# linkedin/spark-tfrecord

Hardware: AMD Instinct MI355X
Metric: rows/sec read+write (1M-row Example round-trip) (higher is better)
Workload: dtype wire(int64/float32/bytes); 1 GPU; model=Example{id:int64, ints:Int64List[8], floats:FloatList[16], tokens:BytesList[2]}, global_batch=1000000, parallelism=dp1, rows_per_rank=1000000, engine=gpu, storage=/dev/shm, crc_verify=True

## Files before the change

### csrc/codec_core.h

```cpp
#pragma once

#include <cstdint>
#include <cstring>

#include "crc32c.h"

namespace tfrec {

using i64 = int64_t;
using u64 = uint64_t;
using u32 = uint32_t;
using u8 = uint8_t;

enum Kind : int32_t { KIND_BYTES = 1, KIND_FLOAT = 2, KIND_INT64 = 3 };

enum RecordFormat : int32_t { FMT_EXAMPLE = 0, FMT_SEQUENCE = 1, FMT_BYTE_ARRAY = 2 };

enum CodecErr : int32_t {
  ERR_OK = 0,
  ERR_TRUNCATED = -1,
  ERR_BAD_VARINT = -2,
  ERR_KIND_MISMATCH = -3,
  ERR_BAD_WIRETYPE = -4,
  ERR_OVERFLOW = -5,
  ERR_NAME_TOO_LONG = -6,
};


TFR_HOSTDEV inline int popcount64(u64 x) { return __builtin_popcountll(x); }

TFR_HOSTDEV inline int ctz64(u64 x) { return __builtin_ctzll(x); }

constexpr u64 kMsbMask = 0x8080808080808080ull;

TFR_HOSTDEV inline const u8* read_varint(const u8* p, const u8* end, u64* out) {
  if (end - p >= 8) {
    u64 w;
    __builtin_memcpy(&w, p, 8);
    u64 stops = ~w & kMsbMask;
    if (stops) {
      int nb = (ctz64(stops) >> 3) + 1;
      u64 v = 0;
      for (int i = 0; i < nb; ++i)
        v |= ((w >> (8 * i)) & 0x7F) << (7 * i);
      *out = v;
      return p + nb;
    }
    u64 v = 0;
    for (int i = 0; i < 8; ++i) v |= ((w >> (8 * i)) & 0x7F) << (7 * i);
    const u8* q = p + 8;
    for (int shift = 56; q < end && shift < 64; shift += 7) {
      u8 b = *q++;
      v |= static_cast<u64>(b & 0x7F) << shift;
      if (!(b & 0x80)) {
        *out = v;
        return q;
      }
    }
    return nullptr;
  }
  u64 v = 0;
  int shift = 0;
  while (p < end) {
    u8 b = *p++;
    v |= static_cast<u64>(b & 0x7F) << shift;
    if (!(b & 0x80)) {
      *out = v;
      return p;
    }
    shift += 7;
    if (shift >= 64) return nullptr;
  }
  return nullptr;
}

TFR_HOSTDEV inline int varint_size(u64 v) {
  int n = 1;
  while (v >= 0x80) {
    v >>= 7;
    ++n;
  }
  return n;
}

TFR_HOSTDEV inline u8* write_varint(u8* p, u64 v) {
  while (v >= 0x80) {
    *p++ = static_cast<u8>(v) | 0x80;
    v >>= 7;
  }
  *p++ = static_cast<u8>(v);
  return p;
}


struct FieldDescRaw {
  int32_t kind;
  int32_t is_seq;
  int32_t name_off;
  int32_t name_len;
};

struct SchemaView {
  int32_t nfields;
  const FieldDescRaw* fields;
  const u8* names;

  TFR_HOSTDEV const u8* name(int f) const { return names + fields[f].name_off; }
  TFR_HOSTDEV int name_len(int f) const { return fields[f].name_len; }
};

TFR_HOSTDEV inline SchemaView schema_view(const u8* blob) {
  SchemaView v;
  int32_t n;
  __builtin_memcpy(&n, blob, 4);
  v.nfields = n;
  v.fields = reinterpret_cast<const FieldDescRaw*>(blob + 4);
  v.names = blob + 4 + n * static_cast<int>(sizeof(FieldDescRaw));
  return v;
}

TFR_HOSTDEV inline bool name_eq(const u8* a, const u8* b, int n) {
  while (n >= 8) {
    u64 x, y;
    __builtin_memcpy(&x, a, 8);
    __builtin_memcpy(&y, b, 8);
    if (x != y) return false;
    a += 8;
    b += 8;
    n -= 8;
  }
  for (int i = 0; i < n; ++i)
    if (a[i] != b[i]) return false;
  return true;
}

TFR_HOSTDEV inline int schema_find(const SchemaView& s, const u8* name, int len,
                                   int want_seq) {
  for (int f = 0; f < s.nfields; ++f) {
    if (s.fields[f].is_seq == want_seq && s.fields[f].name_len == len &&
        name_eq(s.name(f), name, len))
      return f;
  }
  return -1;
}


struct FieldStat {
  i64 pos;
  i64 len;
  i64 nvals;
  i64 nbytes;
  i64 nlists;
  int32_t kind_found;
  int32_t err;
};

TFR_HOSTDEV inline void field_stat_clear(FieldStat* st) {
  st->pos = -1;
  st->len = 0;
  st->nvals = 0;
  st->nbytes = 0;
  st->nlists = 0;
  st->kind_found = 0;
  st->err = 0;
}

TFR_HOSTDEV inline const u8* skip_field(const u8* p, const u8* end, u32 wiretype) {
  u64 tmp;
  switch (wiretype) {
    case 0:
      return read_varint(p, end, &tmp);
    case 1:
      return (end - p >= 8) ? p + 8 : nullptr;
    case 2:
      p = read_varint(p, end, &tmp);
      if (!p || static_cast<u64>(end - p) < tmp) return nullptr;
      return p + tmp;
    case 5:
      return (end - p >= 4) ? p + 4 : nullptr;
    default:
      return nullptr;
  }
}

TFR_HOSTDEV inline int32_t count_list_body(const u8* p, const u8* end, int32_t kind,
                                           i64* nvals, i64* nbytes) {
  while (p < end) {
    u64 tag;
    p = read_varint(p, end, &tag);
    if (!p) return ERR_BAD_VARINT;
    u32 fieldno = static_cast<u32>(tag >> 3);
    u32 wt = static_cast<u32>(tag & 7);
    if (fieldno != 1) {
      p = skip_field(p, end, wt);
      if (!p) return ERR_TRUNCATED;
      continue;
    }
    if (kind == KIND_BYTES) {
      if (wt != 2) return ERR_BAD_WIRETYPE;
      u64 len;
      p = read_varint(p, end, &len);
      if (!p || static_cast<u64>(end - p) < len) return ERR_TRUNCATED;
      *nvals += 1;
      *nbytes += static_cast<i64>(len);
      p += len;
    } else if (kind == KIND_FLOAT) {
      if (wt == 2) {
        u64 len;
        p = read_varint(p, end, &len);
        if (!p || static_cast<u64>(end - p) < len) return ERR_TRUNCATED;
        *nvals += static_cast<i64>(len / 4);
        p += len;
      } else if (wt == 5) {
        if (end - p < 4) return ERR_TRUNCATED;
        *nvals += 1;
        p += 4;
      } else {
        return ERR_BAD_WIRETYPE;
      }
    } else {
      if (wt == 2) {
        u64 len;
        p = read_varint(p, end, &len);
        if (!p || static_cast<u64>(end - p) < len) return ERR_TRUNCATED;
        const u8* q = p;
        const u8* qe = p + len;
        if (len && (qe[-1] & 0x80)) return ERR_BAD_VARINT;
        i64 cnt = 0;
        while (qe - q >= 8) {
          u64 w;
          __builtin_memcpy(&w, q, 8);
          cnt += popcount64(~w & kMsbMask);
          q += 8;
        }
        for (; q < qe; ++q) cnt += !(*q & 0x80);
        *nvals += cnt;
        p = qe;
      } else if (wt == 0) {
        u64 v;
        p = read_varint(p, end, &v);
        if (!p) return ERR_BAD_VARINT;
        *nvals += 1;
      } else {
        return ERR_BAD_WIRETYPE;
      }
    }
  }
  return ERR_OK;
}

TFR_HOSTDEV inline int32_t scan_feature_body(const u8* p, const u8* end,
                                             int32_t expect_kind, int32_t* kind_found,
                                             i64* nvals, i64* nbytes) {
  while (p < end) {
    u64 tag;
    p = read_varint(p, end, &tag);
    if (!p) return ERR_BAD_VARINT;
    u32 fieldno = static_cast<u32>(tag >> 3);
    u32 wt = static_cast<u32>(tag & 7);
    if (fieldno >= 1 && fieldno <= 3 && wt == 2) {
      u64 len;
      p = read_varint(p, end, &len);
      if (!p || static_cast<u64>(end - p) < len) return ERR_TRUNCATED;
      *kind_found = static_cast<int32_t>(fieldno);
      if (expect_kind >= 0 && static_cast<int32_t>(fieldno) != expect_kind)
        return ERR_KIND_MISMATCH;
      int32_t rc = count_list_body(p, p + len, static_cast<int32_t>(fieldno), nvals,
                                   nbytes);
      if (rc != ERR_OK) return rc;
      p += len;
    } else {
      p = skip_field(p, end, wt);
      if (!p) return ERR_TRUNCATED;
    }
  }
  return ERR_OK;
}

TFR_HOSTDEV inline int32_t scan_features_body(const u8* p, const u8* end, i64 base,
                                              const SchemaView& schema, int want_seq,
                                              FieldStat* stats) {
  const u8* body_start = p;
  while (p < end) {
    u64 tag;
    p = read_varint(p, end, &tag);
    if (!p) return ERR_BAD_VARINT;
    u32 fieldno = static_cast<u32>(tag >> 3);
    u32 wt = static_cast<u32>(tag & 7);
    if (fieldno != 1 || wt != 2) {
      p = skip_field(p, end, wt);
      if (!p) return ERR_TRUNCATED;
      continue;
    }
    u64 entry_len;
    p = read_varint(p, end, &entry_len);
    if (!p || static_cast<u64>(end - p) < entry_len) return ERR_TRUNCATED;
    const u8* ep = p;
    const u8* ee = p + entry_len;
    p = ee;
    const u8* key = nullptr;
    u64 key_len = 0;
    const u8* val = nullptr;
    u64 val_len = 0;
    while (ep < ee) {
      u64 etag;
      ep = read_varint(ep, ee, &etag);
      if (!ep) return ERR_BAD_VARINT;
      u32 efn = static_cast<u32>(etag >> 3);
      u32 ewt = static_cast<u32>(etag & 7);
      if (efn == 1 && ewt == 2) {
        ep = read_varint(ep, ee, &key_len);
        if (!ep || static_cast<u64>(ee - ep) < key_len) return ERR_TRUNCATED;
        key = ep;
        ep += key_len;
      } else if (efn == 2 && ewt == 2) {
        ep = read_varint(ep, ee, &val_len);
        if (!ep || static_cast<u64>(ee - ep) < val_len) return ERR_TRUNCATED;
        val = ep;
        ep += val_len;
      } else {
        ep = skip_field(ep, ee, ewt);
        if (!ep) return ERR_TRUNCATED;
      }
    }
    if (!key) continue;
    int f = schema_find(schema, key, static_cast<int>(key_len), want_seq);
    if (f < 0) continue;
    FieldStat* st = &stats[f];
    st->nvals = 0;
    st->nbytes = 0;
    st->nlists = 0;
    st->kind_found = 0;
    st->err = 0;
    st->pos = base + (val ? (val - body_start) : 0);
    st->len = static_cast<i64>(val_len);
    if (!want_seq) {
      int32_t rc = scan_feature_body(val, val + val_len, schema.fields[f].kind,
                                     &st->kind_found, &st->nvals, &st->nbytes);
      if (rc != ERR_OK) st->err = rc;
    } else {
      const u8* lp = val;
      const u8* le = val + val_len;
      while (lp < le) {
        u64 ltag;
        lp = read_varint(lp, le, &ltag);
        if (!lp) {
          st->err = ERR_BAD_VARINT;
          break;
        }
        u32 lfn = static_cast<u32>(ltag >> 3);
        u32 lwt = static_cast<u32>(ltag & 7);
        if (lfn == 1 && lwt == 2) {
          u64 flen;
          lp = read_varint(lp, le, &flen);
          if (!lp || static_cast<u64>(le - lp) < flen) {
            st->err = ERR_TRUNCATED;
            break;
          }
          st->nlists += 1;
          int32_t kf = 0;
          int32_t rc = scan_feature_body(lp, lp + flen, schema.fields[f].kind, &kf,
                                         &st->nvals, &st->nbytes);
          if (rc != ERR_OK) {
            st->err = rc;
            break;
          }
          if (kf) st->kind_found = kf;
          lp += flen;
        } else {
          lp = skip_field(lp, le, lwt);
          if (!lp) {
            st->err = ERR_TRUNCATED;
            break;
          }
        }
      }
    }
  }
  return ERR_OK;
}

TFR_HOSTDEV inline int32_t scan_record(const u8* data, i64 abs_off, i64 rec_len,
                                       int32_t fmt, const SchemaView& schema,
                                       FieldStat* stats) {
  const u8* p = data + abs_off;
  const u8* end = p + rec_len;
  while (p < end) {
    u64 tag;
    p = read_varint(p, end, &tag);
    if (!p) return ERR_BAD_VARINT;
    u32 fieldno = static_cast<u32>(tag >> 3);
    u32 wt = static_cast<u32>(tag & 7);
    bool is_features =
        (fmt == FMT_EXAMPLE && fieldno == 1) || (fmt == FMT_SEQUENCE && fieldno == 1);
    bool is_feature_lists = (fmt == FMT_SEQUENCE && fieldno == 2);
    if ((is_features || is_feature_lists) && wt == 2) {
      u64 len;
      p = read_varint(p, end, &len);
      if (!p || static_cast<u64>(end - p) < len) return ERR_TRUNCATED;
      i64 base = (p - data);
      if (is_features) {
        int32_t rc = scan_features_body(p, p + len, base, schema, 0, stats);
        if (rc != ERR_OK) return rc;
      } else {
        int32_t rc = scan_features_body(p, p + len, base, schema, 1, stats);
        if (rc != ERR_OK) return rc;
      }
      p += len;
    } else {
      p = skip_field(p, end, wt);
      if (!p) return ERR_TRUNCATED;
    }
  }
  return ERR_OK;
}


constexpr int32_t ERR_RETRY_UNFUSED = -100;

TFR_HOSTDEV inline u32 crc32c_step8(u32 crc, u64 w, const uint32_t (*tab)[256]) {
  w ^= crc;
  return tab[7][w & 0xFF] ^ tab[6][(w >> 8) & 0xFF] ^ tab[5][(w >> 16) & 0xFF] ^
         tab[4][(w >> 24) & 0xFF] ^ tab[3][(w >> 32) & 0xFF] ^
         tab[2][(w >> 40) & 0xFF] ^ tab[1][(w >> 48) & 0xFF] ^
         tab[0][(w >> 56) & 0xFF];
}

struct ScanCur {
  const u8* base;
  i64 len;
  i64 pos;
  i64 wpos;
  u64 w0, w1;
  u32 crc;
  const uint32_t (*tab)[256];
};

TFR_HOSTDEV inline u64 cur_load(const ScanCur& c, i64 at) {
  if (at + 8 <= c.len) {
    u64 w;
    __builtin_memcpy(&w, c.base + at, 8);
    return w;
  }
  u64 w = 0;
  for (i64 b = at; b < c.len; ++b) w |= (u64)c.base[b] << (8 * (b - at));
  return w;
}

TFR_HOSTDEV inline void cur_init(ScanCur& c, const u8* base, i64 len,
                                 const uint32_t (*tab)[256]) {
  c.base = base;
  c.len = len;
  c.pos = 0;
  c.wpos = 0;
  c.tab = tab;
  c.crc = 0xFFFFFFFFu;
  c.w0 = cur_load(c, 0);
  c.w1 = cur_load(c, 8);
}

TFR_HOSTDEV inline u64 cur_peek(const ScanCur& c) {
  int sh = (int)(c.pos - c.wpos) * 8;
  if (sh == 0) return c.w0;
  if (sh == 64) return c.w1;
  return (c.w0 >> sh) | (c.w1 << (64 - sh));
}

TFR_HOSTDEV inline void cur_advance(ScanCur& c, i64 k) {
  c.pos += k;
  while (c.pos > c.wpos + 8) {
    if (c.wpos + 8 <= c.len) c.crc = crc32c_step8(c.crc, c.w0, c.tab);
    c.w0 = c.w1;
    c.wpos += 8;
    c.w1 = cur_load(c, c.wpos + 8);
  }
}

TFR_HOSTDEV inline u32 cur_finish_crc(ScanCur& c) {
  while (c.wpos + 8 <= c.len) {
    c.crc = crc32c_step8(c.crc, c.w0, c.tab);
    c.w0 = c.w1;
    c.wpos += 8;
    c.w1 = cur_load(c, c.wpos + 8);
  }
  u32 crc = c.crc;
  for (i64 b = c.wpos; b < c.len; ++b)
    crc = c.tab[0][(crc ^ c.base[b]) & 0xFF] ^ (crc >> 8);
  return ~crc;
}

TFR_HOSTDEV inline bool cur_varint(ScanCur& c, i64 end, u64* out) {
  i64 avail = end - c.pos;
  if (avail <= 0) return false;
  u64 w = cur_peek(c);
  u64 stops = ~w & kMsbMask;
  if (stops) {
    int nb = (ctz64(stops) >> 3) + 1;
    if (nb > avail) return false;
    u64 v = 0;
    for (int i = 0; i < nb; ++i) v |= ((w >> (8 * i)) & 0x7F) << (7 * i);
    *out = v;
    cur_advance(c, nb);
    return true;
  }
  if (avail < 9) return false;
  u64 v = 0;
  for (int i = 0; i < 8; ++i) v |= ((w >> (8 * i)) & 0x7F) << (7 * i);
  cur_advance(c, 8);
  for (int shift = 56; shift < 64 && c.pos < end; shift += 7) {
    u8 b = (u8)cur_peek(c);
    v |= (u64)(b & 0x7F) << shift;
    cur_advance(c, 1);
    if (!(b & 0x80)) {
      *out = v;
      return true;
    }
  }
  return false;
}

TFR_HOSTDEV inline int32_t cur_skip_field(ScanCur& c, i64 end, u32 wt) {
  u64 tmp;
  switch (wt) {
    case 0:
      return cur_varint(c, end, &tmp) ? ERR_OK : ERR_BAD_VARINT;
    case 1:
      if (end - c.pos < 8) return ERR_TRUNCATED;
      cur_advance(c, 8);
      return ERR_OK;
    case 2:
      if (!cur_varint(c, end, &tmp)) return ERR_BAD_VARINT;
      if ((u64)(end - c.pos) < tmp) return ERR_TRUNCATED;
      cur_advance(c, (i64)tmp);
      return ERR_OK;
    case 5:
      if (end - c.pos < 4) return ERR_TRUNCATED;
      cur_advance(c, 4);
      return ERR_OK;
    default:
      return ERR_BAD_WIRETYPE;
  }
}

TFR_HOSTDEV inline i64 cur_count_terms(ScanCur& c, i64 n) {
  i64 cnt = 0;
  while (n >= 8) {
    cnt += popcount64(~cur_peek(c) & kMsbMask);
    cur_advance(c, 8);
    n -= 8;
  }
  if (n > 0) {
    u64 mask = kMsbMask >> (8 * (8 - n));
    cnt += popcount64(~cur_peek(c) & mask);
    cur_advance(c, n);
  }
  return cnt;
}

TFR_HOSTDEV inline int32_t cur_count_list_body(ScanCur& c, i64 end, int32_t kind,
                                               i64* nvals, i64* nbytes) {
  while (c.pos < end) {
    u64 tag;
    if (!cur_varint(c, end, &tag)) return ERR_BAD_VARINT;
    u32 fieldno = (u32)(tag >> 3), wt = (u32)(tag & 7);
    if (fieldno != 1) {
      int32_t rc = cur_skip_field(c, end, wt);
      if (rc != ERR_OK) return rc;
      continue;
    }
    if (kind == KIND_BYTES) {
      if (wt != 2) return ERR_BAD_WIRETYPE;
      u64 blen;
      if (!cur_varint(c, end, &blen)) return ERR_BAD_VARINT;
      if ((u64)(end - c.pos) < blen) return ERR_TRUNCATED;
      *nvals += 1;
      *nbytes += (i64)blen;
      cur_advance(c, (i64)blen);
    } else if (kind == KIND_FLOAT) {
      if (wt == 2) {
        u64 blen;
        if (!cur_varint(c, end, &blen)) return ERR_BAD_VARINT;
        if ((u64)(end - c.pos) < blen) return ERR_TRUNCATED;
        *nvals += (i64)(blen / 4);
        cur_advance(c, (i64)blen);
      } else if (wt == 5) {
        if (end - c.pos < 4) return ERR_TRUNCATED;
        *nvals += 1;
        cur_advance(c, 4);
      } else {
        return ERR_BAD_WIRETYPE;
      }
    } else {
      if (wt == 2) {
        u64 blen;
        if (!cur_varint(c, end, &blen)) return ERR_BAD_VARINT;
        if ((u64)(end - c.pos) < blen) return ERR_TRUNCATED;
        if (blen && (c.base[c.pos + (i64)blen - 1] & 0x80))
          return ERR_BAD_VARINT;
        *nvals += cur_count_terms(c, (i64)blen);
      } else if (wt == 0) {
        u64 v;
        if (!cur_varint(c, end, &v)) return ERR_BAD_VARINT;
        *nvals += 1;
      } else {
        return ERR_BAD_WIRETYPE;
      }
    }
  }
  return ERR_OK;
}

TFR_HOSTDEV inline int32_t cur_scan_feature_body(ScanCur& c, i64 end,
                                                 int32_t expect_kind,
                                                 int32_t* kind_found, i64* nvals,
                                                 i64* nbytes) {
  while (c.pos < end) {
    u64 tag;
    if (!cur_varint(c, end, &tag)) return ERR_BAD_VARINT;
    u32 fieldno = (u32)(tag >> 3), wt = (u32)(tag & 7);
    if (fieldno >= 1 && fieldno <= 3 && wt == 2) {
      u64 blen;
      if (!cur_varint(c, end, &blen)) return ERR_BAD_VARINT;
      if ((u64)(end - c.pos) < blen) return ERR_TRUNCATED;
      *kind_found = (int32_t)fieldno;
      if (expect_kind >= 0 && (int32_t)fieldno != expect_kind)
        return ERR_KIND_MISMATCH;
      int32_t rc = cur_count_list_body(c, c.pos + (i64)blen, (int32_t)fieldno,
                                       nvals, nbytes);
      if (rc != ERR_OK) return rc;
    } else {
      int32_t rc = cur_skip_field(c, end, wt);
      if (rc != ERR_OK) return rc;
    }
  }
  return ERR_OK;
}

TFR_HOSTDEV inline int32_t cur_scan_features_body(ScanCur& c, i64 end, i64 data_rel,
                                                  const SchemaView& schema,
                                                  int want_seq, FieldStat* stats) {
  i64 body_start = c.pos;
  while (c.pos < end) {
    u64 tag;
    if (!cur_varint(c, end, &tag)) return ERR_BAD_VARINT;
    u32 fieldno = (u32)(tag >> 3), wt = (u32)(tag & 7);
    if (fieldno != 1 || wt != 2) {
      int32_t rc = cur_skip_field(c, end, wt);
      if (rc != ERR_OK) return rc;
      continue;
    }
    u64 entry_len;
    if (!cur_varint(c, end, &entry_len)) return ERR_BAD_VARINT;
    if ((u64)(end - c.pos) < entry_len) return ERR_TRUNCATED;
    i64 ee = c.pos + (i64)entry_len;
    int f = -1;
    bool key_seen = false;
    bool val_seen = false;
    while (c.pos < ee) {
      u64 etag;
      if (!cur_varint(c, ee, &etag)) return ERR_BAD_VARINT;
      u32 efn = (u32)(etag >> 3), ewt = (u32)(etag & 7);
      if (efn == 1 && ewt == 2) {
        if (val_seen) return ERR_RETRY_UNFUSED;
        u64 klen;
        if (!cur_varint(c, ee, &klen)) return ERR_BAD_VARINT;
        if ((u64)(ee - c.pos) < klen) return ERR_TRUNCATED;
        f = schema_find(schema, c.base + c.pos, (int)klen, want_seq);
        key_seen = true;
        cur_advance(c, (i64)klen);
      } else if (efn == 2 && ewt == 2) {
        if (!key_seen) return ERR_RETRY_UNFUSED;
        val_seen = true;
        u64 vlen;
        if (!cur_varint(c, ee, &vlen)) return ERR_BAD_VARINT;
        if ((u64)(ee - c.pos) < vlen) return ERR_TRUNCATED;
        i64 ve = c.pos + (i64)vlen;
        if (f < 0) {
          cur_advance(c, (i64)vlen);
          continue;
        }
        FieldStat* st = &stats[f];
        st->nvals = 0;
        st->nbytes = 0;
        st->nlists = 0;
        st->kind_found = 0;
        st->err = 0;
        st->pos = data_rel + c.pos;
        st->len = (i64)vlen;
        if (!want_seq) {
          int32_t rc = cur_scan_feature_body(c, ve, schema.fields[f].kind,
                                             &st->kind_found, &st->nvals,
                                             &st->nbytes);
          if (rc == ERR_RETRY_UNFUSED) return rc;
          if (rc != ERR_OK) st->err = rc;
        } else {
          while (c.pos < ve && st->err == ERR_OK) {
            u64 ltag;
            if (!cur_varint(c, ve, &ltag)) {
              st->err = ERR_BAD_VARINT;
              break;
            }
            u32 lfn = (u32)(ltag >> 3), lwt = (u32)(ltag & 7);
            if (lfn == 1 && lwt == 2) {
              u64 flen;
              if (!cur_varint(c, ve, &flen) || (u64)(ve - c.pos) < flen) {
                st->err = ERR_TRUNCATED;
                break;
              }
              st->nlists += 1;
              int32_t kf = 0;
              int32_t rc = cur_scan_feature_body(c, c.pos + (i64)flen,
                                                 schema.fields[f].kind, &kf,
                                                 &st->nvals, &st->nbytes);
              if (rc == ERR_RETRY_UNFUSED) return rc;
              if (rc != ERR_OK) {
                st->err = rc;
                break;
              }
              if (kf) st->kind_found = kf;
            } else {
              int32_t rc = cur_skip_field(c, ve, lwt);
              if (rc != ERR_OK) {
                st->err = ERR_TRUNCATED;
                break;
              }
            }
          }
        }
        if (c.pos < ve) cur_advance(c, ve - c.pos);
      } else {
        int32_t rc = cur_skip_field(c, ee, ewt);
        if (rc != ERR_OK) return rc;
      }
    }
    if (f >= 0 && !val_seen) {
      FieldStat* st = &stats[f];
      st->pos = data_rel + body_start;
      st->len = 0;
      st->nvals = 0;
      st->nbytes = 0;
      st->nlists = 0;
      st->kind_found = 0;
      st->err = 0;
    }
  }
  return ERR_OK;
}

TFR_HOSTDEV inline int32_t scan_record_fused(const u8* data, i64 abs_off,
                                             i64 rec_len, int32_t fmt,
                                             const SchemaView& schema,
                                             FieldStat* stats, u32* crc_out,
                                             const uint32_t (*tab)[256]) {
  ScanCur c;
  cur_init(c, data + abs_off, rec_len, tab);
  while (c.pos < rec_len) {
    u64 tag;
    if (!cur_varint(c, rec_len, &tag)) return ERR_BAD_VARINT;
    u32 fieldno = (u32)(tag >> 3), wt = (u32)(tag & 7);
    bool is_features = fieldno == 1;
    bool is_fl = (fmt == FMT_SEQUENCE && fieldno == 2);
    if ((is_features || is_fl) && wt == 2) {
      u64 blen;
      if (!cur_varint(c, rec_len, &blen)) return ERR_BAD_VARINT;
      if ((u64)(rec_len - c.pos) < blen) return ERR_TRUNCATED;
      int32_t rc = cur_scan_features_body(c, c.pos + (i64)blen, abs_off, schema,
                                          is_fl ? 1 : 0, stats);
      if (rc != ERR_OK) return rc;
    } else {
      int32_t rc = cur_skip_field(c, rec_len, wt);
      if (rc != ERR_OK) return rc;
    }
  }
  *crc_out = cur_finish_crc(c);
  return ERR_OK;
}


struct DecodeDst {
  i64* i64_vals;
  float* f32_vals;
  u8* bytes_data;
  i64* elem_len;
  i64* sub_count;
};


template <bool OFFS = false>
TFR_HOSTDEV inline int32_t extract_list_body(const u8* p, const u8* end, int32_t kind,
                                             const DecodeDst& dst, i64* vi, i64* bi) {
  while (p < end) {
    u64 tag;
    p = read_varint(p, end, &tag);
    if (!p) return ERR_BAD_VARINT;
    u32 fieldno = static_cast<u32>(tag >> 3);
    u32 wt = static_cast<u32>(tag & 7);
    if (fieldno != 1) {
      p = skip_field(p, end, wt);
      if (!p) return ERR_TRUNCATED;
      continue;
    }
    if (kind == KIND_BYTES) {
      u64 len;
      p = read_varint(p, end, &len);
      if (!p || static_cast<u64>(end - p) < len) return ERR_TRUNCATED;
      u8* d = dst.bytes_data + *bi;
      u64 i = 0;
      for (; i + 8 <= len; i += 8) {
        u64 w;
        __builtin_memcpy(&w, p + i, 8);
        __builtin_memcpy(d + i, &w, 8);
      }
      for (; i < len; ++i) d[i] = p[i];
      dst.elem_len[*vi] = OFFS ? *bi : static_cast<i64>(len);
      *bi += static_cast<i64>(len);
      *vi += 1;
      p += len;
    } else if (kind == KIND_FLOAT) {
      if (wt == 2) {
        u64 len;
        p = read_varint(p, end, &len);
        if (!p || static_cast<u64>(end - p) < len) return ERR_TRUNCATED;
        u64 n = len / 4;
        __builtin_memcpy(dst.f32_vals + *vi, p, n * 4);
        *vi += static_cast<i64>(n);
        p += len;
      } else {
        if (end - p < 4) return ERR_TRUNCATED;
        float v;
        __builtin_memcpy(&v, p, 4);
        dst.f32_vals[(*vi)++] = v;
        p += 4;
      }
    } else {
      if (wt == 2) {
        u64 len;
        p = read_varint(p, end, &len);
        if (!p || static_cast<u64>(end - p) < len) return ERR_TRUNCATED;
        const u8* q = p;
        const u8* qe = p + len;
        while (q < qe) {
          u64 v;
          q = read_varint(q, qe, &v);
          if (!q) return ERR_BAD_VARINT;
          dst.i64_vals[(*vi)++] = static_cast<i64>(v);
        }
        p = qe;
      } else {
        u64 v;
        p = read_varint(p, end, &v);
        if (!p) return ERR_BAD_VARINT;
        dst.i64_vals[(*vi)++] = static_cast<i64>(v);
      }
    }
  }
  return ERR_OK;
}

template <bool OFFS = false>
TFR_HOSTDEV inline int32_t extract_feature_body(const u8* p, const u8* end,
                                                int32_t kind, const DecodeDst& dst,
                                                i64* vi, i64* bi) {
  while (p < end) {
    u64 tag;
    p = read_varint(p, end, &tag);
    if (!p) return ERR_BAD_VARINT;
    u32 fieldno = static_cast<u32>(tag >> 3);
    u32 wt = static_cast<u32>(tag & 7);
    if (fieldno >= 1 && fieldno <= 3 && wt == 2) {
      u64 len;
      p = read_varint(p, end, &len);
      if (!p || static_cast<u64>(end - p) < len) return ERR_TRUNCATED;
      int32_t rc = extract_list_body<OFFS>(p, p + len, kind, dst, vi, bi);
      if (rc != ERR_OK) return rc;
      p += len;
    } else {
      p = skip_field(p, end, wt);
      if (!p) return ERR_TRUNCATED;
    }
  }
  return ERR_OK;
}

template <bool OFFS = false>
TFR_HOSTDEV inline int32_t extract_field(const u8* data, i64 pos, i64 len,
                                         int32_t kind, int32_t is_seq,
                                         const DecodeDst& dst, i64 val_base,
                                         i64 byte_base, i64 list_base) {
  if (pos < 0) return ERR_OK;
  const u8* p = data + pos;
  const u8* end = p + len;
  i64 vi = val_base;
  i64 bi = byte_base;
  if (!is_seq)
    return extract_feature_body<OFFS>(p, end, kind, dst, &vi, &bi);
  i64 li = list_base;
  while (p < end) {
    u64 tag;
    p = read_varint(p, end, &tag);
    if (!p) return ERR_BAD_VARINT;
    u32 fieldno = static_cast<u32>(tag >> 3);
    u32 wt = static_cast<u32>(tag & 7);
    if (fieldno == 1 && wt == 2) {
      u64 flen;
      p = read_varint(p, end, &flen);
      if (!p || static_cast<u64>(end - p) < flen) return ERR_TRUNCATED;
      i64 v_before = vi;
      int32_t rc = extract_feature_body<OFFS>(p, p + flen, kind, dst, &vi, &bi);
      if (rc != ERR_OK) return rc;
      dst.sub_count[li++] = OFFS ? v_before : vi - v_before;
      p += flen;
    } else {
      p = skip_field(p, end, wt);
      if (!p) return ERR_TRUNCATED;
    }
  }
  return ERR_OK;
}


struct FieldColumn {
  int32_t kind;
  int32_t is_seq;
  const u8* presence;
  const i64* row_off;
  const i64* list_off;
  const i64* sub_off;
  const i64* elem_off;
  const u8* bytes_data;
  const i64* i64_vals;
  const float* f32_vals;
};

TFR_HOSTDEV inline i64 list_body_size(const FieldColumn& c, i64 v0, i64 v1) {
  if (c.kind == KIND_FLOAT) {
    i64 n = v1 - v0;
    return n ? (1 + varint_size(static_cast<u64>(4 * n)) + 4 * n) : 0;
  }
  if (c.kind == KIND_INT64) {
    i64 packed = 0;
    for (i64 v = v0; v < v1; ++v)
      packed += varint_size(static_cast<u64>(c.i64_vals[v]));
    return packed ? (1 + varint_size(static_cast<u64>(packed)) + packed) : 0;
  }
  i64 sz = 0;
  for (i64 v = v0; v < v1; ++v) {
    i64 blen = c.elem_off[v + 1] - c.elem_off[v];
    sz += 1 + varint_size(static_cast<u64>(blen)) + blen;
  }
  return sz;
}

TFR_HOSTDEV inline i64 feature_body_size(const FieldColumn& c, i64 v0, i64 v1) {
  i64 body = list_body_size(c, v0, v1);
  return 1 + varint_size(static_cast<u64>(body)) + body;
}

TFR_HOSTDEV inline u8* emit_list_body(u8* o, const FieldColumn& c, i64 v0, i64 v1) {
  if (c.kind == KIND_FLOAT) {
    i64 n = v1 - v0;
    if (n) {
      *o++ = 0x0A;
      o = write_varint(o, static_cast<u64>(4 * n));
      __builtin_memcpy(o, c.f32_vals + v0, static_cast<size_t>(4 * n));
      o += 4 * n;
    }
  } else if (c.kind == KIND_INT64) {
    i64 packed = 0;
    for (i64 v = v0; v < v1; ++v)
      packed += varint_size(static_cast<u64>(c.i64_vals[v]));
    if (packed) {
      *o++ = 0x0A;
      o = write_varint(o, static_cast<u64>(packed));
      for (i64 v = v0; v < v1; ++v)
        o = write_varint(o, static_cast<u64>(c.i64_vals[v]));
    }
  } else {
    for (i64 v = v0; v < v1; ++v) {
      i64 b0 = c.elem_off[v];
      i64 blen = c.elem_off[v + 1] - b0;
      *o++ = 0x0A;
      o = write_varint(o, static_cast<u64>(blen));
      for (i64 i = 0; i < blen; ++i) o[i] = c.bytes_data[b0 + i];
      o += blen;
    }
  }
  return o;
}

TFR_HOSTDEV inline u8* emit_feature_body(u8* o, const FieldColumn& c, i64 v0, i64 v1) {
  i64 body = list_body_size(c, v0, v1);
  *o++ = static_cast<u8>((c.kind << 3) | 2);
  o = write_varint(o, static_cast<u64>(body));
  return emit_list_body(o, c, v0, v1);
}

TFR_HOSTDEV inline i64 features_entry_size(const FieldColumn& c, const SchemaView& s,
                                           int f, i64 v0, i64 v1) {
  i64 fb = feature_body_size(c, v0, v1);
  i64 klen = s.name_len(f);
  return (1 + varint_size(static_cast<u64>(klen)) + klen) +
         (1 + varint_size(static_cast<u64>(fb)) + fb);
}

TFR_HOSTDEV inline u8* emit_features_entry(u8* o, const FieldColumn& c,
                                           const SchemaView& s, int f, i64 v0, i64 v1) {
  i64 fb = feature_body_size(c, v0, v1);
  i64 klen = s.name_len(f);
  *o++ = 0x0A;
  o = write_varint(o, static_cast<u64>(klen));
  const u8* nm = s.name(f);
  for (i64 i = 0; i < klen; ++i) o[i] = nm[i];
  o += klen;
  *o++ = 0x12;
  o = write_varint(o, static_cast<u64>(fb));
  return emit_feature_body(o, c, v0, v1);
}

TFR_HOSTDEV inline i64 feature_list_body_size(const FieldColumn& c, i64 r) {
  i64 sz = 0;
  for (i64 j = c.list_off[r]; j < c.list_off[r + 1]; ++j) {
    i64 fb = feature_body_size(c, c.sub_off[j], c.sub_off[j + 1]);
    sz += 1 + varint_size(static_cast<u64>(fb)) + fb;
  }
  return sz;
}

TFR_HOSTDEV inline u8* emit_feature_list_body(u8* o, const FieldColumn& c, i64 r) {
  for (i64 j = c.list_off[r]; j < c.list_off[r + 1]; ++j) {
    i64 fb = feature_body_size(c, c.sub_off[j], c.sub_off[j + 1]);
    *o++ = 0x0A;
    o = write_varint(o, static_cast<u64>(fb));
    o = emit_feature_body(o, c, c.sub_off[j], c.sub_off[j + 1]);
  }
  return o;
}

TFR_HOSTDEV inline i64 feature_lists_entry_size(const FieldColumn& c,
                                                const SchemaView& s, int f, i64 r) {
  i64 flb = feature_list_body_size(c, r);
  i64 klen = s.name_len(f);
  return (1 + varint_size(static_cast<u64>(klen)) + klen) +
         (1 + varint_size(static_cast<u64>(flb)) + flb);
}

TFR_HOSTDEV inline u8* emit_feature_lists_entry(u8* o, const FieldColumn& c,
                                                const SchemaView& s, int f, i64 r) {
  i64 flb = feature_list_body_size(c, r);
  i64 klen = s.name_len(f);
  *o++ = 0x0A;
  o = write_varint(o, static_cast<u64>(klen));
  const u8* nm = s.name(f);
  for (i64 i = 0; i < klen; ++i) o[i] = nm[i];
  o += klen;
  *o++ = 0x12;
  o = write_varint(o, static_cast<u64>(flb));
  return emit_feature_list_body(o, c, r);
}

TFR_HOSTDEV inline i64 record_payload_size(const FieldColumn* cols,
                                           const SchemaView& s, int32_t fmt, i64 r) {
  i64 ctx_body = 0;
  i64 fl_body = 0;
  for (int f = 0; f < s.nfields; ++f) {
    const FieldColumn& c = cols[f];
    if (!c.presence[r]) continue;
    if (!c.is_seq) {
      i64 e = features_entry_size(c, s, f, c.row_off[r], c.row_off[r + 1]);
      ctx_body += 1 + varint_size(static_cast<u64>(e)) + e;
    } else {
      i64 e = feature_lists_entry_size(c, s, f, r);
      fl_body += 1 + varint_size(static_cast<u64>(e)) + e;
    }
  }
  i64 total = 0;
  if (fmt == FMT_EXAMPLE) {
    total += 1 + varint_size(static_cast<u64>(ctx_body)) + ctx_body;
  } else {
    if (ctx_body) total += 1 + varint_size(static_cast<u64>(ctx_body)) + ctx_body;
    total += 1 + varint_size(static_cast<u64>(fl_body)) + fl_body;
  }
  return total;
}

TFR_HOSTDEV inline u8* emit_record_payload(u8* o, const FieldColumn* cols,
                                           const SchemaView& s, int32_t fmt, i64 r) {
  i64 ctx_body = 0, fl_body = 0;
  for (int f = 0; f < s.nfields; ++f) {
    const FieldColumn& c = cols[f];
    if (!c.presence[r]) continue;
    if (!c.is_seq) {
      i64 e = features_entry_size(c, s, f, c.row_off[r], c.row_off[r + 1]);
      ctx_body += 1 + varint_size(static_cast<u64>(e)) + e;
    } else {
      i64 e = feature_lists_entry_size(c, s, f, r);
      fl_body += 1 + varint_size(static_cast<u64>(e)) + e;
    }
  }
  auto emit_ctx = [&](u8* oo) {
    for (int f = 0; f < s.nfields; ++f) {
      const FieldColumn& c = cols[f];
      if (!c.presence[r] || c.is_seq) continue;
      i64 e = features_entry_size(c, s, f, c.row_off[r], c.row_off[r + 1]);
      *oo++ = 0x0A;
      oo = write_varint(oo, static_cast<u64>(e));
      oo = emit_features_entry(oo, c, s, f, c.row_off[r], c.row_off[r + 1]);
    }
    return oo;
  };
  auto emit_fl = [&](u8* oo) {
    for (int f = 0; f < s.nfields; ++f) {
      const FieldColumn& c = cols[f];
      if (!c.presence[r] || !c.is_seq) continue;
      i64 e = feature_lists_entry_size(c, s, f, r);
      *oo++ = 0x0A;
      oo = write_varint(oo, static_cast<u64>(e));
      oo = emit_feature_lists_entry(oo, c, s, f, r);
    }
    return oo;
  };
  if (fmt == FMT_EXAMPLE) {
    *o++ = 0x0A;
    o = write_varint(o, static_cast<u64>(ctx_body));
    o = emit_ctx(o);
  } else {
    if (ctx_body) {
      *o++ = 0x0A;
      o = write_varint(o, static_cast<u64>(ctx_body));
      o = emit_ctx(o);
    }
    *o++ = 0x12;
    o = write_varint(o, static_cast<u64>(fl_body));
    o = emit_fl(o);
  }
  return o;
}



struct WriteCur {
  u8* base;
  i64 pos;
  i64 wpos;
  u64 win;
  u32 crc;
  const uint32_t (*tab)[256];
};

TFR_HOSTDEV inline void wcur_init(WriteCur& w, u8* base,
                                  const uint32_t (*tab)[256]) {
  w.base = base;
  w.pos = 0;
  w.wpos = 0;
  w.win = 0;
  w.crc = 0xFFFFFFFFu;
  w.tab = tab;
}

TFR_HOSTDEV inline void wcur_flush8(WriteCur& w) {
  __builtin_memcpy(w.base + w.wpos, &w.win, 8);
  w.crc = crc32c_step8(w.crc, w.win, w.tab);
  w.wpos += 8;
  w.win = 0;
}

TFR_HOSTDEV inline void wcur_put(WriteCur& w, u8 b) {
  w.win |= (u64)b << (8 * (w.pos - w.wpos));
  if (++w.pos - w.wpos == 8) wcur_flush8(w);
}

TFR_HOSTDEV inline void wcur_varint(WriteCur& w, u64 v) {
  while (v >= 0x80) {
    wcur_put(w, (u8)(v | 0x80));
    v >>= 7;
  }
  wcur_put(w, (u8)v);
}

TFR_HOSTDEV inline void wcur_bytes(WriteCur& w, const u8* src, i64 n) {
  while (n > 0 && (w.pos - w.wpos) != 0) {
    wcur_put(w, *src++);
    --n;
  }
  while (n >= 8) {
    __builtin_memcpy(&w.win, src, 8);
    w.pos += 8;
    wcur_flush8(w);
    src += 8;
    n -= 8;
  }
  while (n-- > 0) wcur_put(w, *src++);
}

TFR_HOSTDEV inline u32 wcur_finish(WriteCur& w) {
  int rem = (int)(w.pos - w.wpos);
  if (!rem) return ~w.crc;
  __builtin_memcpy(w.base + w.wpos, &w.win, (size_t)rem);
  u32 crc = w.crc;
  for (int i = 0; i < rem; ++i)
    crc = w.tab[0][(crc ^ (u8)(w.win >> (8 * i))) & 0xFF] ^ (crc >> 8);
  return ~crc;
}

TFR_HOSTDEV inline void wcur_list_body(WriteCur& w, const FieldColumn& c,
                                       i64 v0, i64 v1) {
  if (c.kind == KIND_FLOAT) {
    i64 n = v1 - v0;
    if (n) {
      wcur_put(w, 0x0A);
      wcur_varint(w, (u64)(4 * n));
      wcur_bytes(w, (const u8*)(c.f32_vals + v0), 4 * n);
    }
  } else if (c.kind == KIND_INT64) {
    i64 packed = 0;
    for (i64 v = v0; v < v1; ++v)
      packed += varint_size((u64)c.i64_vals[v]);
    if (packed) {
      wcur_put(w, 0x0A);
      wcur_varint(w, (u64)packed);
      for (i64 v = v0; v < v1; ++v) wcur_varint(w, (u64)c.i64_vals[v]);
    }
  } else {
    for (i64 v = v0; v < v1; ++v) {
      i64 b0 = c.elem_off[v];
      i64 blen = c.elem_off[v + 1] - b0;
      wcur_put(w, 0x0A);
      wcur_varint(w, (u64)blen);
      wcur_bytes(w, c.bytes_data + b0, blen);
    }
  }
}

TFR_HOSTDEV inline void wcur_feature_body(WriteCur& w, const FieldColumn& c,
                                          i64 v0, i64 v1) {
  i64 body = list_body_size(c, v0, v1);
  wcur_put(w, (u8)((c.kind << 3) | 2));
  wcur_varint(w, (u64)body);
  wcur_list_body(w, c, v0, v1);
}

TFR_HOSTDEV inline void wcur_features_entry(WriteCur& w, const FieldColumn& c,
                                            const SchemaView& s, int f, i64 v0,
                                            i64 v1) {
  i64 fb = feature_body_size(c, v0, v1);
  i64 klen = s.name_len(f);
  wcur_put(w, 0x0A);
  wcur_varint(w, (u64)klen);
  wcur_bytes(w, s.name(f), klen);
  wcur_put(w, 0x12);
  wcur_varint(w, (u64)fb);
  wcur_feature_body(w, c, v0, v1);
}

TFR_HOSTDEV inline void wcur_feature_list_body(WriteCur& w,
                                               const FieldColumn& c, i64 r) {
  for (i64 j = c.list_off[r]; j < c.list_off[r + 1]; ++j) {
    i64 fb = feature_body_size(c, c.sub_off[j], c.sub_off[j + 1]);
    wcur_put(w, 0x0A);
    wcur_varint(w, (u64)fb);
    wcur_feature_body(w, c, c.sub_off[j], c.sub_off[j + 1]);
  }
}

TFR_HOSTDEV inline void wcur_feature_lists_entry(WriteCur& w,
                                                 const FieldColumn& c,
                                                 const SchemaView& s, int f,
                                                 i64 r) {
  i64 flb = feature_list_body_size(c, r);
  i64 klen = s.name_len(f);
  wcur_put(w, 0x0A);
  wcur_varint(w, (u64)klen);
  wcur_bytes(w, s.name(f), klen);
  wcur_put(w, 0x12);
  wcur_varint(w, (u64)flb);
  wcur_feature_list_body(w, c, r);
}

TFR_HOSTDEV inline i64 emit_record_payload_fused(u8* o, const FieldColumn* cols,
                                                 const SchemaView& s, int32_t fmt,
                                                 i64 r, u32* crc_out,
                                                 const uint32_t (*tab)[256]) {
  i64 ctx_body = 0, fl_body = 0;
  for (int f = 0; f < s.nfields; ++f) {
    const FieldColumn& c = cols[f];
    if (!c.presence[r]) continue;
    if (!c.is_seq) {
      i64 e = features_entry_size(c, s, f, c.row_off[r], c.row_off[r + 1]);
      ctx_body += 1 + varint_size((u64)e) + e;
    } else {
      i64 e = feature_lists_entry_size(c, s, f, r);
      fl_body += 1 + varint_size((u64)e) + e;
    }
  }
  WriteCur w;
  wcur_init(w, o, tab);
  auto emit_ctx = [&]() {
    for (int f = 0; f < s.nfields; ++f) {
      const FieldColumn& c = cols[f];
      if (!c.presence[r] || c.is_seq) continue;
      i64 e = features_entry_size(c, s, f, c.row_off[r], c.row_off[r + 1]);
      wcur_put(w, 0x0A);
      wcur_varint(w, (u64)e);
      wcur_features_entry(w, c, s, f, c.row_off[r], c.row_off[r + 1]);
    }
  };
  auto emit_fl = [&]() {
    for (int f = 0; f < s.nfields; ++f) {
      const FieldColumn& c = cols[f];
      if (!c.presence[r] || !c.is_seq) continue;
      i64 e = feature_lists_entry_size(c, s, f, r);
      wcur_put(w, 0x0A);
      wcur_varint(w, (u64)e);
      wcur_feature_lists_entry(w, c, s, f, r);
    }
  };
  if (fmt == FMT_EXAMPLE) {
    wcur_put(w, 0x0A);
    wcur_varint(w, (u64)ctx_body);
    emit_ctx();
  } else {
    if (ctx_body) {
      wcur_put(w, 0x0A);
      wcur_varint(w, (u64)ctx_body);
      emit_ctx();
    }
    wcur_put(w, 0x12);
    wcur_varint(w, (u64)fl_body);
    emit_fl();
  }
  *crc_out = wcur_finish(w);
  return w.pos;
}

constexpr i64 kFrameOverhead = 16;

TFR_HOSTDEV inline void write_frame_header_footer(u8* file, i64 frame_off,
                                                  i64 payload_len,
                                                  const u32 (*tab)[256]) {
  u8* h = file + frame_off;
  u64 len_le = static_cast<u64>(payload_len);
  __builtin_memcpy(h, &len_le, 8);
  u32 lc = mask_crc(crc32c_sw(h, 8, 0, tab));
  __builtin_memcpy(h + 8, &lc, 4);
  u32 dc = mask_crc(crc32c_sw(h + 12, static_cast<size_t>(payload_len), 0, tab));
  __builtin_memcpy(h + 12 + payload_len, &dc, 4);
}

TFR_HOSTDEV inline void write_frame_header_footer_crc(u8* file, i64 frame_off,
                                                      i64 payload_len,
                                                      u32 payload_crc,
                                                      const u32 (*tab)[256]) {
  u8* h = file + frame_off;
  u64 len_le = static_cast<u64>(payload_len);
  __builtin_memcpy(h, &len_le, 8);
  u32 lc = mask_crc(crc32c_sw(h, 8, 0, tab));
  __builtin_memcpy(h + 8, &lc, 4);
  u32 dc = mask_crc(payload_crc);
  __builtin_memcpy(h + 12 + payload_len, &dc, 4);
}

}
```

### csrc/hip/kernels.hip

```cpp

#include <hip/hip_runtime.h>
#include <pybind11/pybind11.h>
#include <pybind11/stl.h>
#include <rocprim/rocprim.hpp>

#include <fcntl.h>
#include <sys/mman.h>
#include <sys/stat.h>
#include <unistd.h>

#include <cstdint>
#include <map>
#include <mutex>
#include <stdexcept>
#include <string>
#include <vector>

#include "../codec_core.h"

namespace py = pybind11;
using namespace tfrec;

#define HIP_CHECK(expr)                                                          \
  do {                                                                           \
    hipError_t _e = (expr);                                                      \
    if (_e != hipSuccess)                                                        \
      throw std::runtime_error(std::string("HIP error: ") +                      \
                               hipGetErrorString(_e) + " at " __FILE__ ":" +     \
                               std::to_string(__LINE__));                        \
  } while (0)

namespace {

constexpr int kBlock = 256;

__device__ inline void stage_crc_tables(uint32_t (*lds)[256]) {
  const uint32_t* src = &kCrcTables.t[0][0];
  uint32_t* dst = &lds[0][0];
  for (int i = threadIdx.x; i < 8 * 256; i += blockDim.x) dst[i] = src[i];
  __syncthreads();
}

__device__ inline void set_err(int32_t* err, int32_t code, i64 r) {
  err[0] = code;
  i64 v = r + 1;
  atomicMax(&err[1], v > 0x7FFFFFFF ? (int32_t)0x7FFFFFFF : (int32_t)v);
}


__global__ void crc_verify_kernel(const u8* __restrict__ data,
                                  const i64* __restrict__ off,
                                  const i64* __restrict__ len, i64 R,
                                  unsigned long long* err_out) {
  __shared__ uint32_t tab[8][256];
  stage_crc_tables(tab);
  for (i64 r = blockIdx.x * (i64)blockDim.x + threadIdx.x; r < R;
       r += (i64)gridDim.x * blockDim.x) {
    const u8* h = data + off[r] - 12;
    u32 len_crc, data_crc;
    __builtin_memcpy(&len_crc, h + 8, 4);
    __builtin_memcpy(&data_crc, h + 12 + len[r], 4);
    bool ok = mask_crc(crc32c_sw(h, 8, 0, tab)) == len_crc &&
              mask_crc(crc32c_sw(h + 12, (size_t)len[r], 0, tab)) == data_crc;
    if (!ok) atomicMin(err_out, (unsigned long long)(r + 1));
  }
}


static_assert(sizeof(FieldStat) == 48, "FieldStat layout shared with Python");

__global__ void scan_records_kernel(const u8* __restrict__ data,
                                    const i64* __restrict__ off,
                                    const i64* __restrict__ len, i64 R, int32_t fmt,
                                    const u8* __restrict__ schema_blob, int F,
                                    FieldStat* __restrict__ stats,
                                    int32_t* __restrict__ err,
                                    unsigned long long* crc_err,
                                    i64 rec_base, const i64* gate) {
  __shared__ uint32_t tab[8][256];
  if (gate && *gate) return;
  if (crc_err) stage_crc_tables(tab);
  SchemaView schema = schema_view(schema_blob);
  for (i64 r = blockIdx.x * (i64)blockDim.x + threadIdx.x; r < R;
       r += (i64)gridDim.x * blockDim.x) {
    FieldStat* st = stats + r * F;
    for (int f = 0; f < F; ++f) field_stat_clear(&st[f]);
    int32_t rc;
    if (crc_err) {
      u32 payload_crc = 0;
      rc = scan_record_fused(data, off[r], len[r], fmt, schema, st,
                             &payload_crc, tab);
      if (rc == ERR_RETRY_UNFUSED) {
        for (int f = 0; f < F; ++f) field_stat_clear(&st[f]);
        rc = scan_record(data, off[r], len[r], fmt, schema, st);
        payload_crc = crc32c_sw(data + off[r], (size_t)len[r], 0, tab);
      }
      if (rc != ERR_OK)
        payload_crc = crc32c_sw(data + off[r], (size_t)len[r], 0, tab);
      const u8* h = data + off[r] - 12;
      u32 len_crc, data_crc;
      __builtin_memcpy(&len_crc, h + 8, 4);
      __builtin_memcpy(&data_crc, h + 12 + len[r], 4);
      bool ok = mask_crc(crc32c_sw(h, 8, 0, tab)) == len_crc &&
                mask_crc(payload_crc) == data_crc;
      if (!ok) atomicMin(crc_err, (unsigned long long)(rec_base + r + 1));
    } else {
      rc = scan_record(data, off[r], len[r], fmt, schema, st);
    }
    if (rc != ERR_OK) set_err(err, rc, rec_base + r);
    for (int f = 0; f < F; ++f)
      if (st[f].err != ERR_OK) set_err(err, st[f].err, rec_base + r);
  }
}


struct DevFieldDst {
  int32_t kind;
  int32_t is_seq;
  i64* i64_vals;
  float* f32_vals;
  u8* bytes_data;
  i64* elem_off;
  i64* sub_off;
  u8* presence;
  const i64* val_base;
  const i64* byte_base;
  const i64* list_base;
  i64 cap_vals;
  i64 cap_bytes;
  i64 cap_elem_off;
  i64 cap_sub_off;
};

__device__ inline void store_end_sentinels(const DevFieldDst* __restrict__ metas,
                                           int F, i64 r_end) {
  if (blockIdx.x != 0) return;
  for (int f = threadIdx.x; f < F; f += blockDim.x) {
    const DevFieldDst& m = metas[f];
    if (m.kind == KIND_BYTES && m.elem_off && m.val_base && m.byte_base)
      m.elem_off[m.val_base[r_end]] = m.byte_base[r_end];
    if (m.is_seq && m.sub_off && m.list_base && m.val_base)
      m.sub_off[m.list_base[r_end]] = m.val_base[r_end];
  }
}

__global__ void extract_gate_kernel(const DevFieldDst* __restrict__ metas, int F,
                                    i64 r_end, const i64* broken,
                                    const unsigned long long* crc,
                                    const int32_t* scan_err, i64* refused) {
  int bad = 0;
  if (threadIdx.x == 0) {
    if (broken && *broken) bad = 1;
    if (crc && *crc != ~0ULL) bad = 1;
    if (scan_err && scan_err[0] != 0) bad = 1;
  }
  for (int f = threadIdx.x; f < F; f += blockDim.x) {
    const DevFieldDst& m = metas[f];
    i64 nv = m.val_base ? m.val_base[r_end] : 0;
    i64 nb = m.byte_base ? m.byte_base[r_end] : 0;
    i64 nl = m.list_base ? m.list_base[r_end] : 0;
    if (m.kind == KIND_BYTES) {
      if (nb > m.cap_bytes || nv + 1 > m.cap_elem_off) bad = 1;
    } else if (nv > m.cap_vals) {
      bad = 1;
    }
    if (m.is_seq && nl + 1 > m.cap_sub_off) bad = 1;
  }
  int any = __syncthreads_or(bad);
  if (threadIdx.x == 0) *refused = any ? 1 : 0;
}

__global__ void extract_fields_kernel(const u8* __restrict__ data, i64 R, int F,
                                      const FieldStat* __restrict__ stats,
                                      const DevFieldDst* __restrict__ metas,
                                      int32_t* __restrict__ err, i64 r0,
                                      const i64* refused) {
  if (refused && *refused) return;
  store_end_sentinels(metas, F, r0 + R);
  i64 total = R * F;
  for (i64 idx = blockIdx.x * (i64)blockDim.x + threadIdx.x; idx < total;
       idx += (i64)gridDim.x * blockDim.x) {
    i64 q = idx / F;
    int f = (int)(idx - q * F);
    i64 r = r0 + q;
    const DevFieldDst& m = metas[f];
    const FieldStat& st = stats[r * F + f];
    DecodeDst dst{m.i64_vals, m.f32_vals, m.bytes_data, m.elem_off, m.sub_off};
    if (m.presence) m.presence[r] = st.pos >= 0 ? 1 : 0;
    int32_t rc = extract_field<true>(data, st.pos, st.len, m.kind, m.is_seq,
                                     dst, m.val_base ? m.val_base[r] : 0,
                                     m.byte_base ? m.byte_base[r] : 0,
                                     m.list_base ? m.list_base[r] : 0);
    if (rc != ERR_OK) set_err(err, rc, r);
  }
}



__global__ void size_records_kernel(const FieldColumn* __restrict__ cols,
                                    const u8* __restrict__ schema_blob, int32_t fmt,
                                    i64 R, i64* __restrict__ psize) {
  SchemaView schema = schema_view(schema_blob);
  for (i64 r = blockIdx.x * (i64)blockDim.x + threadIdx.x; r < R;
       r += (i64)gridDim.x * blockDim.x) {
    psize[r] = record_payload_size(cols, schema, fmt, r) + kFrameOverhead;
  }
}

__global__ void emit_records_kernel(const FieldColumn* __restrict__ cols,
                                    const u8* __restrict__ schema_blob, int32_t fmt,
                                    i64 r0, i64 R, const i64* __restrict__ frame_off,
                                    u8* __restrict__ file,
                                    int32_t* __restrict__ err) {
  __shared__ uint32_t tab[8][256];
  stage_crc_tables(tab);
  SchemaView schema = schema_view(schema_blob);
  for (i64 r = r0 + blockIdx.x * (i64)blockDim.x + threadIdx.x; r < R;
       r += (i64)gridDim.x * blockDim.x) {
    i64 payload = (frame_off[r + 1] - frame_off[r]) - kFrameOverhead;
    u8* o = file + frame_off[r] + 12;
    u32 crc = 0;
    i64 emitted = emit_record_payload_fused(o, cols, schema, fmt, r, &crc,
                                            tab);
    if (emitted != payload) set_err(err, ERR_OVERFLOW, r);
    write_frame_header_footer_crc(file, frame_off[r], payload, crc, tab);
  }
}


constexpr i64 kWaveRecordBytes = 8 << 10;

__device__ inline u32 crc32c_wave(const u8* p, i64 n,
                                  const uint32_t (*tab)[256]) {
  int lane = threadIdx.x & 63;
  i64 chunk = (n + 63) / 64;
  if (chunk < 64) chunk = 64;
  i64 s = (i64)lane * chunk;
  i64 e = s + chunk < n ? s + chunk : n;
  u32 my = (s < e) ? crc32c_sw(p + s, (size_t)(e - s), 0, tab) : 0;
  u32 acc = __shfl(my, 0);
  if (chunk < n) {
    u32 op = crc32c_shift_elem((u64)chunk);
    for (int i = 1; i < 64; ++i) {
      i64 si = (i64)i * chunk;
      if (si >= n) break;
      u32 ci = __shfl(my, i);
      i64 li = (si + chunk < n ? chunk : n - si);
      acc = (li == chunk) ? (crc_gfmul(acc, op) ^ ci)
                          : crc32c_combine_fast(acc, ci, (u64)li);
    }
  }
  return acc;
}

__device__ inline void copy_wave(u8* d, const u8* s, i64 n) {
  int lane = threadIdx.x & 63;
  i64 i = (i64)lane * 8;
  for (; i + 8 <= n; i += 64 * 8) {
    u64 w;
    __builtin_memcpy(&w, s + i, 8);
    __builtin_memcpy(d + i, &w, 8);
  }
  i64 tail = n & ~((i64)7);
  for (i64 b = tail + lane; b < n; b += 64) d[b] = s[b];
}

__global__ void crc_verify_wave_kernel(const u8* __restrict__ data,
                                       const i64* __restrict__ off,
                                       const i64* __restrict__ len, i64 R,
                                       unsigned long long* err_out) {
  __shared__ uint32_t tab[8][256];
  stage_crc_tables(tab);
  i64 wave = (blockIdx.x * (i64)blockDim.x + threadIdx.x) / 64;
  i64 nwaves = ((i64)gridDim.x * blockDim.x) / 64;
  for (i64 r = wave; r < R; r += nwaves) {
    const u8* h = data + off[r] - 12;
    u32 payload = crc32c_wave(h + 12, len[r], tab);
    if ((threadIdx.x & 63) == 0) {
      u32 len_crc, data_crc;
      __builtin_memcpy(&len_crc, h + 8, 4);
      __builtin_memcpy(&data_crc, h + 12 + len[r], 4);
      bool ok = mask_crc(crc32c_sw(h, 8, 0, tab)) == len_crc &&
                mask_crc(payload) == data_crc;
      if (!ok) atomicMin(err_out, (unsigned long long)(r + 1));
    }
  }
}

__global__ void frame_bytes_wave_kernel(const u8* __restrict__ src,
                                        const i64* __restrict__ elem_off,
                                        const i64* __restrict__ frame_off, i64 R,
                                        u8* __restrict__ file) {
  __shared__ uint32_t tab[8][256];
  stage_crc_tables(tab);
  i64 wave = (blockIdx.x * (i64)blockDim.x + threadIdx.x) / 64;
  i64 nwaves = ((i64)gridDim.x * blockDim.x) / 64;
  for (i64 r = wave; r < R; r += nwaves) {
    i64 n = elem_off[r + 1] - elem_off[r];
    const u8* s = src + elem_off[r];
    u8* d = file + frame_off[r] + 12;
    copy_wave(d, s, n);
    u32 crc = crc32c_wave(s, n, tab);
    if ((threadIdx.x & 63) == 0)
      write_frame_header_footer_crc(file, frame_off[r], n, crc, tab);
  }
}

__global__ void gather_payloads_wave_kernel(const u8* __restrict__ data,
                                            const i64* __restrict__ off,
                                            const i64* __restrict__ len,
                                            const i64* __restrict__ dst_off,
                                            i64 R, u8* __restrict__ out) {
  i64 wave = (blockIdx.x * (i64)blockDim.x + threadIdx.x) / 64;
  i64 nwaves = ((i64)gridDim.x * blockDim.x) / 64;
  for (i64 r = wave; r < R; r += nwaves)
    copy_wave(out + dst_off[r], data + off[r], len[r]);
}


__device__ inline i64 wave_incl_scan(i64 v) {
  int lane = threadIdx.x & 63;
  for (int d = 1; d < 64; d <<= 1) {
    i64 y = __shfl_up(v, d);
    if (lane >= d) v += y;
  }
  return v;
}

__device__ inline i64 wave_extract_i64_packed(const u8* __restrict__ p, i64 n,
                                              i64* __restrict__ out, i64 base,
                                              bool* bad) {
  int lane = threadIdx.x & 63;
  i64 chunk = (n + 63) / 64;
  i64 lo = (i64)lane * chunk;
  i64 hi = lo + chunk < n ? lo + chunk : n;
  i64 cnt = 0;
  for (i64 i = lo; i < hi; ++i) cnt += !(p[i] & 0x80);
  i64 incl = wave_incl_scan(cnt);
  i64 excl = incl - cnt;
  i64 total = __shfl(incl, 63);
  i64 q = lo;
  i64 pre = 0;
  if (lo > 0 && lo < hi) {
    if (p[lo - 1] & 0x80) {
      while (q < hi && (p[q] & 0x80)) ++q;
      if (q < hi) {
        ++q;
        pre = 1;
      }
    }
  }
  i64 idx = base + excl + pre;
  i64 idx_end = base + total;
  bool overlong = false;
  while (q < hi) {
    u64 v = 0;
    int shift = 0;
    i64 j = q;
    bool terminated = false;
    while (j < n && shift < 70) {
      u8 b = p[j++];
      v |= (u64)(b & 0x7F) << shift;
      shift += 7;
      if (!(b & 0x80)) {
        terminated = true;
        break;
      }
    }
    if (!terminated) {
      overlong = true;
      break;
    }
    if (idx < idx_end) out[idx] = (i64)v;
    ++idx;
    q = j;
  }
  *bad = __any(overlong) != 0;
  return total;
}

__device__ inline int32_t extract_list_body_wave(const u8* __restrict__ p,
                                                 const u8* end, int32_t kind,
                                                 const DecodeDst& dst, i64* vi,
                                                 i64* bi) {
  int lane = threadIdx.x & 63;
  while (p < end) {
    u64 tag;
    p = read_varint(p, end, &tag);
    if (!p) return ERR_BAD_VARINT;
    u32 fieldno = (u32)(tag >> 3), wt = (u32)(tag & 7);
    if (fieldno != 1) {
      p = skip_field(p, end, wt);
      if (!p) return ERR_TRUNCATED;
      continue;
    }
    if (kind == KIND_BYTES) {
      u64 len;
      p = read_varint(p, end, &len);
      if (!p || (u64)(end - p) < len) return ERR_TRUNCATED;
      copy_wave(dst.bytes_data + *bi, p, (i64)len);
      if (lane == 0) dst.elem_len[*vi] = *bi;
      *bi += (i64)len;
      *vi += 1;
      p += len;
    } else if (kind == KIND_FLOAT) {
      if (wt == 2) {
        u64 len;
        p = read_varint(p, end, &len);
        if (!p || (u64)(end - p) < len) return ERR_TRUNCATED;
        u64 nv = len / 4;
        copy_wave((u8*)(dst.f32_vals + *vi), p, (i64)(nv * 4));
        *vi += (i64)nv;
        p += len;
      } else {
        if (end - p < 4) return ERR_TRUNCATED;
        if (lane == 0) {
          float v;
          __builtin_memcpy(&v, p, 4);
          dst.f32_vals[*vi] = v;
        }
        (*vi)++;
        p += 4;
      }
    } else {
      if (wt == 2) {
        u64 len;
        p = read_varint(p, end, &len);
        if (!p || (u64)(end - p) < len) return ERR_TRUNCATED;
        bool bad;
        *vi += wave_extract_i64_packed(p, (i64)len, dst.i64_vals, *vi, &bad);
        if (bad) return ERR_BAD_VARINT;
        p += len;
      } else {
        u64 v;
        p = read_varint(p, end, &v);
        if (!p) return ERR_BAD_VARINT;
        if (lane == 0) dst.i64_vals[*vi] = (i64)v;
        (*vi)++;
      }
    }
  }
  return ERR_OK;
}

__device__ inline int32_t extract_feature_body_wave(const u8* __restrict__ p,
                                                    const u8* end, int32_t kind,
                                                    const DecodeDst& dst,
                                                    i64* vi, i64* bi) {
  while (p < end) {
    u64 tag;
    p = read_varint(p, end, &tag);
    if (!p) return ERR_BAD_VARINT;
    u32 fieldno = (u32)(tag >> 3), wt = (u32)(tag & 7);
    if (fieldno >= 1 && fieldno <= 3 && wt == 2) {
      u64 len;
      p = read_varint(p, end, &len);
      if (!p || (u64)(end - p) < len) return ERR_TRUNCATED;
      int32_t rc = extract_list_body_wave(p, p + len, kind, dst, vi, bi);
      if (rc != ERR_OK) return rc;
      p += len;
    } else {
      p = skip_field(p, end, wt);
      if (!p) return ERR_TRUNCATED;
    }
  }
  return ERR_OK;
}

__device__ inline int32_t extract_field_wave(const u8* __restrict__ data,
                                             i64 pos, i64 len, int32_t kind,
                                             int32_t is_seq, const DecodeDst& dst,
                                             i64 val_base, i64 byte_base,
                                             i64 list_base) {
  if (pos < 0) return ERR_OK;
  int lane = threadIdx.x & 63;
  const u8* p = data + pos;
  const u8* end = p + len;
  i64 vi = val_base;
  i64 bi = byte_base;
  if (!is_seq) return extract_feature_body_wave(p, end, kind, dst, &vi, &bi);
  i64 li = list_base;
  while (p < end) {
    u64 tag;
    p = read_varint(p, end, &tag);
    if (!p) return ERR_BAD_VARINT;
    u32 fieldno = (u32)(tag >> 3), wt = (u32)(tag & 7);
    if (fieldno == 1 && wt == 2) {
      u64 flen;
      p = read_varint(p, end, &flen);
      if (!p || (u64)(end - p) < flen) return ERR_TRUNCATED;
      i64 v_before = vi;
      int32_t rc = extract_feature_body_wave(p, p + flen, kind, dst, &vi, &bi);
      if (rc != ERR_OK) return rc;
      if (lane == 0) dst.sub_count[li] = v_before;
      ++li;
      p += flen;
    } else {
      p = skip_field(p, end, wt);
      if (!p) return ERR_TRUNCATED;
    }
  }
  return ERR_OK;
}

__global__ void scan_records_wave_kernel(const u8* __restrict__ data,
                                         const i64* __restrict__ off,
                                         const i64* __restrict__ len, i64 R,
                                         int32_t fmt,
                                         const u8* __restrict__ schema_blob,
                                         int F, FieldStat* __restrict__ stats,
                                         int32_t* __restrict__ err,
                                         unsigned long long* crc_err,
                                         i64 rec_base, const i64* gate) {
  __shared__ uint32_t tab[8][256];
  if (gate && *gate) return;
  stage_crc_tables(tab);
  SchemaView schema = schema_view(schema_blob);
  i64 wave = (blockIdx.x * (i64)blockDim.x + threadIdx.x) / 64;
  i64 nwaves = ((i64)gridDim.x * blockDim.x) / 64;
  int lane = threadIdx.x & 63;
  for (i64 r = wave; r < R; r += nwaves) {
    if (lane == 0) {
      FieldStat* st = stats + r * F;
      for (int f = 0; f < F; ++f) field_stat_clear(&st[f]);
      int32_t rc = scan_record(data, off[r], len[r], fmt, schema, st);
      if (rc != ERR_OK) set_err(err, rc, rec_base + r);
      for (int f = 0; f < F; ++f)
        if (st[f].err != ERR_OK) set_err(err, st[f].err, rec_base + r);
    }
    if (crc_err) {
      const u8* h = data + off[r] - 12;
      u32 payload = crc32c_wave(h + 12, len[r], tab);
      if (lane == 0) {
        u32 len_crc, data_crc;
        __builtin_memcpy(&len_crc, h + 8, 4);
        __builtin_memcpy(&data_crc, h + 12 + len[r], 4);
        bool ok = mask_crc(crc32c_sw(h, 8, 0, tab)) == len_crc &&
                  mask_crc(payload) == data_crc;
        if (!ok) atomicMin(crc_err, (unsigned long long)(rec_base + r + 1));
      }
    }
  }
}

__global__ void extract_fields_wave_kernel(const u8* __restrict__ data, i64 R,
                                           int F,
                                           const FieldStat* __restrict__ stats,
                                           const DevFieldDst* __restrict__ metas,
                                           int32_t* __restrict__ err, i64 r0,
                                           const i64* refused) {
  if (refused && *refused) return;
  store_end_sentinels(metas, F, r0 + R);
  i64 total = R * F;
  i64 wave = (blockIdx.x * (i64)blockDim.x + threadIdx.x) / 64;
  i64 nwaves = ((i64)gridDim.x * blockDim.x) / 64;
  for (i64 idx = wave; idx < total; idx += nwaves) {
    i64 q = idx / F;
    int f = (int)(idx - q * F);
    i64 r = r0 + q;
    const DevFieldDst& m = metas[f];
    const FieldStat& st = stats[r * F + f];
    DecodeDst dst{m.i64_vals, m.f32_vals, m.bytes_data, m.elem_off, m.sub_off};
    bool lane0 = (threadIdx.x & 63) == 0;
    if (lane0 && m.presence) m.presence[r] = st.pos >= 0 ? 1 : 0;
    int32_t rc = extract_field_wave(data, st.pos, st.len, m.kind, m.is_seq, dst,
                                    m.val_base ? m.val_base[r] : 0,
                                    m.byte_base ? m.byte_base[r] : 0,
                                    m.list_base ? m.list_base[r] : 0);
    if (rc != ERR_OK && lane0) set_err(err, rc, r);
  }
}


__device__ inline i64 wave_emit_i64_packed(u8* __restrict__ o,
                                           const i64* __restrict__ vals,
                                           i64 v0, i64 v1) {
  int lane = threadIdx.x & 63;
  i64 n = v1 - v0;
  i64 chunk = (n + 63) / 64;
  i64 lo = v0 + (i64)lane * chunk;
  i64 hi = lo + chunk < v1 ? lo + chunk : v1;
  i64 sz = 0;
  for (i64 v = lo; v < hi; ++v) sz += varint_size((u64)vals[v]);
  i64 incl = wave_incl_scan(sz);
  u8* q = o + (incl - sz);
  for (i64 v = lo; v < hi; ++v) q = write_varint(q, (u64)vals[v]);
  return __shfl(incl, 63);
}

struct WaveCur {
  u8* base;
  i64 pos;
};

__device__ inline void wvc_put(WaveCur& w, u8 b) {
  if ((threadIdx.x & 63) == 0) w.base[w.pos] = b;
  w.pos += 1;
}

__device__ inline void wvc_varint(WaveCur& w, u64 v) {
  if ((threadIdx.x & 63) == 0) write_varint(w.base + w.pos, v);
  w.pos += varint_size(v);
}

__device__ inline void wvc_bytes(WaveCur& w, const u8* s, i64 n) {
  copy_wave(w.base + w.pos, s, n);
  w.pos += n;
}

__device__ inline void wvc_list_body(WaveCur& w, const FieldColumn& c, i64 v0,
                                     i64 v1) {
  if (c.kind == KIND_FLOAT) {
    i64 n = v1 - v0;
    if (n) {
      wvc_put(w, 0x0A);
      wvc_varint(w, (u64)(4 * n));
      wvc_bytes(w, (const u8*)(c.f32_vals + v0), 4 * n);
    }
  } else if (c.kind == KIND_INT64) {
    i64 packed = 0;
    for (i64 v = v0; v < v1; ++v) packed += varint_size((u64)c.i64_vals[v]);
    if (packed) {
      wvc_put(w, 0x0A);
      wvc_varint(w, (u64)packed);
      w.pos += wave_emit_i64_packed(w.base + w.pos, c.i64_vals, v0, v1);
    }
  } else {
    for (i64 v = v0; v < v1; ++v) {
      i64 b0 = c.elem_off[v];
      i64 blen = c.elem_off[v + 1] - b0;
      wvc_put(w, 0x0A);
      wvc_varint(w, (u64)blen);
      wvc_bytes(w, c.bytes_data + b0, blen);
    }
  }
}

__device__ inline void wvc_feature_body(WaveCur& w, const FieldColumn& c,
                                        i64 v0, i64 v1) {
  i64 body = list_body_size(c, v0, v1);
  wvc_put(w, (u8)((c.kind << 3) | 2));
  wvc_varint(w, (u64)body);
  wvc_list_body(w, c, v0, v1);
}

__device__ inline void wvc_features_entry(WaveCur& w, const FieldColumn& c,
                                          const SchemaView& s, int f, i64 v0,
                                          i64 v1) {
  i64 fb = feature_body_size(c, v0, v1);
  i64 klen = s.name_len(f);
  wvc_put(w, 0x0A);
  wvc_varint(w, (u64)klen);
  wvc_bytes(w, s.name(f), klen);
  wvc_put(w, 0x12);
  wvc_varint(w, (u64)fb);
  wvc_feature_body(w, c, v0, v1);
}

__device__ inline void wvc_feature_lists_entry(WaveCur& w, const FieldColumn& c,
                                               const SchemaView& s, int f,
                                               i64 r) {
  i64 flb = feature_list_body_size(c, r);
  i64 klen = s.name_len(f);
  wvc_put(w, 0x0A);
  wvc_varint(w, (u64)klen);
  wvc_bytes(w, s.name(f), klen);
  wvc_put(w, 0x12);
  wvc_varint(w, (u64)flb);
  for (i64 j = c.list_off[r]; j < c.list_off[r + 1]; ++j) {
    i64 fb = feature_body_size(c, c.sub_off[j], c.sub_off[j + 1]);
    wvc_put(w, 0x0A);
    wvc_varint(w, (u64)fb);
    wvc_feature_body(w, c, c.sub_off[j], c.sub_off[j + 1]);
  }
}

__device__ inline i64 emit_record_payload_wave(u8* o, const FieldColumn* cols,
                                               const SchemaView& s, int32_t fmt,
                                               i64 r) {
  i64 ctx_body = 0, fl_body = 0;
  for (int f = 0; f < s.nfields; ++f) {
    const FieldColumn& c = cols[f];
    if (!c.presence[r]) continue;
    if (!c.is_seq) {
      i64 e = features_entry_size(c, s, f, c.row_off[r], c.row_off[r + 1]);
      ctx_body += 1 + varint_size((u64)e) + e;
    } else {
      i64 e = feature_lists_entry_size(c, s, f, r);
      fl_body += 1 + varint_size((u64)e) + e;
    }
  }
  WaveCur w{o, 0};
  auto emit_ctx = [&]() {
    for (int f = 0; f < s.nfields; ++f) {
      const FieldColumn& c = cols[f];
      if (!c.presence[r] || c.is_seq) continue;
      i64 e = features_entry_size(c, s, f, c.row_off[r], c.row_off[r + 1]);
      wvc_put(w, 0x0A);
      wvc_varint(w, (u64)e);
      wvc_features_entry(w, c, s, f, c.row_off[r], c.row_off[r + 1]);
    }
  };
  auto emit_fl = [&]() {
    for (int f = 0; f < s.nfields; ++f) {
      const FieldColumn& c = cols[f];
      if (!c.presence[r] || !c.is_seq) continue;
      i64 e = feature_lists_entry_size(c, s, f, r);
      wvc_put(w, 0x0A);
      wvc_varint(w, (u64)e);
      wvc_feature_lists_entry(w, c, s, f, r);
    }
  };
  if (fmt == FMT_EXAMPLE) {
    wvc_put(w, 0x0A);
    wvc_varint(w, (u64)ctx_body);
    emit_ctx();
  } else {
    if (ctx_body) {
      wvc_put(w, 0x0A);
      wvc_varint(w, (u64)ctx_body);
      emit_ctx();
    }
    wvc_put(w, 0x12);
    wvc_varint(w, (u64)fl_body);
    emit_fl();
  }
  return w.pos;
}

__global__ void emit_records_wave_kernel(const FieldColumn* __restrict__ cols,
                                         const u8* __restrict__ schema_blob,
                                         int32_t fmt, i64 r0, i64 R,
                                         const i64* __restrict__ frame_off,
                                         u8* __restrict__ file,
                                         int32_t* __restrict__ err) {
  __shared__ uint32_t tab[8][256];
  stage_crc_tables(tab);
  SchemaView schema = schema_view(schema_blob);
  i64 wave = (blockIdx.x * (i64)blockDim.x + threadIdx.x) / 64;
  i64 nwaves = ((i64)gridDim.x * blockDim.x) / 64;
  int lane = threadIdx.x & 63;
  for (i64 r = r0 + wave; r < R; r += nwaves) {
    i64 payload = (frame_off[r + 1] - frame_off[r]) - kFrameOverhead;
    u8* o = file + frame_off[r] + 12;
    i64 emitted = emit_record_payload_wave(o, cols, schema, fmt, r);
    if (emitted != payload && lane == 0) set_err(err, ERR_OVERFLOW, r);
    __threadfence_block();
    u32 crc = crc32c_wave(o, payload, tab);
    if (lane == 0)
      write_frame_header_footer_crc(file, frame_off[r], payload, crc, tab);
  }
}

__global__ void frame_bytes_kernel(const u8* __restrict__ src,
                                   const i64* __restrict__ elem_off,
                                   const i64* __restrict__ frame_off, i64 R,
                                   u8* __restrict__ file) {
  __shared__ uint32_t tab[8][256];
  stage_crc_tables(tab);
  for (i64 r = blockIdx.x * (i64)blockDim.x + threadIdx.x; r < R;
       r += (i64)gridDim.x * blockDim.x) {
    i64 n = elem_off[r + 1] - elem_off[r];
    WriteCur w;
    wcur_init(w, file + frame_off[r] + 12, tab);
    wcur_bytes(w, src + elem_off[r], n);
    u32 crc = wcur_finish(w);
    write_frame_header_footer_crc(file, frame_off[r], n, crc, tab);
  }
}

__device__ inline u32 crc8b_reg(u64 w, const uint32_t (*tab)[256]) {
  w ^= 0xFFFFFFFFull;
  u32 c = tab[7][w & 0xFF] ^ tab[6][(w >> 8) & 0xFF] ^ tab[5][(w >> 16) & 0xFF] ^
          tab[4][(w >> 24) & 0xFF] ^ tab[3][(w >> 32) & 0xFF] ^
          tab[2][(w >> 40) & 0xFF] ^ tab[1][(w >> 48) & 0xFF] ^
          tab[0][(w >> 56) & 0xFF];
  return ~c;
}

constexpr int kPosPerLane = 16;

template <typename F>
__device__ inline void eval_frame_chunk(const u8* __restrict__ data,
                                        const u64* __restrict__ wdata, i64 N,
                                        i64 c, i64 pos_start, i64 pos_end,
                                        const uint32_t (*tab)[256], F&& f) {
  i64 p0 = c * kPosPerLane;
  i64 w0 = p0 >> 3;
  u64 w[4];
  if (p0 + 32 <= N) {
#pragma unroll
    for (int j = 0; j < 4; ++j) w[j] = wdata[w0 + j];
  } else {
#pragma unroll
    for (int j = 0; j < 4; ++j) {
      u64 v = 0;
      i64 boff = (w0 + j) * 8;
      for (int b = 0; b < 8 && boff + b < N; ++b)
        v |= (u64)data[boff + b] << (8 * b);
      w[j] = v;
    }
  }
#pragma unroll
  for (int k = 0; k < kPosPerLane; ++k) {
    i64 i = p0 + k;
    if (i + 16 > N || i >= pos_end) break;
    if (i < pos_start) continue;
    constexpr int _ppl = kPosPerLane;
    static_assert(_ppl == 16, "index math below assumes 16 positions");
    const int wi = k >> 3;
    const int sh = (k & 7) * 8;
    u64 len = (sh == 0) ? w[wi] : (w[wi] >> sh) | (w[wi + 1] << (64 - sh));
    if (len > (u64)(N - i) - 16) continue;
    const int wi2 = (k + 8) >> 3;
    const int sh2 = sh;
    u64 hi = (sh2 == 0) ? w[wi2]
                        : (w[wi2] >> sh2) | (w[wi2 + 1] << (64 - sh2));
    u32 want = (u32)hi;
    if (mask_crc(crc8b_reg(len, tab)) != want) continue;
    f(i, (i64)len);
  }
}

template <bool EMIT>
__global__ void frame_scan_pass_kernel(const u8* __restrict__ data, i64 N,
                                       i64 pos_start, i64 pos_end,
                                       i64 block_base,
                                       i64* __restrict__ block_data,
                                       i64* __restrict__ cand_pos,
                                       i64* __restrict__ cand_len) {
  __shared__ uint32_t tab[8][256];
  __shared__ unsigned int cnt[256];
  stage_crc_tables(tab);
  const u64* wdata = reinterpret_cast<const u64*>(data);
  i64 c_lo = pos_start / kPosPerLane;
  i64 c_hi = (pos_end + kPosPerLane - 1) / kPosPerLane;
  i64 c = c_lo + (i64)blockIdx.x * blockDim.x + threadIdx.x;
  unsigned int my = 0;
  if (c < c_hi)
    eval_frame_chunk(data, wdata, N, c, pos_start, pos_end, tab,
                     [&](i64, i64) { ++my; });
  cnt[threadIdx.x] = my;
  __syncthreads();
  if (!EMIT) {
    for (int off = blockDim.x / 2; off; off >>= 1) {
      if ((int)threadIdx.x < off) cnt[threadIdx.x] += cnt[threadIdx.x + off];
      __syncthreads();
    }
    if (threadIdx.x == 0) block_data[block_base + blockIdx.x] = (i64)cnt[0];
    return;
  }
  for (int off = 1; off < (int)blockDim.x; off <<= 1) {
    unsigned int v = (int)threadIdx.x >= off ? cnt[threadIdx.x - off] : 0;
    __syncthreads();
    cnt[threadIdx.x] += v;
    __syncthreads();
  }
  i64 slot = block_data[block_base + blockIdx.x] + (i64)(cnt[threadIdx.x] - my);
  if (c < c_hi)
    eval_frame_chunk(data, wdata, N, c, pos_start, pos_end, tab,
                     [&](i64 i, i64 len) {
                       cand_pos[slot] = i;
                       cand_len[slot] = len;
                       ++slot;
                     });
}

__global__ void frame_chain_kernel(const i64* __restrict__ pos,
                                   const i64* __restrict__ len, i64 C,
                                   const i64* __restrict__ carry_in,
                                   i64* __restrict__ carry_out,
                                   i64* __restrict__ off,
                                   i64* __restrict__ broken) {
  for (i64 k = blockIdx.x * (i64)blockDim.x + threadIdx.x; k < C;
       k += (i64)gridDim.x * blockDim.x) {
    i64 p = pos[k];
    i64 want = k == 0 ? *carry_in : pos[k - 1] + 16 + len[k - 1];
    if (p != want) *broken = 1;
    off[k] = p + 12;
    if (k == C - 1) *carry_out = p + 16 + len[k];
  }
}

__global__ void stream_snapshot_kernel(const i64* count, const i64* status,
                                       int nst, const i64* carry, const i64* v,
                                       const i64* b, const i64* l, i64 stride,
                                       int F, i64 r, i64* out) {
  int n = 2 + nst + (v ? 3 * F : 0);
  for (int i = threadIdx.x; i < n; i += blockDim.x) {
    i64 x;
    if (i == 0) {
      x = count ? *count : 0;
    } else if (i <= nst) {
      x = status[i - 1];
    } else if (i == nst + 1) {
      x = carry ? *carry : 0;
    } else {
      int k = i - (nst + 2);
      int plane = k / F;
      int f = k - plane * F;
      const i64* src = plane == 0 ? v : plane == 1 ? b : l;
      x = src[(i64)f * stride + r];
    }
    out[i] = x;
  }
}


struct InferSlot {
  unsigned long long hash;
  long long nameref;
  long long code;
};
static_assert(sizeof(InferSlot) == 24, "layout shared with Python [S,3] i64");

__device__ inline u64 fnv1a64(const u8* s, u64 n) {
  u64 h = 1469598103934665603ull;
  for (u64 i = 0; i < n; ++i) h = (h ^ s[i]) * 1099511628211ull;
  return h ? h : 1ull;
}

constexpr int kLdsInfer = 64;

struct LdsInferSlot {
  unsigned long long hash;
  long long nameref;
  unsigned int code;
};

__device__ inline bool lds_infer_merge(LdsInferSlot* ltab, u64 hash,
                                       long long nameref, int code) {
  int idx = (int)(hash % (u64)kLdsInfer);
  for (int probe = 0; probe < kLdsInfer; ++probe) {
    LdsInferSlot& s = ltab[idx];
    unsigned long long seen =
        atomicCAS(&s.hash, 0ull, (unsigned long long)hash);
    if (seen == 0ull) s.nameref = nameref;
    if (seen == 0ull || seen == hash) {
      atomicMax(&s.code, (unsigned int)code);
      return true;
    }
    idx = (idx + 1) % kLdsInfer;
  }
  return false;
}

__device__ inline bool infer_slot_merge(InferSlot* table, int lo, int half,
                                        u64 hash, long long nameref, int code) {
  int idx = lo + (int)(hash % (u64)half);
  for (int probe = 0; probe < half; ++probe) {
    InferSlot& s = table[idx];
    unsigned long long seen =
        atomicCAS(&s.hash, 0ull, (unsigned long long)hash);
    if (seen == 0ull) s.nameref = nameref;
    if (seen == 0ull || seen == hash) {
      atomicMax((unsigned long long*)&s.code, (unsigned long long)code);
      return true;
    }
    idx = (idx + 1 - lo) % half + lo;
  }
  return false;
}

__device__ inline int32_t infer_features_body_dev(const u8* data, const u8* p,
                                                  const u8* end, bool seq,
                                                  LdsInferSlot* ltab,
                                                  InferSlot* table, int nslots) {
  int half = nslots / 2;
  int lo = seq ? half : 0;
  while (p < end) {
    u64 tag;
    p = read_varint(p, end, &tag);
    if (!p) return ERR_BAD_VARINT;
    u32 fieldno = (u32)(tag >> 3), wt = (u32)(tag & 7);
    if (fieldno != 1 || wt != 2) {
      p = skip_field(p, end, wt);
      if (!p) return ERR_TRUNCATED;
      continue;
    }
    u64 entry_len;
    p = read_varint(p, end, &entry_len);
    if (!p || (u64)(end - p) < entry_len) return ERR_TRUNCATED;
    const u8* ep = p;
    const u8* ee = p + entry_len;
    p = ee;
    const u8* key = nullptr;
    u64 key_len = 0;
    const u8* val = nullptr;
    u64 val_len = 0;
    while (ep < ee) {
      u64 etag;
      ep = read_varint(ep, ee, &etag);
      if (!ep) return ERR_BAD_VARINT;
      u32 efn = (u32)(etag >> 3), ewt = (u32)(etag & 7);
      if (efn == 1 && ewt == 2) {
        ep = read_varint(ep, ee, &key_len);
        if (!ep || (u64)(ee - ep) < key_len) return ERR_TRUNCATED;
        key = ep;
        ep += key_len;
      } else if (efn == 2 && ewt == 2) {
        ep = read_varint(ep, ee, &val_len);
        if (!ep || (u64)(ee - ep) < val_len) return ERR_TRUNCATED;
        val = ep;
        ep += val_len;
      } else {
        ep = skip_field(ep, ee, ewt);
        if (!ep) return ERR_TRUNCATED;
      }
    }
    if (!key) continue;
    int code = 0;
    if (val) {
      if (!seq) {
        int32_t kf = 0;
        i64 nvals = 0, nbytes = 0;
        int32_t rc = scan_feature_body(val, val + val_len, -1, &kf, &nvals, &nbytes);
        if (rc != ERR_OK) return rc;
        if (kf != 0 && nvals > 0) code = (4 - kf) + (nvals > 1 ? 3 : 0);
      } else {
        const u8* lp = val;
        const u8* le = val + val_len;
        int kind_seen = 0;
        while (lp < le) {
          u64 ltag;
          lp = read_varint(lp, le, &ltag);
          if (!lp) return ERR_BAD_VARINT;
          u32 lfn = (u32)(ltag >> 3), lwt = (u32)(ltag & 7);
          if (lfn == 1 && lwt == 2) {
            u64 flen;
            lp = read_varint(lp, le, &flen);
            if (!lp || (u64)(le - lp) < flen) return ERR_TRUNCATED;
            int32_t kf = 0;
            i64 nvals = 0, nbytes = 0;
            int32_t rc = scan_feature_body(lp, lp + flen, -1, &kf, &nvals, &nbytes);
            if (rc != ERR_OK) return rc;
            if (kf) {
              int r = 4 - kf;
              kind_seen = kind_seen > r ? kind_seen : r;
            }
            lp += flen;
          } else {
            lp = skip_field(lp, le, lwt);
            if (!lp) return ERR_TRUNCATED;
          }
        }
        if (kind_seen) code = 6 + kind_seen;
      }
    }
    if (key_len > 0xFFFF) return ERR_NAME_TOO_LONG;
    long long nameref = ((long long)(key - data) << 16) | (long long)key_len;
    u64 hash = fnv1a64(key, key_len);
    if (!lds_infer_merge(ltab, hash, nameref, code) &&
        !infer_slot_merge(table, lo, half, hash, nameref, code))
      return ERR_OVERFLOW;
  }
  return ERR_OK;
}

__global__ void infer_codes_kernel(const u8* __restrict__ data,
                                   const i64* __restrict__ off,
                                   const i64* __restrict__ len, i64 R, int32_t fmt,
                                   InferSlot* __restrict__ table, int nslots,
                                   int32_t* __restrict__ err) {
  __shared__ LdsInferSlot lctx[kLdsInfer];
  __shared__ LdsInferSlot lseq[kLdsInfer];
  for (int i = threadIdx.x; i < kLdsInfer; i += blockDim.x) {
    lctx[i].hash = 0;
    lctx[i].code = 0;
    lseq[i].hash = 0;
    lseq[i].code = 0;
  }
  __syncthreads();
  for (i64 r = blockIdx.x * (i64)blockDim.x + threadIdx.x; r < R;
       r += (i64)gridDim.x * blockDim.x) {
    const u8* p = data + off[r];
    const u8* end = p + len[r];
    while (p < end) {
      u64 tag;
      const u8* np = read_varint(p, end, &tag);
      if (!np) {
        set_err(err, ERR_BAD_VARINT, r);
        break;
      }
      p = np;
      u32 fieldno = (u32)(tag >> 3), wt = (u32)(tag & 7);
      bool is_features = fieldno == 1;
      bool is_fl = (fmt == FMT_SEQUENCE && fieldno == 2);
      if ((is_features || is_fl) && wt == 2) {
        u64 blen;
        p = read_varint(p, end, &blen);
        if (!p || (u64)(end - p) < blen) {
          set_err(err, ERR_TRUNCATED, r);
          break;
        }
        int32_t rc = infer_features_body_dev(data, p, p + blen, is_fl,
                                             is_fl ? lseq : lctx, table, nslots);
        if (rc != ERR_OK) {
          set_err(err, rc, r);
          break;
        }
        p += blen;
      } else {
        p = skip_field(p, end, wt);
        if (!p) {
          set_err(err, ERR_TRUNCATED, r);
          break;
        }
      }
    }
  }
  __syncthreads();
  int half = nslots / 2;
  for (int i = threadIdx.x; i < kLdsInfer; i += blockDim.x) {
    if (lctx[i].hash &&
        !infer_slot_merge(table, 0, half, lctx[i].hash, lctx[i].nameref,
                          (int)lctx[i].code))
      err[0] = ERR_OVERFLOW;
    if (lseq[i].hash &&
        !infer_slot_merge(table, half, half, lseq[i].hash, lseq[i].nameref,
                          (int)lseq[i].code))
      err[0] = ERR_OVERFLOW;
  }
}

__global__ void gather_payloads_kernel(const u8* __restrict__ data,
                                       const i64* __restrict__ off,
                                       const i64* __restrict__ len,
                                       const i64* __restrict__ dst_off, i64 R,
                                       u8* __restrict__ out) {
  for (i64 r = blockIdx.x * (i64)blockDim.x + threadIdx.x; r < R;
       r += (i64)gridDim.x * blockDim.x) {
    const u8* s = data + off[r];
    u8* d = out + dst_off[r];
    i64 n = len[r];
    i64 i = 0;
    for (; i + 8 <= n; i += 8) {
      u64 w;
      __builtin_memcpy(&w, s + i, 8);
      __builtin_memcpy(d + i, &w, 8);
    }
    for (; i < n; ++i) d[i] = s[i];
  }
}


inline int grid_for(i64 n, i64 max_blocks = 0) {
  i64 blocks = (n + kBlock - 1) / kBlock;
  i64 cap = max_blocks > 0 && max_blocks < 8192 ? max_blocks : 8192;
  if (blocks > cap) blocks = cap;
  if (blocks < 1) blocks = 1;
  return (int)blocks;
}

void gpu_crc_verify(uintptr_t data, uintptr_t off, uintptr_t len, i64 R,
                    uintptr_t err_out, uintptr_t stream, i64 avg_bytes) {
  if (avg_bytes > kWaveRecordBytes) {
    hipLaunchKernelGGL(crc_verify_wave_kernel, dim3(grid_for(R * 64)),
                       dim3(kBlock), 0, (hipStream_t)stream, (const u8*)data,
                       (const i64*)off, (const i64*)len, R,
                       (unsigned long long*)err_out);
  } else {
    hipLaunchKernelGGL(crc_verify_kernel, dim3(grid_for(R)), dim3(kBlock), 0,
                       (hipStream_t)stream, (const u8*)data, (const i64*)off,
                       (const i64*)len, R, (unsigned long long*)err_out);
  }
  HIP_CHECK(hipGetLastError());
}

void gpu_scan_records(uintptr_t data, uintptr_t off, uintptr_t len, i64 R,
                      int32_t fmt, uintptr_t schema_blob, int F, uintptr_t stats,
                      uintptr_t err, uintptr_t crc_err, uintptr_t stream,
                      i64 avg_bytes, i64 rec_base, i64 max_blocks,
                      uintptr_t gate) {
  if (R <= 0) return;
  if (avg_bytes > kWaveRecordBytes) {
    hipLaunchKernelGGL(scan_records_wave_kernel,
                       dim3(grid_for(R * 64, max_blocks)), dim3(kBlock), 0,
                       (hipStream_t)stream, (const u8*)data, (const i64*)off,
                       (const i64*)len, R, fmt, (const u8*)schema_blob, F,
                       (FieldStat*)stats, (int32_t*)err,
                       (unsigned long long*)crc_err, rec_base,
                       (const i64*)gate);
  } else {
    hipLaunchKernelGGL(scan_records_kernel, dim3(grid_for(R, max_blocks)),
                       dim3(kBlock), 0, (hipStream_t)stream, (const u8*)data,
                       (const i64*)off, (const i64*)len, R, fmt,
                       (const u8*)schema_blob, F, (FieldStat*)stats,
                       (int32_t*)err, (unsigned long long*)crc_err, rec_base,
                       (const i64*)gate);
  }
  HIP_CHECK(hipGetLastError());
}

void gpu_extract_fields(uintptr_t data, i64 R, int F, uintptr_t stats,
                        py::list metas, uintptr_t meta_dev, uintptr_t err,
                        uintptr_t stream, i64 avg_bytes, i64 r0,
                        i64 max_blocks, bool upload, uintptr_t gate_broken,
                        uintptr_t gate_crc, uintptr_t gate_err,
                        uintptr_t gate_out) {
  if (R <= 0 || F <= 0) return;
  if (upload) {
    std::vector<DevFieldDst> host_metas(F);
    for (int f = 0; f < F; ++f) {
      py::dict d = metas[f].cast<py::dict>();
      auto ptr = [&](const char* k) {
        return d.contains(k) ? d[k].cast<uintptr_t>() : (uintptr_t)0;
      };
      auto cap = [&](const char* k) {
        return d.contains(k) ? d[k].cast<i64>() : (i64)0;
      };
      DevFieldDst& m = host_metas[f];
      m.kind = d["kind"].cast<int32_t>();
      m.is_seq = d["is_seq"].cast<int32_t>();
      m.i64_vals = (i64*)ptr("i64_vals");
      m.f32_vals = (float*)ptr("f32_vals");
      m.bytes_data = (u8*)ptr("bytes_data");
      m.elem_off = (i64*)ptr("elem_off");
      m.sub_off = (i64*)ptr("sub_off");
      m.presence = (u8*)ptr("presence");
      m.val_base = (const i64*)ptr("val_base");
      m.byte_base = (const i64*)ptr("byte_base");
      m.list_base = (const i64*)ptr("list_base");
      m.cap_vals = cap("cap_vals");
      m.cap_bytes = cap("cap_bytes");
      m.cap_elem_off = cap("cap_elem_off");
      m.cap_sub_off = cap("cap_sub_off");
    }
    HIP_CHECK(hipMemcpyAsync((void*)meta_dev, host_metas.data(),
                             sizeof(DevFieldDst) * F, hipMemcpyHostToDevice,
                             (hipStream_t)stream));
  }
  if (gate_out) {
    hipLaunchKernelGGL(extract_gate_kernel, dim3(1), dim3(kBlock), 0,
                       (hipStream_t)stream, (const DevFieldDst*)meta_dev, F,
                       r0 + R, (const i64*)gate_broken,
                       (const unsigned long long*)gate_crc,
                       (const int32_t*)gate_err, (i64*)gate_out);
  }
  if (avg_bytes > kWaveRecordBytes) {
    hipLaunchKernelGGL(extract_fields_wave_kernel,
                       dim3(grid_for(R * F * 64, max_blocks)), dim3(kBlock), 0,
                       (hipStream_t)stream, (const u8*)data, R, F,
                       (const FieldStat*)stats, (const DevFieldDst*)meta_dev,
                       (int32_t*)err, r0, (const i64*)gate_out);
  } else {
    hipLaunchKernelGGL(extract_fields_kernel,
                       dim3(grid_for(R * F, max_blocks)), dim3(kBlock), 0,
                       (hipStream_t)stream, (const u8*)data, R, F,
                       (const FieldStat*)stats, (const DevFieldDst*)meta_dev,
                       (int32_t*)err, r0, (const i64*)gate_out);
  }
  HIP_CHECK(hipGetLastError());
}

struct SnapshotEvent {
  int device = -1;
  hipEvent_t ev = nullptr;
};
thread_local SnapshotEvent snapshot_event;

void gpu_stream_snapshot(uintptr_t count, uintptr_t status, int nst,
                         uintptr_t carry, uintptr_t v, uintptr_t b, uintptr_t l,
                         i64 stride, int F, i64 r, uintptr_t out_host,
                         uintptr_t stream) {
  int dev = 0;
  HIP_CHECK(hipGetDevice(&dev));
  SnapshotEvent& se = snapshot_event;
  if (se.device != dev) {
    if (se.ev) (void)hipEventDestroy(se.ev);
    se.ev = nullptr;
    HIP_CHECK(hipEventCreateWithFlags(&se.ev, hipEventDisableTiming));
    se.device = dev;
  }
  void* out_dev = nullptr;
  HIP_CHECK(hipHostGetDevicePointer(&out_dev, (void*)out_host, 0));
  hipLaunchKernelGGL(stream_snapshot_kernel, dim3(1), dim3(kBlock), 0,
                     (hipStream_t)stream, (const i64*)count,
                     (const i64*)status, nst, (const i64*)carry, (const i64*)v,
                     (const i64*)b, (const i64*)l, stride, v ? F : 0, r,
                     (i64*)out_dev);
  HIP_CHECK(hipGetLastError());
  HIP_CHECK(hipEventRecord(se.ev, (hipStream_t)stream));
}

void gpu_stream_snapshot_wait() {
  SnapshotEvent& se = snapshot_event;
  if (!se.ev)
    throw std::runtime_error("gpu_stream_snapshot_wait: no snapshot taken");
  py::gil_scoped_release rel;
  HIP_CHECK(hipEventSynchronize(se.ev));
}

size_t gpu_devcols_bytes(int F) { return sizeof(FieldColumn) * (size_t)F; }

void fill_devcols(py::list cols, std::vector<FieldColumn>& out) {
  int F = (int)cols.size();
  out.resize(F);
  for (int f = 0; f < F; ++f) {
    py::dict d = cols[f].cast<py::dict>();
    FieldColumn& c = out[f];
    c.kind = d["kind"].cast<int32_t>();
    c.is_seq = d["is_seq"].cast<int32_t>();
    c.presence = (const u8*)d["presence"].cast<uintptr_t>();
    c.row_off = (const i64*)d["row_off"].cast<uintptr_t>();
    c.list_off = (const i64*)d["list_off"].cast<uintptr_t>();
    c.sub_off = (const i64*)d["sub_off"].cast<uintptr_t>();
    c.elem_off = (const i64*)d["elem_off"].cast<uintptr_t>();
    c.bytes_data = (const u8*)d["values_bytes"].cast<uintptr_t>();
    c.i64_vals = (const i64*)d["values_i64"].cast<uintptr_t>();
    c.f32_vals = (const float*)d["values_f32"].cast<uintptr_t>();
  }
}

void gpu_size_records(py::list cols, uintptr_t cols_dev, uintptr_t schema_blob,
                      int32_t fmt, i64 R, uintptr_t psize, uintptr_t stream) {
  static thread_local std::vector<FieldColumn> host_cols;
  fill_devcols(cols, host_cols);
  HIP_CHECK(hipMemcpyAsync((void*)cols_dev, host_cols.data(),
                           sizeof(FieldColumn) * host_cols.size(),
                           hipMemcpyHostToDevice, (hipStream_t)stream));
  hipLaunchKernelGGL(size_records_kernel, dim3(grid_for(R)), dim3(kBlock), 0,
                     (hipStream_t)stream, (const FieldColumn*)cols_dev,
                     (const u8*)schema_blob, fmt, R, (i64*)psize);
  HIP_CHECK(hipGetLastError());
}

void gpu_emit_records(uintptr_t cols_dev, uintptr_t schema_blob, int32_t fmt,
                      i64 r0, i64 R, uintptr_t frame_off, uintptr_t file,
                      uintptr_t err, uintptr_t stream, i64 avg_bytes) {
  if (avg_bytes > kWaveRecordBytes) {
    hipLaunchKernelGGL(emit_records_wave_kernel, dim3(grid_for((R - r0) * 64)),
                       dim3(kBlock), 0, (hipStream_t)stream,
                       (const FieldColumn*)cols_dev, (const u8*)schema_blob,
                       fmt, r0, R, (const i64*)frame_off, (u8*)file,
                       (int32_t*)err);
  } else {
    hipLaunchKernelGGL(emit_records_kernel, dim3(grid_for(R - r0)),
                       dim3(kBlock), 0, (hipStream_t)stream,
                       (const FieldColumn*)cols_dev, (const u8*)schema_blob,
                       fmt, r0, R, (const i64*)frame_off, (u8*)file,
                       (int32_t*)err);
  }
  HIP_CHECK(hipGetLastError());
}

void gpu_frame_bytes(uintptr_t src, uintptr_t elem_off, uintptr_t frame_off, i64 R,
                     uintptr_t file, uintptr_t stream, i64 avg_bytes) {
  if (avg_bytes > kWaveRecordBytes) {
    hipLaunchKernelGGL(frame_bytes_wave_kernel, dim3(grid_for(R * 64)),
                       dim3(kBlock), 0, (hipStream_t)stream, (const u8*)src,
                       (const i64*)elem_off, (const i64*)frame_off, R,
                       (u8*)file);
  } else {
    hipLaunchKernelGGL(frame_bytes_kernel, dim3(grid_for(R)), dim3(kBlock), 0,
                       (hipStream_t)stream, (const u8*)src, (const i64*)elem_off,
                       (const i64*)frame_off, R, (u8*)file);
  }
  HIP_CHECK(hipGetLastError());
}

i64 gpu_frame_scan_blocks(i64 pos_start, i64 pos_end) {
  i64 c_lo = pos_start / kPosPerLane;
  i64 c_hi = (pos_end + kPosPerLane - 1) / kPosPerLane;
  i64 n = c_hi - c_lo;
  return (n + kBlock - 1) / kBlock;
}

void gpu_frame_scan_count(uintptr_t data, i64 N, i64 pos_start, i64 pos_end,
                          i64 block_base, uintptr_t block_counts,
                          uintptr_t stream) {
  i64 B = gpu_frame_scan_blocks(pos_start, pos_end);
  if (B <= 0) return;
  hipLaunchKernelGGL(frame_scan_pass_kernel<false>, dim3((uint32_t)B),
                     dim3(kBlock), 0, (hipStream_t)stream, (const u8*)data, N,
                     pos_start, pos_end, block_base, (i64*)block_counts,
                     nullptr, nullptr);
  HIP_CHECK(hipGetLastError());
}

void gpu_frame_scan_emit(uintptr_t data, i64 N, i64 pos_start, i64 pos_end,
                         i64 block_base, uintptr_t block_off,
                         uintptr_t cand_pos, uintptr_t cand_len,
                         uintptr_t stream) {
  i64 B = gpu_frame_scan_blocks(pos_start, pos_end);
  if (B <= 0) return;
  hipLaunchKernelGGL(frame_scan_pass_kernel<true>, dim3((uint32_t)B),
                     dim3(kBlock), 0, (hipStream_t)stream, (const u8*)data, N,
                     pos_start, pos_end, block_base, (i64*)block_off,
                     (i64*)cand_pos, (i64*)cand_len);
  HIP_CHECK(hipGetLastError());
}

void gpu_frame_chain(uintptr_t pos, uintptr_t len, i64 C, uintptr_t carry_in,
                     uintptr_t carry_out, uintptr_t off, uintptr_t broken,
                     uintptr_t stream) {
  if (C <= 0) return;
  hipLaunchKernelGGL(frame_chain_kernel, dim3(grid_for(C)), dim3(kBlock), 0,
                     (hipStream_t)stream, (const i64*)pos, (const i64*)len, C,
                     (const i64*)carry_in, (i64*)carry_out, (i64*)off,
                     (i64*)broken);
  HIP_CHECK(hipGetLastError());
}

void gpu_infer_codes(uintptr_t data, uintptr_t off, uintptr_t len, i64 R,
                     int32_t fmt, uintptr_t table, int nslots, uintptr_t err,
                     uintptr_t stream) {
  hipLaunchKernelGGL(infer_codes_kernel, dim3(grid_for(R)), dim3(kBlock), 0,
                     (hipStream_t)stream, (const u8*)data, (const i64*)off,
                     (const i64*)len, R, fmt, (InferSlot*)table, nslots,
                     (int32_t*)err);
  HIP_CHECK(hipGetLastError());
}

void gpu_gather_payloads(uintptr_t data, uintptr_t off, uintptr_t len,
                         uintptr_t dst_off, i64 R, uintptr_t out,
                         uintptr_t stream, i64 avg_bytes) {
  if (avg_bytes > kWaveRecordBytes) {
    hipLaunchKernelGGL(gather_payloads_wave_kernel, dim3(grid_for(R * 64)),
                       dim3(kBlock), 0, (hipStream_t)stream, (const u8*)data,
                       (const i64*)off, (const i64*)len, (const i64*)dst_off,
                       R, (u8*)out);
  } else {
    hipLaunchKernelGGL(gather_payloads_kernel, dim3(grid_for(R)), dim3(kBlock),
                       0, (hipStream_t)stream, (const u8*)data,
                       (const i64*)off, (const i64*)len, (const i64*)dst_off,
                       R, (u8*)out);
  }
  HIP_CHECK(hipGetLastError());
}


struct StridedLoadI64 {
  const i64* p;
  i64 stride;
  __host__ __device__ i64 operator()(i64 i) const { return p[i * stride]; }
};

size_t gpu_scan_temp_bytes(i64 n) {
  size_t bytes = 0;
  auto it = rocprim::make_transform_iterator(
      rocprim::make_counting_iterator<i64>(0), StridedLoadI64{nullptr, 1});
  (void)rocprim::inclusive_scan(nullptr, bytes, it, (i64*)nullptr, (size_t)n,
                                rocprim::plus<i64>());
  return bytes;
}


struct Seg3 {
  i64 v0, v1, v2;
  u32 flag;
};

struct Seg3Combine {
  __host__ __device__ Seg3 operator()(const Seg3& a, const Seg3& b) const {
    if (b.flag) return b;
    return Seg3{a.v0 + b.v0, a.v1 + b.v1, a.v2 + b.v2, a.flag};
  }
};

struct Seg3Load {
  const i64* stats;
  i64 n;
  int F;
  i64 r0;
  i64 stride;
  const i64* b0;
  const i64* b1;
  const i64* b2;
  __host__ __device__ Seg3 operator()(i64 idx) const {
    i64 f = idx / n;
    i64 q = idx - f * n;
    const i64* st = stats + ((r0 + q) * F + f) * 6;
    if (q != 0) return Seg3{st[2], st[3], st[4], 0u};
    i64 at = f * stride + r0;
    return Seg3{st[2] + b0[at], st[3] + b1[at], st[4] + b2[at], 1u};
  }
};

struct Seg3OutRef {
  i64* o0;
  i64* o1;
  i64* o2;
  __host__ __device__ Seg3OutRef& operator=(const Seg3& v) {
    *o0 = v.v0;
    *o1 = v.v1;
    *o2 = v.v2;
    return *this;
  }
};

struct Seg3OutIt {
  using value_type = Seg3;
  using reference = Seg3OutRef;
  using pointer = Seg3OutRef*;
  using difference_type = i64;
  using iterator_category = std::random_access_iterator_tag;
  i64* b0;
  i64* b1;
  i64* b2;
  i64 n;
  i64 r0;
  i64 stride;
  i64 pos;
  __host__ __device__ Seg3OutRef operator*() const { return (*this)[0]; }
  __host__ __device__ Seg3OutRef operator[](i64 k) const {
    i64 idx = pos + k;
    i64 f = idx / n;
    i64 q = idx - f * n;
    i64 at = f * stride + r0 + q + 1;
    return Seg3OutRef{b0 + at, b1 + at, b2 + at};
  }
  __host__ __device__ Seg3OutIt operator+(i64 k) const {
    return Seg3OutIt{b0, b1, b2, n, r0, stride, pos + k};
  }
  __host__ __device__ Seg3OutIt& operator+=(i64 k) {
    pos += k;
    return *this;
  }
  __host__ __device__ Seg3OutIt& operator++() {
    ++pos;
    return *this;
  }
};

size_t gpu_stat_scan_temp_bytes(i64 R, int F) {
  size_t bytes = 0;
  auto in = rocprim::make_transform_iterator(
      rocprim::make_counting_iterator<i64>(0),
      Seg3Load{nullptr, R, F, 0, R + 1, nullptr, nullptr, nullptr});
  Seg3OutIt out{nullptr, nullptr, nullptr, R, 0, R + 1, 0};
  (void)rocprim::inclusive_scan(nullptr, bytes, in, out, (size_t)(R * F),
                                Seg3Combine());
  return bytes;
}

void gpu_stat_scans(uintptr_t temp, size_t temp_bytes, uintptr_t stats, i64 R,
                    int F, uintptr_t val_base, uintptr_t byte_base,
                    uintptr_t list_base, uintptr_t stream, i64 r0, i64 r1,
                    i64 stride) {
  auto s = (hipStream_t)stream;
  if (r1 < 0) r1 = R;
  if (stride <= 0) stride = R + 1;
  if (r0 < 0 || r1 > R || r1 >= stride)
    throw std::runtime_error("gpu_stat_scans: range outside the planes");
  i64 n = r1 - r0;
  if (n <= 0 || F <= 0) return;
  auto in = rocprim::make_transform_iterator(
      rocprim::make_counting_iterator<i64>(0),
      Seg3Load{(const i64*)stats, n, F, r0, stride, (const i64*)val_base,
               (const i64*)byte_base, (const i64*)list_base});
  Seg3OutIt out{(i64*)val_base, (i64*)byte_base, (i64*)list_base, n, r0,
                stride, 0};
  size_t tb = temp_bytes;
  HIP_CHECK(rocprim::inclusive_scan((void*)temp, tb, in, out,
                                    (size_t)(n * F), Seg3Combine(), s));
}

void gpu_excl_sum_strided(uintptr_t temp, size_t temp_bytes, uintptr_t in,
                          i64 stride, uintptr_t out, i64 n, uintptr_t stream) {
  auto s = (hipStream_t)stream;
  HIP_CHECK(hipMemsetAsync((void*)out, 0, sizeof(i64), s));
  if (n <= 0) return;
  auto it = rocprim::make_transform_iterator(
      rocprim::make_counting_iterator<i64>(0), StridedLoadI64{(const i64*)in, stride});
  size_t tb = temp_bytes;
  hipError_t e = rocprim::inclusive_scan((void*)temp, tb, it, (i64*)out + 1,
                                         (size_t)n, rocprim::plus<i64>(), s);
  HIP_CHECK(e);
}


struct MappedFile {
  void* ptr = nullptr;
  size_t n = 0;
  dev_t dev = 0;
  ino_t ino = 0;
  bool pinned = false;
  bool writable = false;
};

std::map<std::string, MappedFile> g_mmap_cache;
std::mutex g_mmap_mu;
size_t g_mmap_bytes = 0;
constexpr size_t kMmapCacheCap = 4ull << 30;

void drop_mapping_locked(const std::string& key) {
  auto it = g_mmap_cache.find(key);
  if (it == g_mmap_cache.end()) return;
  if (it->second.pinned) {
    (void)hipDeviceSynchronize();
    (void)hipHostUnregister(it->second.ptr);
  }
  munmap(it->second.ptr, it->second.n);
  g_mmap_bytes -= it->second.n;
  g_mmap_cache.erase(it);
}

void sweep_stale_locked() {
  for (auto it = g_mmap_cache.begin(); it != g_mmap_cache.end();) {
    struct stat st {};
    bool live = stat(it->first.c_str(), &st) == 0 &&
                st.st_dev == it->second.dev && st.st_ino == it->second.ino &&
                (size_t)st.st_size >= it->second.n;
    if (live) {
      ++it;
    } else {
      auto key = it->first;
      ++it;
      drop_mapping_locked(key);
    }
  }
}

py::tuple file_mmap_pinned(const std::string& path, i64 n, bool writable) {
  if (n <= 0) return py::make_tuple((uintptr_t)0, true);
  std::lock_guard<std::mutex> lk(g_mmap_mu);
  sweep_stale_locked();
  int flags = writable ? (O_RDWR | O_CREAT) : O_RDWR;
  int fd = ::open(path.c_str(), flags, 0644);
  bool rdonly = false;
  if (fd < 0 && !writable) {
    fd = ::open(path.c_str(), O_RDONLY);
    rdonly = true;
  }
  if (fd < 0)
    throw std::runtime_error("open failed: " + path + ": " + strerror(errno));
  struct stat st {};
  if (fstat(fd, &st) != 0) {
    ::close(fd);
    throw std::runtime_error("stat failed: " + path);
  }
  auto it = g_mmap_cache.find(path);
  if (it != g_mmap_cache.end()) {
    MappedFile& m = it->second;
    if (m.dev == st.st_dev && m.ino == st.st_ino && m.n == (size_t)n &&
        st.st_size >= (off_t)n && (m.writable || !writable)) {
      ::close(fd);
      return py::make_tuple((uintptr_t)m.ptr, m.pinned);
    }
    drop_mapping_locked(path);
  }
  if (writable && st.st_size != (off_t)n && ftruncate(fd, (off_t)n) != 0) {
    int e = errno;
    ::close(fd);
    throw std::runtime_error("ftruncate failed: " + path + ": " + strerror(e));
  }
  if (!writable && st.st_size < (off_t)n) {
    ::close(fd);
    throw std::runtime_error("short file: " + path);
  }
  while (g_mmap_bytes + (size_t)n > kMmapCacheCap && !g_mmap_cache.empty())
    drop_mapping_locked(g_mmap_cache.begin()->first);
  int prot = PROT_READ | ((writable || !rdonly) ? PROT_WRITE : 0);
  void* p = mmap(nullptr, (size_t)n, prot, MAP_SHARED, fd, 0);
  ::close(fd);
  if (p == MAP_FAILED)
    throw std::runtime_error("mmap failed: " + path + ": " + strerror(errno));
  bool pinned = hipHostRegister(p, (size_t)n, hipHostRegisterDefault) == hipSuccess;
  if (!pinned) (void)hipGetLastError();
  MappedFile m{p, (size_t)n, st.st_dev, st.st_ino, pinned,
               writable || !rdonly};
  g_mmap_cache[path] = m;
  g_mmap_bytes += (size_t)n;
  return py::make_tuple((uintptr_t)p, pinned);
}

void file_mmap_drop(const std::string& path) {
  std::lock_guard<std::mutex> lk(g_mmap_mu);
  drop_mapping_locked(path);
}

void file_mmap_sync(const std::string& path) {
  std::lock_guard<std::mutex> lk(g_mmap_mu);
  auto it = g_mmap_cache.find(path);
  if (it != g_mmap_cache.end() && it->second.ptr) {
    if (msync(it->second.ptr, it->second.n, MS_SYNC) != 0)
      throw std::runtime_error("msync failed: " + path + ": " +
                               strerror(errno));
  }
  int fd = ::open(path.c_str(), O_RDONLY);
  if (fd >= 0) {
    (void)fsync(fd);
    ::close(fd);
  }
}


void gpu_memcpy_d2h(uintptr_t dst, uintptr_t src, i64 n, uintptr_t stream) {
  HIP_CHECK(hipMemcpyAsync((void*)dst, (const void*)src, (size_t)n,
                           hipMemcpyDeviceToHost, (hipStream_t)stream));
}

void gpu_memcpy_h2d(uintptr_t dst, uintptr_t src, i64 n, uintptr_t stream) {
  HIP_CHECK(hipMemcpyAsync((void*)dst, (const void*)src, (size_t)n,
                           hipMemcpyHostToDevice, (hipStream_t)stream));
}

}

void register_gpu(py::module_& m) {
  m.def("gpu_device_count", []() {
    int n = 0;
    hipError_t e = hipGetDeviceCount(&n);
    return (e == hipSuccess) ? n : -static_cast<int>(e);
  });
  m.def("gpu_crc_verify", &gpu_crc_verify, py::arg("data"), py::arg("off"),
        py::arg("len"), py::arg("R"), py::arg("err_out"), py::arg("stream"),
        py::arg("avg_bytes") = 0);
  m.def("gpu_scan_records", &gpu_scan_records, py::arg("data"), py::arg("off"),
        py::arg("len"), py::arg("R"), py::arg("fmt"), py::arg("schema_blob"),
        py::arg("F"), py::arg("stats"), py::arg("err"), py::arg("crc_err"),
        py::arg("stream"), py::arg("avg_bytes") = 0, py::arg("rec_base") = 0,
        py::arg("max_blocks") = 0, py::arg("gate") = 0);
  m.def("gpu_extract_fields", &gpu_extract_fields, py::arg("data"),
        py::arg("R"), py::arg("F"), py::arg("stats"), py::arg("metas"),
        py::arg("meta_dev"), py::arg("err"), py::arg("stream"),
        py::arg("avg_bytes") = 0, py::arg("r0") = 0,
        py::arg("max_blocks") = 0, py::arg("upload") = true,
        py::arg("gate_broken") = 0, py::arg("gate_crc") = 0,
        py::arg("gate_err") = 0, py::arg("gate_out") = 0);
  m.def("gpu_stream_snapshot", &gpu_stream_snapshot, py::arg("count"),
        py::arg("status"), py::arg("nst"), py::arg("carry"), py::arg("v"),
        py::arg("b"), py::arg("l"), py::arg("stride"), py::arg("F"),
        py::arg("r"), py::arg("out_host"), py::arg("stream"));
  m.def("gpu_stream_snapshot_wait", &gpu_stream_snapshot_wait);
  m.def("gpu_size_records", &gpu_size_records);
  m.def("gpu_emit_records", &gpu_emit_records, py::arg("cols_dev"),
        py::arg("schema_blob"), py::arg("fmt"), py::arg("r0"), py::arg("R"),
        py::arg("frame_off"), py::arg("file"), py::arg("err"),
        py::arg("stream"), py::arg("avg_bytes") = 0);
  m.def("gpu_frame_bytes", &gpu_frame_bytes, py::arg("src"),
        py::arg("elem_off"), py::arg("frame_off"), py::arg("R"),
        py::arg("file"), py::arg("stream"), py::arg("avg_bytes") = 0);
  m.def("gpu_frame_scan_blocks", &gpu_frame_scan_blocks);
  m.def("gpu_frame_scan_count", &gpu_frame_scan_count);
  m.def("gpu_frame_scan_emit", &gpu_frame_scan_emit);
  m.def("gpu_frame_chain", &gpu_frame_chain);
  m.def("gpu_gather_payloads", &gpu_gather_payloads, py::arg("data"),
        py::arg("off"), py::arg("len"), py::arg("dst_off"), py::arg("R"),
        py::arg("out"), py::arg("stream"), py::arg("avg_bytes") = 0);
  m.def("gpu_infer_codes", &gpu_infer_codes);
  m.def("gpu_scan_temp_bytes", &gpu_scan_temp_bytes);
  m.def("gpu_stat_scan_temp_bytes", &gpu_stat_scan_temp_bytes);
  m.def("gpu_stat_scans", &gpu_stat_scans, py::arg("temp"),
        py::arg("temp_bytes"), py::arg("stats"), py::arg("R"), py::arg("F"),
        py::arg("val_base"), py::arg("byte_base"), py::arg("list_base"),
        py::arg("stream"), py::arg("r0") = 0, py::arg("r1") = -1,
        py::arg("stride") = 0);
  m.def("gpu_excl_sum_strided", &gpu_excl_sum_strided);
  m.def("file_mmap_pinned", &file_mmap_pinned, py::arg("path"), py::arg("n"),
        py::arg("writable"));
  m.def("file_mmap_drop", &file_mmap_drop);
  m.def("file_mmap_sync", &file_mmap_sync);
  m.def("gpu_memcpy_d2h", &gpu_memcpy_d2h);
  m.def("gpu_memcpy_h2d", &gpu_memcpy_h2d);
  m.def("gpu_devcols_bytes", &gpu_devcols_bytes);
  m.def("gpu_devmeta_bytes", []() { return sizeof(DevFieldDst); });
  m.def("gpu_fieldstat_words", []() { return sizeof(FieldStat) / 8; });
}
```

### spark_tfrecord_amd/engine/gpu.py

```python

from __future__ import annotations

import os
import threading
import warnings
from typing import List, NamedTuple, Optional

import numpy as np
import torch

from .. import _native
from . import stream_plan
from ..columnar import RecordBatch, WireColumn, schema_blob, wire_fields
from ..schema import KIND_BYTES, KIND_FLOAT, KIND_INT64, StructType, is_sequence_field, wire_kind_of

FMT = {"Example": _native.FMT_EXAMPLE, "SequenceExample": _native.FMT_SEQUENCE}


def _stream() -> int:
    return torch.cuda.current_stream().cuda_stream


def _dev(x, dtype, device="cuda") -> torch.Tensor:
    if isinstance(x, torch.Tensor):
        return x.to(device=device, dtype=dtype).contiguous()
    arr = np.ascontiguousarray(x)
    with warnings.catch_warnings():
        warnings.simplefilter("ignore", UserWarning)
        return torch.as_tensor(arr, dtype=dtype).to(device)


def check_native():
    if not getattr(_native, "HAS_GPU_KERNELS", False):
        raise RuntimeError("_native was built without HIP kernels; rebuild "
                           "with build_native.py before using the GPU engine")



_pinned_tls = threading.local()


def pinned_buffer(tag: str, nbytes: int) -> torch.Tensor:
    pool = getattr(_pinned_tls, "pool", None)
    if pool is None:
        pool = _pinned_tls.pool = {}
    buf = pool.get(tag)
    if buf is None or buf.numel() < nbytes:
        cap = max(nbytes, int((buf.numel() if buf is not None else 1 << 20) * 1.5))
        buf = torch.empty(cap, dtype=torch.uint8, pin_memory=True)
        pool[tag] = buf
    return buf


_CHUNK = 64 << 20
_READ_SLICE = int(os.environ.get("TFREC_READ_SLICE", 32 << 20))
_SPLIT_SLICES = os.environ.get("TFREC_READ_SPLIT", "1") != "0"
_WRITE_SLICES = int(os.environ.get("TFREC_WRITE_SLICES", 8))
_STREAM_DECODE = os.environ.get("TFREC_STREAM_DECODE", "1") != "0"
_STREAM_HEADROOM = float(os.environ.get("TFREC_STREAM_HEADROOM", 1.125))
_STREAM_EXTRACT = os.environ.get("TFREC_STREAM_EXTRACT", "1") != "0"
_SYNC_WRITES = os.environ.get("TFREC_SYNC", "1") != "0"


def read_file_to_device(path: str, device="cuda") -> torch.Tensor:
    n = os.path.getsize(path)
    dev_t = torch.empty(max(n, 1), dtype=torch.uint8, device=device)[:n]
    if n:
        ptr, pinned = _native.file_mmap_pinned(path, n, False)
        if pinned:
            _multi_dma(dev_t.data_ptr(), ptr, n, _native.gpu_memcpy_h2d,
                       after_main=True)
            return dev_t
    return _read_file_staged(path, dev_t)


_copy_streams: Optional[list] = None


def _dma_streams() -> list:
    global _copy_streams
    if _copy_streams is None:
        _copy_streams = [torch.cuda.Stream() for _ in range(2)]
    return _copy_streams


def _multi_dma(dst: int, src: int, n: int, fn, after_main: bool):
    streams = _dma_streams()
    main = torch.cuda.current_stream()
    k = min(len(streams), max(1, n // (16 << 20)))
    span = (n + k - 1) // k
    for i in range(k):
        o = i * span
        m = min(span, n - o)
        s = streams[i]
        s.wait_stream(main)
        fn(dst + o, src + o, m, s.cuda_stream)
    if after_main:
        for i in range(k):
            main.wait_stream(streams[i])
    else:
        for i in range(k):
            streams[i].synchronize()


def _read_file_staged(path: str, dev: torch.Tensor) -> torch.Tensor:
    n = dev.numel()
    buf = pinned_buffer("fread", min(n, 2 * _CHUNK) or 1)
    ev = [torch.cuda.Event(), torch.cuda.Event()]
    fd = os.open(path, os.O_RDONLY)
    try:
        pos = 0
        which = 0
        while pos < n:
            m = min(_CHUNK, n - pos)
            ev[which].synchronize()
            _native.pread_parallel(fd, buf.data_ptr() + which * _CHUNK, m, pos)
            dev[pos:pos + m].copy_(buf[which * _CHUNK:which * _CHUNK + m],
                                   non_blocking=True)
            ev[which].record()
            pos += m
            which ^= 1 if n > _CHUNK else 0
    finally:
        os.close(fd)
    return dev


def _upload_files(dst: torch.Tensor, entries):
    main = torch.cuda.current_stream()
    streams = _dma_streams()
    used = []
    for k, (path, nbytes, off) in enumerate(entries):
        if not nbytes:
            continue
        ptr, pinned = _native.file_mmap_pinned(path, nbytes, False)
        if pinned:
            st = streams[k % len(streams)]
            st.wait_stream(main)
            _native.gpu_memcpy_h2d(dst.data_ptr() + off, ptr, nbytes,
                                   st.cuda_stream)
            used.append(st)
        else:
            _read_file_staged(path, dst[off:off + nbytes])
    for st in set(used):
        main.wait_stream(st)


def _upload_group(items, device):
    sizes = [os.path.getsize(it[0]) for it in items]
    offs = [0]
    for n in sizes[:-1]:
        offs.append(offs[-1] + n)
    total = sum(sizes)
    comp = torch.empty(max(total, 1), dtype=torch.uint8, device=device)[:total]
    _upload_files(comp, [(it[0], n, o) for it, n, o in zip(items, sizes, offs)])
    return comp, offs, sizes


def device_to_file(img: torch.Tensor, path: str):
    n = img.numel()
    if n == 0:
        open(path, "wb").close()
        return
    ptr, pinned = _native.file_mmap_pinned(path, n, True)
    if pinned:
        _multi_dma(ptr, img.data_ptr(), n, _native.gpu_memcpy_d2h,
                   after_main=False)
        if _SYNC_WRITES:
            _native.file_mmap_sync(path)
        return
    _write_file_staged(img, path)


def _write_file_staged(img: torch.Tensor, path: str):
    n = img.numel()
    buf = pinned_buffer("fwrite", min(n, 2 * _CHUNK) or 1)
    ev = [torch.cuda.Event(), torch.cuda.Event()]
    fd = os.open(path, os.O_RDWR | os.O_CREAT, 0o644)
    try:
        pos = 0
        which = 0
        m0 = min(_CHUNK, n)
        if n:
            buf[0:m0].copy_(img[0:m0], non_blocking=True)
            ev[0].record()
        while pos < n:
            m = min(_CHUNK, n - pos)
            nxt = pos + m
            nwhich = which ^ (1 if n > _CHUNK else 0)
            if nxt < n:
                m2 = min(_CHUNK, n - nxt)
                buf[nwhich * _CHUNK:nwhich * _CHUNK + m2].copy_(
                    img[nxt:nxt + m2], non_blocking=True)
                ev[nwhich].record()
            ev[which].synchronize()
            _native.pwrite_parallel(fd, buf.data_ptr() + which * _CHUNK, m, pos)
            pos = nxt
            which = nwhich
        os.ftruncate(fd, n)
        if _SYNC_WRITES:
            os.fsync(fd)
    finally:
        os.close(fd)



_scan_ws = {}


def _scan_workspace(n: int, device) -> torch.Tensor:
    key = (device.index if hasattr(device, "index") else 0)
    need = _native.gpu_scan_temp_bytes(max(n, 1))
    ws = _scan_ws.get(key)
    if ws is None or ws.numel() < need:
        ws = torch.empty(int(need * 2), dtype=torch.uint8, device=device)
        _scan_ws[key] = ws
    return ws


def _excl_sum_into(out_ptr: int, in_ptr: int, stride: int, n: int, device):
    ws = _scan_workspace(n, device)
    _native.gpu_excl_sum_strided(ws.data_ptr(), ws.numel(), in_ptr, stride,
                                 out_ptr, n, _stream())


def _stat_scan_workspace(R: int, F: int, device) -> torch.Tensor:
    key = ("stat", device.index if hasattr(device, "index") else 0)
    need = _native.gpu_stat_scan_temp_bytes(R, F)
    ws = _scan_ws.get(key)
    if ws is None or ws.numel() < need:
        ws = torch.empty(int(need * 2) or 1, dtype=torch.uint8, device=device)
        _scan_ws[key] = ws
    return ws


def excl_sum(t: torch.Tensor) -> torch.Tensor:
    n = t.numel()
    out = torch.empty(n + 1, dtype=torch.int64, device=t.device)
    _excl_sum_into(out.data_ptr(), t.data_ptr(), 1, n, t.device)
    return out


def device_to_bytes(img: torch.Tensor) -> bytes:
    n = img.numel()
    buf = pinned_buffer("d2h", n)
    buf[:n].copy_(img, non_blocking=True)
    torch.cuda.synchronize()
    return buf.numpy()[:n].tobytes()


def device_to_pinned_view(img: torch.Tensor, tag: str = "d2h_img") -> np.ndarray:
    n = img.numel()
    buf = pinned_buffer(tag, n)
    buf[:n].copy_(img, non_blocking=True)
    torch.cuda.synchronize()
    return buf.numpy()[:n]



def scan_frames_device(data: torch.Tensor):
    check_native()
    N = data.numel()
    device = data.device
    if N == 0:
        z = torch.zeros(0, dtype=torch.int64, device=device)
        return z, z.clone()
    B = _native.gpu_frame_scan_blocks(0, N)
    block_counts = torch.empty(B, dtype=torch.int64, device=device)
    _native.gpu_frame_scan_count(data.data_ptr(), N, 0, N, 0,
                                 block_counts.data_ptr(), _stream())
    off, lens, _ = _emit_and_chain(data, [(0, N)], block_counts, N)
    return off, lens


def _emit_and_chain(data, ranges, block_counts, N):
    device = data.device
    block_off = excl_sum(block_counts)
    C = int(block_off[-1].item())
    if C == 0:
        raise RuntimeError("corrupt TFRecord: no valid frame header found")
    pos = torch.empty(C, dtype=torch.int64, device=device)
    lens = torch.empty(C, dtype=torch.int64, device=device)
    base = 0
    for s, e in ranges:
        _native.gpu_frame_scan_emit(data.data_ptr(), N, s, e, base,
                                    block_off.data_ptr(), pos.data_ptr(),
                                    lens.data_ptr(), _stream())
        base += _native.gpu_frame_scan_blocks(s, e)
    expect_next = pos + 16 + lens
    ok = bool(((pos[0] == 0) & (expect_next[-1] == N)
               & (expect_next[:-1] == pos[1:]).all()).item())
    if not ok:
        pos_h = pos.cpu().numpy()
        len_h = lens.cpu().numpy()
        keep = []
        cur = 0
        pmap = {int(p): i for i, p in enumerate(pos_h)}
        while cur < N:
            i = pmap.get(cur)
            if i is None:
                raise RuntimeError(
                    f"corrupt TFRecord: broken frame chain at offset {cur}")
            keep.append(i)
            cur = int(pos_h[i] + 16 + len_h[i])
        sel = torch.as_tensor(np.asarray(keep, np.int64), device=device)
        pos = pos[sel]
        lens = lens[sel]
    return pos + 12, lens, ok



def crc_verify_device(data: torch.Tensor, off: torch.Tensor, lens: torch.Tensor,
                      avg_bytes: int = 0):
    R = off.numel()
    if R == 0:
        return
    if not avg_bytes:
        avg_bytes = max(0, (data.numel() // R) - 16)
    err = torch.full((1,), -1, dtype=torch.int64, device=data.device)
    _native.gpu_crc_verify(data.data_ptr(), off.data_ptr(), lens.data_ptr(), R,
                           err.data_ptr(), _stream(), avg_bytes)
    bad = int(err.item())
    if bad != -1:
        raise RuntimeError(
            f"corrupt TFRecord: bad CRC in record {bad - 1 if bad > 0 else bad}")


def decode_device(data: torch.Tensor, off: torch.Tensor, lens: torch.Tensor,
                  schema: StructType, record_type: str,
                  verify_crc: bool = True) -> RecordBatch:
    check_native()
    device = data.device
    R = off.numel()
    fields = wire_fields(schema)
    F = len(fields)
    if verify_crc and record_type == "ByteArray":
        crc_verify_device(data, off, lens)

    if record_type == "ByteArray":
        dst_off = excl_sum(lens.contiguous())
        total = int(dst_off[-1].item())
        out = torch.empty(total, dtype=torch.uint8, device=device)
        if R:
            _native.gpu_gather_payloads(data.data_ptr(), off.data_ptr(),
                                        lens.data_ptr(), dst_off.data_ptr(), R,
                                        out.data_ptr(), _stream(), total // R)
        col = WireColumn(kind=KIND_BYTES, is_seq=False,
                         presence=torch.ones(R, dtype=torch.uint8, device=device),
                         row_off=torch.arange(R + 1, dtype=torch.int64, device=device),
                         values=out, elem_off=dst_off)
        return RecordBatch(schema, [col], R)

    if F == 0 or R == 0:
        cols = [WireColumn(wire_kind_of(f.dataType), is_sequence_field(f.dataType),
                           torch.zeros(R, dtype=torch.uint8, device=device),
                           torch.zeros(R + 1, dtype=torch.int64, device=device),
                           torch.zeros(0, dtype=torch.int64, device=device))
                for f in fields]
        return RecordBatch(schema, cols, R)

    blob = _schema_blob_device(schema, device)
    stats = torch.empty((R, F, 6), dtype=torch.int64, device=device)
    err = torch.zeros(2, dtype=torch.int32, device=device)
    crc_err = None
    fuse_crc = verify_crc
    if fuse_crc:
        crc_err = torch.full((1,), -1, dtype=torch.int64, device=device)
    avg_bytes = max(0, (data.numel() // R) - 16) if R else 0
    _native.gpu_scan_records(data.data_ptr(), off.data_ptr(), lens.data_ptr(),
                             R, FMT[record_type], blob.data_ptr(), F,
                             stats.data_ptr(), err.data_ptr(),
                             crc_err.data_ptr() if fuse_crc else 0,
                             _stream(), avg_bytes)

    val_base = torch.empty((F, R + 1), dtype=torch.int64, device=device)
    byte_base = torch.empty((F, R + 1), dtype=torch.int64, device=device)
    list_base = torch.empty((F, R + 1), dtype=torch.int64, device=device)
    val_base[:, 0] = 0
    byte_base[:, 0] = 0
    list_base[:, 0] = 0
    ws = _stat_scan_workspace(R, F, device)
    _native.gpu_stat_scans(ws.data_ptr(), ws.numel(), stats.data_ptr(), R, F,
                           val_base.data_ptr(), byte_base.data_ptr(),
                           list_base.data_ptr(), _stream())
    totals = torch.stack([val_base[:, -1], byte_base[:, -1], list_base[:, -1]])
    totals_h = totals.cpu()
    _raise_scan_errors(int(crc_err.item()) if fuse_crc else -1,
                       int(err[0].item()), int(err[1].item()))
    vals = _FieldValues(fields, data.numel(), device)
    vals.reserve(totals_h, data.numel())
    presence = torch.empty((F, R), dtype=torch.uint8, device=device)
    vals.extract(data, stats, (val_base, byte_base, list_base), presence, 0, R,
                 _MetaTable(F, device), err, avg_bytes)
    vals.confirm(totals_h)
    cols = vals.columns(presence, val_base, list_base, R)
    if int(err[0].item()) != 0:
        _raise_extract_error(int(err[0].item()), int(err[1].item()))
    return RecordBatch(schema, cols, R)


_schema_blobs = {}


def _schema_blob_device(schema: StructType, device) -> torch.Tensor:
    raw = bytes(schema_blob(schema))
    key = (raw, str(torch.device(device)))
    blob = _schema_blobs.get(key)
    if blob is None:
        if len(_schema_blobs) >= 64:
            _schema_blobs.clear()
        blob = torch.frombuffer(bytearray(raw), dtype=torch.uint8).to(device)
        _schema_blobs[key] = blob
    return blob


def _raise_scan_errors(crc_bad: int, rc: int, rec1: int):
    if crc_bad != -1:
        raise RuntimeError(f"corrupt TFRecord: bad CRC in record {crc_bad - 1}")
    if rc != 0:
        rec = rec1 - 1
        where = f" in record {rec}" if rec >= 0 else ""
        raise RuntimeError(f"TFRecord decode failed{where} (native error "
                           f"{rc}; kind mismatch or malformed record)")


def _raise_extract_error(rc: int, rec1: int):
    rec = rec1 - 1
    where = f" (record {rec})" if rec >= 0 else ""
    raise RuntimeError(f"TFRecord decode failed in value extraction"
                       f"{where} (native error {rc})")


class _MetaTable:

    def __init__(self, F: int, device):
        self.dev = torch.empty(F * _native.gpu_devmeta_bytes(),
                               dtype=torch.uint8, device=device)
        self.last = None

    def changed(self, metas) -> bool:
        key = [tuple(m.items()) for m in metas]
        if key == self.last:
            return False
        self.last = key
        return True


class _FieldValues:

    _BUFS = {"i64_vals": (torch.int64, 0, 0, lambda k, seq: k == KIND_INT64),
             "f32_vals": (torch.float32, 0, 0, lambda k, seq: k == KIND_FLOAT),
             "elem_off": (torch.int64, 0, 1, lambda k, seq: k == KIND_BYTES),
             "bytes_data": (torch.uint8, 1, 0, lambda k, seq: k == KIND_BYTES),
             "sub_off": (torch.int64, 2, 1, lambda k, seq: seq)}

    def __init__(self, fields, total_bytes: int, device):
        self.total_bytes = total_bytes
        self.device = device
        self.kinds = [wire_kind_of(f.dataType) for f in fields]
        self.seqs = [is_sequence_field(f.dataType) for f in fields]
        self.filled = [[0] * len(fields) for _ in range(3)]
        self.bufs = [{k: torch.empty(0, dtype=d, device=device)
                      for k, (d, _, _, _) in self._BUFS.items()} for _ in fields]

    def reserve(self, totals, bytes_seen: int):
        for i, bufs in enumerate(self.bufs):
            for name, (_, dim, extra, fills) in self._BUFS.items():
                if not fills(self.kinds[i], self.seqs[i]):
                    continue
                need = int(totals[dim][i]) + extra
                old = bufs[name]
                cap = stream_plan.grown_capacity(
                    old.numel(), need, bytes_seen, self.total_bytes,
                    _STREAM_HEADROOM, min_unit=1)
                if cap == old.numel():
                    continue
                new = torch.empty(cap, dtype=old.dtype, device=self.device)
                k = min(self.filled[dim][i] + extra, old.numel())
                if k:
                    new[:k].copy_(old[:k])
                if old.numel():
                    last_read["regrows"] = last_read.get("regrows", 0) + 1
                bufs[name] = new

    def confirm(self, totals):
        self.filled = [[int(totals[d][i]) for i in range(len(self.bufs))]
                       for d in range(3)]

    def extract(self, data, stats, planes, presence, r0: int, r1: int,
                meta: _MetaTable, err, avg_bytes: int, gate=None):
        v, b, l = planes
        metas = []
        for i, bufs in enumerate(self.bufs):
            vals = bufs["i64_vals" if self.kinds[i] == KIND_INT64 else "f32_vals"]
            metas.append({
                "kind": self.kinds[i], "is_seq": 1 if self.seqs[i] else 0,
                **{name: t.data_ptr() for name, t in bufs.items()},
                "presence": presence[i].data_ptr(),
                "val_base": v[i].data_ptr(),
                "byte_base": b[i].data_ptr(),
                "list_base": l[i].data_ptr() if self.seqs[i] else 0,
                "cap_vals": vals.numel(),
                "cap_bytes": bufs["bytes_data"].numel(),
                "cap_elem_off": bufs["elem_off"].numel(),
                "cap_sub_off": bufs["sub_off"].numel(),
            })
        g_broken, g_crc, g_err, g_out = gate or (0, 0, 0, 0)
        _native.gpu_extract_fields(data.data_ptr(), r1 - r0, len(self.bufs),
                                   stats.data_ptr(), metas,
                                   meta.dev.data_ptr(), err.data_ptr(),
                                   _stream(), avg_bytes, r0=r0,
                                   upload=meta.changed(metas),
                                   gate_broken=g_broken, gate_crc=g_crc,
                                   gate_err=g_err, gate_out=g_out)

    def columns(self, presence, val_base, list_base, R: int) -> List[WireColumn]:
        cols = []
        for i, bufs in enumerate(self.bufs):
            kind, seq = self.kinds[i], self.seqs[i]
            nv, nb, nl = (self.filled[d][i] for d in range(3))
            values = (bufs["i64_vals"][:nv] if kind == KIND_INT64 else
                      bufs["f32_vals"][:nv] if kind == KIND_FLOAT else
                      bufs["bytes_data"][:nb])
            cols.append(WireColumn(
                kind, seq, presence[i][:R], val_base[i][:R + 1], values,
                bufs["elem_off"][:nv + 1] if kind == KIND_BYTES else None,
                list_base[i][:R + 1] if seq else None,
                bufs["sub_off"][:nl + 1] if seq else None))
        return cols


def decode_buffer_device(data_np: np.ndarray, schema: StructType, record_type: str,
                         verify_crc: bool = True, device="cuda") -> RecordBatch:
    data_np = np.ascontiguousarray(data_np, np.uint8)
    n = data_np.size
    stage = pinned_buffer("h2d", n)
    stage.numpy()[:n] = data_np
    data = torch.empty(n, dtype=torch.uint8, device=device)
    data.copy_(stage[:n], non_blocking=True)
    off, lens = scan_frames_device(data)
    return decode_device(data, off, lens, schema, record_type, verify_crc)


def read_file_to_batch(path: str, schema: StructType, record_type: str,
                       verify_crc: bool = True, device="cuda") -> RecordBatch:
    return read_file_to_batch_pipelined(path, schema, record_type, verify_crc,
                                        device)



def _col_ptrs(col: WireColumn) -> dict:
    def p(t):
        return t.data_ptr() if isinstance(t, torch.Tensor) and t.numel() else 0

    return {
        "kind": col.kind, "is_seq": 1 if col.is_seq else 0,
        "presence": p(col.presence), "row_off": p(col.row_off),
        "list_off": p(col.list_off) if col.list_off is not None else 0,
        "sub_off": p(col.sub_off) if col.sub_off is not None else 0,
        "elem_off": p(col.elem_off) if col.elem_off is not None else 0,
        "values_bytes": p(col.values) if col.kind == KIND_BYTES else 0,
        "values_i64": p(col.values) if col.kind == KIND_INT64 else 0,
        "values_f32": p(col.values) if col.kind == KIND_FLOAT else 0,
    }


def _check_emit_err(err: torch.Tensor):
    if int(err[0].item()) != 0:
        rec = int(err[1].item()) - 1
        where = f" in record {rec}" if rec >= 0 else ""
        raise RuntimeError(f"TFRecord encode failed: size/emit mismatch{where}")


def _size_records(batch: RecordBatch, record_type: str, device):
    blob = _schema_blob_device(batch.schema, device)
    col_dicts = [_col_ptrs(c) for c in batch.columns]
    cols_dev = torch.empty(_native.gpu_devcols_bytes(len(col_dicts)),
                           dtype=torch.uint8, device=device)
    psize = torch.empty(batch.num_rows, dtype=torch.int64, device=device)
    _native.gpu_size_records(col_dicts, cols_dev.data_ptr(), blob.data_ptr(),
                             FMT[record_type], batch.num_rows,
                             psize.data_ptr(), _stream())
    return cols_dev, blob, psize, excl_sum(psize)


def encode_device(batch: RecordBatch, record_type: str) -> torch.Tensor:
    check_native()
    R = batch.num_rows
    device = batch.columns[0].presence.device if batch.columns else torch.device("cuda")
    if record_type == "ByteArray":
        col = batch.columns[0]
        lens = col.elem_off[1:] - col.elem_off[:-1]
        frame_off = excl_sum((lens + 16).contiguous())
        total = int(frame_off[-1].item())
        file = torch.empty(total, dtype=torch.uint8, device=device)
        if R:
            _native.gpu_frame_bytes(col.values.data_ptr(), col.elem_off.data_ptr(),
                                    frame_off.data_ptr(), R, file.data_ptr(),
                                    _stream(), (total // R) - 16)
        return file

    cols_dev, blob, _, frame_off = _size_records(batch, record_type, device)
    total = int(frame_off[-1].item())
    file = torch.empty(total, dtype=torch.uint8, device=device)
    err = torch.zeros(2, dtype=torch.int32, device=device)
    _native.gpu_emit_records(cols_dev.data_ptr(), blob.data_ptr(),
                             FMT[record_type], 0, R, frame_off.data_ptr(),
                             file.data_ptr(), err.data_ptr(), _stream(),
                             total // max(R, 1))
    _check_emit_err(err)
    return file


def write_batch_to_file(batch: RecordBatch, path: str,
                        record_type: str = "Example",
                        slices: Optional[int] = None) -> int:
    check_native()
    R = batch.num_rows
    if record_type == "ByteArray" or R == 0:
        img = encode_device(batch, record_type)
        device_to_file(img, path)
        return img.numel()
    device = batch.columns[0].presence.device
    cols_dev, blob, _, frame_off = _size_records(batch, record_type, device)
    S = max(1, min(slices if slices is not None else _WRITE_SLICES, R))
    ridx = [R * s // S for s in range(S + 1)]
    bounds = frame_off[ridx].cpu()
    total = int(bounds[-1])
    file = torch.empty(total, dtype=torch.uint8, device=device)
    err = torch.zeros(2, dtype=torch.int32, device=device)
    ptr, pinned = _native.file_mmap_pinned(path, total, True)
    if not pinned:
        _native.gpu_emit_records(cols_dev.data_ptr(), blob.data_ptr(),
                                 FMT[record_type], 0, R, frame_off.data_ptr(),
                                 file.data_ptr(), err.data_ptr(), _stream(),
                                 total // R)
        _check_emit_err(err)
        _write_file_staged(file, path)
        return total
    main = torch.cuda.current_stream()
    streams = _dma_streams()
    for s in range(S):
        _native.gpu_emit_records(cols_dev.data_ptr(), blob.data_ptr(),
                                 FMT[record_type], ridx[s], ridx[s + 1],
                                 frame_off.data_ptr(), file.data_ptr(),
                                 err.data_ptr(), _stream(), total // R)
        b0, b1 = int(bounds[s]), int(bounds[s + 1])
        if b1 > b0:
            w = streams[s % len(streams)]
            w.wait_stream(main)
            _native.gpu_memcpy_d2h(ptr + b0, file.data_ptr() + b0, b1 - b0,
                                   w.cuda_stream)
    for w in streams:
        w.synchronize()
    if _SYNC_WRITES:
        _native.file_mmap_sync(path)
    _check_emit_err(err)
    return total


last_read = {}

_ST_BROKEN, _ST_CRC, _ST_ERR, _ST_XERR, _ST_NOEXT, _ST_CARRY = 0, 1, 2, 3, 4, 5


class _StreamStatus:

    def __init__(self, max_chains: int, device):
        self.words = torch.zeros(_ST_CARRY + 1 + max_chains, dtype=torch.int64,
                                 device=device)
        self.words[_ST_CRC] = -1
        self.err = self.words[_ST_ERR:_ST_ERR + 1].view(torch.int32)
        self.xerr = self.words[_ST_XERR:_ST_XERR + 1].view(torch.int32)

    def addr(self, word: int) -> int:
        return self.words.data_ptr() + word * 8

    def carry_addr(self, k: int) -> int:
        return self.addr(_ST_CARRY + k)


class _Snapshot:

    def __init__(self, h: np.ndarray, F: int):
        self.count = int(h[0])
        st = h[1:1 + _ST_CARRY]
        self.broken = int(st[_ST_BROKEN]) != 0
        pair = st[_ST_ERR:_ST_ERR + 1].view(np.int32)
        self.scan_error = (int(st[_ST_CRC]), int(pair[0]), int(pair[1]))
        xpair = st[_ST_XERR:_ST_XERR + 1].view(np.int32)
        self.xerr = (int(xpair[0]), int(xpair[1]))
        self.refused = int(st[_ST_NOEXT]) != 0
        self.chain_end = int(h[1 + _ST_CARRY])
        self.totals = h[2 + _ST_CARRY:].reshape(3, F) if F else None


class _StreamRows:

    def __init__(self, total_bytes: int, F: int, device):
        self.total_bytes = total_bytes
        self.F = F
        self.device = device
        self.cap = 0
        self.pos = self.lens = self.off = self.stats = None
        self.planes = None
        self.presence = None

    def _alloc(self, cap: int):
        i64 = dict(dtype=torch.int64, device=self.device)
        planes = presence = None
        if self.F:
            planes = [torch.empty((self.F, cap + 1), **i64) for _ in range(3)]
            for t in planes:
                t[:, 0] = 0
            presence = torch.empty((self.F, cap), dtype=torch.uint8,
                                   device=self.device)
        return (torch.empty(cap, **i64), torch.empty(cap, **i64),
                torch.empty(cap, **i64),
                torch.empty((cap, self.F, 6), **i64) if self.F else None,
                planes, presence)

    def cand_ptrs(self, c: int):
        return (self.pos.data_ptr() + c * 8, self.lens.data_ptr() + c * 8,
                self.off.data_ptr() + c * 8)

    def row_ptrs(self, r: int):
        return (self.off.data_ptr() + r * 8, self.lens.data_ptr() + r * 8,
                self.stats.data_ptr() + r * self.F * 48)

    def scan_stats(self, r0: int, r1: int):
        ws = _stat_scan_workspace(r1 - r0, self.F, self.device)
        v, b, l = self.planes
        _native.gpu_stat_scans(ws.data_ptr(), ws.numel(),
                               self.stats.data_ptr(), r1, self.F, v.data_ptr(),
                               b.data_ptr(), l.data_ptr(), _stream(), r0=r0,
                               r1=r1, stride=self.cap + 1)

    def reserve(self, need: int, n_cand: int, n_scanned: int, bytes_seen: int):
        cap = stream_plan.grown_capacity(self.cap, need, bytes_seen,
                                         self.total_bytes, _STREAM_HEADROOM)
        if cap == self.cap:
            return
        pos, lens, off, stats, planes, presence = self._alloc(cap)
        if n_cand:
            pos[:n_cand].copy_(self.pos[:n_cand])
            lens[:n_cand].copy_(self.lens[:n_cand])
            off[:n_cand].copy_(self.off[:n_cand])
        if n_scanned and stats is not None:
            stats[:n_scanned].copy_(self.stats[:n_scanned])
            for new, old in zip(planes, self.planes):
                new[:, :n_scanned + 1].copy_(old[:, :n_scanned + 1])
            presence[:, :n_scanned].copy_(self.presence[:, :n_scanned])
        self.pos, self.lens, self.off, self.stats = pos, lens, off, stats
        self.planes, self.presence = planes, presence
        if self.cap:
            last_read["regrows"] = last_read.get("regrows", 0) + 1
        self.cap = cap


class _StreamedRead:

    def __init__(self, data: torch.Tensor, nslices: int, schema: StructType,
                 record_type: str, verify_crc: bool):
        device = data.device
        self.data = data
        self.n = data.numel()
        self.schema = schema
        self.record_type = record_type
        self.verify_crc = verify_crc
        fields = wire_fields(schema)
        F = self.F = len(fields)
        self.do_scan = record_type != "ByteArray" and F > 0
        self.status = _StreamStatus(nslices, device)
        self.rows = _StreamRows(self.n, F if self.do_scan else 0, device)
        if self.do_scan:
            self.blob = _schema_blob_device(schema, device)
            self.vals = _FieldValues(fields, self.n, device)
            self.meta = _MetaTable(F, device)
        self.C = 0
        self.nchain = 0
        self.r_done = 0
        self.x_done = 0
        self.x_pending = None
        self.sized = False
        self.bytes_done = 0
        self.clean = True
        self.avg_bytes = None

    def _snapshot(self, count_ptr: int, r: int) -> _Snapshot:
        F = self.F if self.rows.planes is not None else 0
        n = 2 + _ST_CARRY + 3 * F
        buf = pinned_buffer("snapshot", n * 8)
        v, b, l = ([t.data_ptr() for t in self.rows.planes] if F
                   else (0, 0, 0))
        _native.gpu_stream_snapshot(
            count_ptr, self.status.addr(0), _ST_CARRY,
            self.status.carry_addr(self.nchain), v, b, l, self.rows.cap + 1,
            F, r, buf.data_ptr(), _stream())
        _native.gpu_stream_snapshot_wait()
        last_read["host_waits"] = last_read.get("host_waits", 0) + 1
        return _Snapshot(buf.numpy()[:n * 8].view(np.int64).copy(), F)

    def _settle(self, snap: _Snapshot):
        crc_bad, rc, _ = snap.scan_error
        if crc_bad != -1 or rc != 0:
            self.clean = False
        if self.x_pending is None:
            return
        assert self.x_pending == self.r_done
        if not snap.refused:
            self.x_done = self.x_pending
            self.vals.confirm(snap.totals)
        elif self.clean:
            self.vals.reserve(snap.totals, self.bytes_done)
        self.x_pending = None

    def _extract(self, r1: int, gated: bool):
        st = self.status
        gate = (st.addr(_ST_BROKEN), st.addr(_ST_CRC), st.addr(_ST_ERR),
                st.addr(_ST_NOEXT)) if gated else None
        self.vals.extract(self.data, self.rows.stats, self.rows.planes,
                          self.rows.presence, self.x_done, r1, self.meta,
                          st.xerr, self.avg_bytes, gate)

    def step(self, p: stream_plan.SlicePlan, counts: Optional[torch.Tensor],
             last: bool) -> bool:
        count_ptr = 0
        if counts is not None:
            block_off = excl_sum(counts)
            count_ptr = block_off.data_ptr() + counts.numel() * 8
        snap = self._snapshot(count_ptr, self.r_done)
        if snap.broken:
            return False
        if self.do_scan:
            self._settle(snap)
        c_s = snap.count
        if c_s:
            self.rows.reserve(self.C + c_s, self.C, self.r_done, p.scan_hi)
            pos, lens, off = self.rows.cand_ptrs(self.C)
            _native.gpu_frame_scan_emit(self.data.data_ptr(), self.n,
                                        p.scan_lo, p.scan_hi, 0,
                                        block_off.data_ptr(), pos, lens,
                                        _stream())
            _native.gpu_frame_chain(pos, lens, c_s,
                                    self.status.carry_addr(self.nchain),
                                    self.status.carry_addr(self.nchain + 1),
                                    off, self.status.addr(_ST_BROKEN),
                                    _stream())
            self.nchain += 1
            self.C += c_s
        if not self.do_scan:
            return True
        avail = stream_plan.launchable_records(self.C, last)
        r0 = self.r_done
        if avail > r0:
            if self.avg_bytes is None:
                self.avg_bytes = max(0, p.scan_hi // avail - 16)
            off, lens, stats = self.rows.row_ptrs(r0)
            _native.gpu_scan_records(
                self.data.data_ptr(), off, lens, avail - r0,
                FMT[self.record_type], self.blob.data_ptr(), self.F, stats,
                self.status.err.data_ptr(),
                self.status.addr(_ST_CRC) if self.verify_crc else 0, _stream(),
                self.avg_bytes, rec_base=r0,
                gate=self.status.addr(_ST_BROKEN))
            self.rows.scan_stats(r0, avail)
            self.r_done = avail
        self.bytes_done = p.scan_hi
        if not _STREAM_EXTRACT or not self.clean or avail <= self.x_done:
            return True
        if not self.sized:
            if last:
                return True
            snap = self._snapshot(0, avail)
            if snap.broken:
                return False
            self._settle(snap)
            if not self.clean:
                return True
            self.vals.reserve(snap.totals, p.scan_hi)
            self.sized = True
        self._extract(avail, gated=True)
        self.x_pending = avail
        return True

    def finish(self) -> Optional[RecordBatch]:
        R, n = self.C, self.n
        if R == 0:
            return None
        snap = self._snapshot(0, R)
        if snap.broken or snap.chain_end != n:
            return None
        if not self.do_scan:
            return decode_device(self.data, self.rows.off[:R],
                                 self.rows.lens[:R], self.schema,
                                 self.record_type, self.verify_crc)
        crc_bad, rc, rec1 = snap.scan_error
        _raise_scan_errors(crc_bad if self.verify_crc else -1, rc, rec1)
        if not self.clean:
            raise RuntimeError("streamed decode: scan error lost")
        self._settle(snap)
        xerr = snap.xerr
        if self.x_done < R:
            self.vals.reserve(snap.totals, n)
            self._extract(R, gated=False)
            self.x_done = R
            self.vals.confirm(snap.totals)
            xerr = self._snapshot(0, R).xerr
        val_base, _, list_base = self.rows.planes
        cols = self.vals.columns(self.rows.presence, val_base, list_base, R)
        if xerr[0] != 0:
            _raise_extract_error(*xerr)
        return RecordBatch(self.schema, cols, R)


def _issue_h2d_slices(data: torch.Tensor, ptr: int, plan) -> list:
    main = torch.cuda.current_stream()
    streams = _dma_streams()
    for st in streams:
        st.wait_stream(main)
    events = []
    for s, p in enumerate(plan):
        half = (p.b1 - p.b0) // 2 if _SPLIT_SLICES and len(streams) > 1 else 0
        parts = ([(p.b0, p.b0 + half, 0), (p.b0 + half, p.b1, 1)] if half
                 else [(p.b0, p.b1, s % len(streams))])
        evs = []
        for lo, hi, k in parts:
            st = streams[k]
            _native.gpu_memcpy_h2d(data.data_ptr() + lo, ptr + lo, hi - lo,
                                   st.cuda_stream)
            ev = torch.cuda.Event()
            ev.record(st)
            evs.append(ev)
        events.append(evs)
    for st in streams:
        data.record_stream(st)
    return events


def _scan_blocks(p: stream_plan.SlicePlan) -> int:
    if p.scan_hi <= p.scan_lo:
        return 0
    return int(_native.gpu_frame_scan_blocks(p.scan_lo, p.scan_hi))


def _count_slice(data, p, evs, block_counts, base: int) -> int:
    main = torch.cuda.current_stream()
    for ev in evs:
        main.wait_event(ev)
    nb = _scan_blocks(p)
    if nb:
        _native.gpu_frame_scan_count(data.data_ptr(), data.numel(), p.scan_lo,
                                     p.scan_hi, base, block_counts.data_ptr(),
                                     _stream())
    return nb


def _read_unstreamed(data, plan, block_counts, events, first: int,
                     schema: StructType, record_type: str,
                     verify_crc: bool) -> RecordBatch:
    last_read["path"] = "fallback" if _STREAM_DECODE else "unstreamed"
    base = sum(_scan_blocks(p) for p in plan[:first])
    for p, evs in zip(plan[first:], events[first:]):
        base += _count_slice(data, p, evs, block_counts, base)
    ranges = [(p.scan_lo, p.scan_hi) for p in plan if p.scan_hi > p.scan_lo]
    off, lens, _ = _emit_and_chain(data, ranges, block_counts, data.numel())
    return decode_device(data, off, lens, schema, record_type, verify_crc)


def read_file_to_batch_pipelined(path: str, schema: StructType, record_type: str,
                                 verify_crc: bool = True,
                                 device="cuda") -> RecordBatch:
    check_native()
    n = os.path.getsize(path)
    if n == 0:
        z = torch.zeros(0, dtype=torch.int64, device=device)
        return decode_device(torch.zeros(0, dtype=torch.uint8, device=device),
                             z, z.clone(), schema, record_type, verify_crc)
    ptr, pinned = _native.file_mmap_pinned(path, n, False)
    if not pinned:
        data = _read_file_staged(path, torch.empty(n, dtype=torch.uint8,
                                                   device=device))
        off, lens = scan_frames_device(data)
        return decode_device(data, off, lens, schema, record_type, verify_crc)
    data = torch.empty(n, dtype=torch.uint8, device=device)
    plan = stream_plan.plan_slices(n, _READ_SLICE)
    S = len(plan)
    block_counts = torch.empty(max(sum(_scan_blocks(p) for p in plan), 1),
                               dtype=torch.int64, device=data.device)
    events = _issue_h2d_slices(data, ptr, plan)
    last_read.update(path="streamed", slices=S, regrows=0, host_waits=0)
    unstreamed = (data, plan, block_counts, events)
    decode = (schema, record_type, verify_crc)
    if not _STREAM_DECODE:
        return _read_unstreamed(*unstreamed, 0, *decode)

    rd = _StreamedRead(data, S, *decode)
    base = 0
    for s, p in enumerate(plan):
        nb = _count_slice(data, p, events[s], block_counts, base)
        counts = block_counts[base:base + nb] if nb else None
        base += nb
        if not rd.step(p, counts, last=s == S - 1):
            return _read_unstreamed(*unstreamed, s + 1, *decode)
    batch = rd.finish()
    if batch is None:
        return _read_unstreamed(*unstreamed, S, *decode)
    return batch


def gz_device_meta(path: str):
    from ..io import paths as P

    if not getattr(_native, "HAS_GPU_KERNELS", False):
        return None
    return P.parse_gz_segments_file(path)


def _device_inflate_group(data: torch.Tensor, gz_items, device) -> bool:
    comp, comp_offs, _ = _upload_group(gz_items, device)
    in_off = []
    in_len = []
    out_off = []
    out_len = []
    for (p, meta, out_base), coff in zip(gz_items, comp_offs):
        body_off, segs, _crc, _isize = meta
        so = coff + body_off
        uo = out_base
        for c, u in segs:
            in_off.append(so)
            in_len.append(c)
            out_off.append(uo)
            out_len.append(u)
            so += c
            uo += u
    meta_np = np.array([in_off, in_len, out_off, out_len], np.int64)
    force = os.environ.get("TFREC_INFLATE_STREAMS", "")
    spw_lit = 2
    if force in ("1", "2", "4"):
        spw_lit = int(force)
        lit = np.full(meta_np.shape[1], spw_lit > 1)
    else:
        lit = meta_np[1] >= (0.85 * np.maximum(meta_np[3], 1))
    err = torch.full((1,), -1, dtype=torch.int64, device=device)
    for mask, spw in ((lit, spw_lit), (~lit, 1)):
        k = int(mask.sum())
        if k == 0:
            continue
        idx = np.nonzero(mask)[0]
        if spw == 2 and k > 2:
            idx = idx[np.argsort(-meta_np[3, idx], kind="stable")]
        sub = torch.as_tensor(
            np.ascontiguousarray(meta_np[:, idx])).to(device)
        _native.gpu_inflate_segments(
            comp.data_ptr(), sub[0].data_ptr(), sub[1].data_ptr(),
            sub[2].data_ptr(), sub[3].data_ptr(), k,
            data.data_ptr(), err.data_ptr(), _stream(), spw)
    return int(err.item()) == -1


class DeviceDecompressRejected(Exception):

    def __init__(self, paths, message):
        super().__init__(message)
        self.paths = list(paths)


class ForeignGzipRejected(DeviceDecompressRejected):

    def __init__(self, paths):
        super().__init__(
            paths, f"device inflate rejected {len(paths)} gzip file(s)")


class SnappyRejected(DeviceDecompressRejected):

    def __init__(self, paths):
        super().__init__(
            paths, f"device snappy decode rejected {len(paths)} file(s)")


last_foreign: list = []

_FOREIGN_DEFAULT_CHUNK = 32 << 10
_FOREIGN_MAX_FILES = 4096


def _foreign_chunk_bytes(chunk_bytes: Optional[int] = None) -> int:
    if chunk_bytes is None:
        chunk_bytes = os.environ.get("TFREC_GZ_FOREIGN_CHUNK",
                                     _FOREIGN_DEFAULT_CHUNK)
    chunk_bytes = int(chunk_bytes)
    if chunk_bytes < 64:
        raise ValueError(
            f"foreign gzip chunk stride must be >= 64 bytes, got {chunk_bytes}")
    return chunk_bytes


def foreign_gz_meta(path: str):
    if not getattr(_native, "HAS_GPU_KERNELS", False):
        return None
    try:
        size = os.path.getsize(path)
        if size < 18:
            return None
        with open(path, "rb") as f:
            head = f.read(min(size, 128 << 10))
            f.seek(size - 8)
            trailer = f.read(8)
    except OSError:
        return None
    return _foreign_gz_parse(head, trailer, size)


def _foreign_gz_parse(head: bytes, trailer: bytes, size: int):
    if head[:3] != b"\x1f\x8b\x08" or head[3] & 0xE0:
        return None
    flg = head[3]
    pos = 10
    if flg & 0x04:
        if pos + 2 > len(head):
            return None
        pos += 2 + int.from_bytes(head[pos:pos + 2], "little")
    for bit in (0x08, 0x10):
        if flg & bit:
            end = head.find(b"\x00", pos)
            if end < 0:
                return None
            pos = end + 1
    if flg & 0x02:
        pos += 2
    body_len = size - 8 - pos
    crc = int.from_bytes(trailer[:4], "little")
    isize = int.from_bytes(trailer[4:], "little")
    if (pos > len(head) or body_len <= 0 or body_len >= (1 << 32)
            or isize == 0 or isize > body_len * 1032 + 64):
        return None
    return pos, body_len, crc, isize


def _device_inflate_foreign_group(data: torch.Tensor, items, device,
                                  chunk_bytes: Optional[int] = None):
    chunk = _foreign_chunk_bytes(chunk_bytes)
    CC, FC, RC = (_native.FOREIGN_CHUNK_COLS, _native.FOREIGN_FILE_COLS,
                  _native.FOREIGN_RES_COLS)
    piece = int(_native.FOREIGN_CRC_PIECE)
    ok_all = []
    del last_foreign[:]
    for lo in range(0, len(items), _FOREIGN_MAX_FILES):
        part = items[lo:lo + _FOREIGN_MAX_FILES]
        nfile = len(part)
        comp, comp_offs, comp_sizes = _upload_group(part, device)
        ft = np.zeros((nfile, FC), np.int64)
        chunk0 = sym0 = piece0 = 0
        for k, (p, meta, out_base) in enumerate(part):
            body_off, body_len, crc, isize = meta
            if (body_off + body_len + 8 != comp_sizes[k] or out_base < 0
                    or out_base + isize > data.numel()):
                raise ValueError(f"foreign gzip extents changed under the "
                                 f"read: {p}")
            nchunk = -(-body_len // chunk)
            ft[k, :9] = (comp_offs[k] + body_off, body_len, isize, crc, chunk0,
                         nchunk, out_base, sym0, piece0)
            chunk0 += nchunk
            sym0 += isize
            piece0 += -(-isize // piece)
        ct = np.zeros((chunk0, CC), np.int64)
        ct[:, 0] = np.repeat(np.arange(nfile), ft[:, 5])
        ct[:, 1] = -1
        ct[:, 4] = -2
        ct[:, 6] = -1
        res = np.zeros((nfile, RC), np.int64)
        res[:, 0] = -1
        ft_d = torch.as_tensor(ft).to(device)
        ct_d = torch.as_tensor(ct).to(device)
        res_d = torch.as_tensor(res).to(device)
        sym = torch.empty(sym0, dtype=torch.int16, device=device)
        piece_crc = torch.empty(piece0, dtype=torch.int32, device=device)
        max_pieces = int((-(-ft[:, 2] // piece)).max())
        _native.gpu_inflate_foreign(
            comp.data_ptr(), ft_d.data_ptr(), ct_d.data_ptr(),
            res_d.data_ptr(), piece_crc.data_ptr(), sym.data_ptr(),
            data.data_ptr(), nfile, chunk0, max_pieces, chunk, _stream())
        out = res_d.cpu().numpy()
        for k, (p, _, _) in enumerate(part):
            ok_all.append(int(out[k, 0]) == -1)
            last_foreign.append((p, int(out[k, 1]), int(out[k, 3]),
                                 int(out[k, 0])))
    return ok_all


last_snappy: list = []

SNAPPY_MAX_CHUNK_RAW = 1 << 20


def snappy_on_device() -> bool:
    val = os.environ.get("TFREC_SNAPPY", "device").lower()
    if val not in ("device", "host"):
        raise ValueError(
            f"Unsupported TFREC_SNAPPY {val!r} (expected 'device' or 'host')")
    return val == "device"


def snappy_device_meta(path: str):
    import mmap

    from ..io import paths as P

    if not getattr(_native, "HAS_GPU_KERNELS", False) or not snappy_on_device():
        return None
    try:
        size = os.path.getsize(path)
        if size == 0:
            return np.zeros((0, 4), np.int64), 0
        with open(path, "rb") as f:
            with mmap.mmap(f.fileno(), 0, access=mmap.ACCESS_READ) as mm:
                chunks, total = P.snappy_walk(mm, path)
    except (OSError, ValueError):
        return None
    ext = np.array(chunks, np.int64).reshape(-1, 4)
    if ext.shape[0] and int(ext[:, 3].max()) > SNAPPY_MAX_CHUNK_RAW:
        return None
    return ext, total


def _snappy_max_waves(device) -> int:
    return 16 * torch.cuda.get_device_properties(device).multi_processor_count


def _device_unsnap_group(data: torch.Tensor, items, device):
    del last_snappy[:]
    nfile = len(items)
    comp, comp_offs, comp_sizes = _upload_group(items, device)
    tables = []
    chunk0 = np.zeros(nfile, np.int64)
    nchunk = 0
    for k, (p, meta, out_base) in enumerate(items):
        ext, total = meta
        chunk0[k] = nchunk
        if ext.shape[0]:
            t = np.empty((ext.shape[0], 5), np.int64)
            t[:, 0] = ext[:, 0] + comp_offs[k]
            t[:, 1] = ext[:, 1]
            t[:, 2] = ext[:, 2] + out_base
            t[:, 3] = ext[:, 3]
            t[:, 4] = k
            if (ext[:, 0].min() < 0 or ext[:, 1].min() < 0
                    or (ext[:, 0] + ext[:, 1]).max() > comp_sizes[k]
                    or ext[:, 2].min() < 0 or ext[:, 3].min() < 0
                    or (ext[:, 2] + ext[:, 3]).max() > total
                    or out_base < 0 or out_base + total > data.numel()):
                raise ValueError(f"snappy extents changed under the read: {p}")
            tables.append(t)
            nchunk += ext.shape[0]
    err = np.full(nfile, -1, np.int64)
    if nchunk:
        assert int(_native.SNAPPY_CHUNK_COLS) == 5
        ct_d = torch.as_tensor(np.concatenate(tables)).to(device)
        c0_d = torch.as_tensor(chunk0).to(device)
        err_d = torch.as_tensor(err).to(device)
        _native.gpu_unsnap_chunks(
            comp.data_ptr(), ct_d.data_ptr(), c0_d.data_ptr(), nchunk,
            data.data_ptr(), err_d.data_ptr(), _snappy_max_waves(device),
            _stream())
        err = err_d.cpu().numpy()
    ok = []
    for k, (p, meta, _) in enumerate(items):
        ok.append(int(err[k]) == -1)
        last_snappy.append((p, int(meta[0].shape[0]), int(err[k])))
    return ok


class DeviceSource(NamedTuple):
    kind: str
    meta: object
    nbytes: int


def _gzip_source(path: str) -> Optional[DeviceSource]:
    meta = gz_device_meta(path)
    if meta is None:
        return None
    return DeviceSource("gzip", meta, sum(u for _, u in meta[1]))


def _foreign_source(path: str) -> Optional[DeviceSource]:
    meta = foreign_gz_meta(path)
    return None if meta is None else DeviceSource("foreign", meta, meta[3])


def _snappy_source(path: str) -> Optional[DeviceSource]:
    meta = snappy_device_meta(path)
    return None if meta is None else DeviceSource("snappy", meta, meta[1])


def device_source(path: str,
                  foreign_gzip: bool = False) -> Optional[DeviceSource]:
    from ..io import paths as P

    codec = P.codec_from_path(path)
    if codec is None:
        return DeviceSource("raw", None, os.path.getsize(path))
    if codec == "gzip":
        return _gzip_source(path) or (_foreign_source(path) if foreign_gzip
                                      else None)
    if codec == "snappy":
        return _snappy_source(path)
    return None


def _source_image(path: str, src: Optional[DeviceSource], device,
                  chunk_bytes: Optional[int] = None) -> Optional[torch.Tensor]:
    if src is None:
        return None
    if src.kind == "raw":
        return read_file_to_device(path, device)
    data = torch.empty(max(src.nbytes, 1), dtype=torch.uint8,
                       device=device)[:src.nbytes]
    items = [(path, src.meta, 0)]
    if src.kind == "gzip":
        ok = _device_inflate_group(data, items, device)
    elif src.kind == "foreign":
        ok = _device_inflate_foreign_group(data, items, device, chunk_bytes)[0]
    else:
        ok = _device_unsnap_group(data, items, device)[0]
    return data if ok else None


def read_file_image(path: str, foreign_gzip: bool = False,
                    device="cuda") -> Optional[torch.Tensor]:
    return _source_image(path, device_source(path, foreign_gzip), device)


def read_gzip_file_to_device(path: str, device="cuda") -> Optional[torch.Tensor]:
    return _source_image(path, _gzip_source(path), device)


def read_foreign_gzip_file_to_device(path: str,
                                     chunk_bytes: Optional[int] = None,
                                     device="cuda") -> Optional[torch.Tensor]:
    check_native()
    return _source_image(path, _foreign_source(path), device, chunk_bytes)


def read_snappy_file_to_device(path: str,
                               device="cuda") -> Optional[torch.Tensor]:
    check_native()
    return _source_image(path, _snappy_source(path), device)


def _deflate_max_waves(device) -> int:
    return 8 * torch.cuda.get_device_properties(device).multi_processor_count


def gzip_image_device(img: torch.Tensor, seg: Optional[int] = None) -> torch.Tensor:
    from ..io import paths as P

    check_native()
    if img.dtype != torch.uint8 or img.dim() != 1 or not img.is_contiguous():
        raise ValueError("gzip_image_device expects a contiguous 1-D uint8 tensor")
    n = img.numel()
    if seg is None:
        seg = P._gz_segment_size(n)
    seg = int(seg)
    if seg <= 0:
        raise ValueError(f"segment size must be positive, got {seg}")
    nseg = max(1, -(-n // seg))
    if nseg > P._GZ_MAX_SEGS:
        raise ValueError(
            f"{n} bytes in {seg}-byte segments need {nseg} segments; the "
            f"gzip segment table holds at most {P._GZ_MAX_SEGS}")
    device = img.device
    seg_max = min(seg, n)
    slot = (_native.deflate_seg_out_bound(seg_max) + 7) & ~7
    nwaves = min(-(-nseg // 4) * 4, _deflate_max_waves(device))
    tok_cap = max(seg_max, 1)
    staging = torch.empty(nseg * slot, dtype=torch.uint8, device=device)
    tok_ws = torch.empty(nwaves * tok_cap, dtype=torch.int32, device=device)
    comp_len = torch.empty(nseg, dtype=torch.int64, device=device)
    comp_off = torch.empty(nseg + 1, dtype=torch.int64, device=device)
    seg_crc = torch.empty(nseg, dtype=torch.int32, device=device)
    err = torch.full((1,), -1, dtype=torch.int64, device=device)
    result = torch.empty(2, dtype=torch.int64, device=device)
    body_off = 20 + 8 * nseg
    out_cap = body_off + nseg * slot + 8
    out = torch.empty(out_cap, dtype=torch.uint8, device=device)
    _native.gpu_deflate_segments(
        img.data_ptr(), n, seg, nseg, staging.data_ptr(), slot,
        comp_len.data_ptr(), seg_crc.data_ptr(), tok_ws.data_ptr(), tok_cap,
        nwaves, float(P._GZ_STORED_THRESHOLD), err.data_ptr(), _stream())
    _excl_sum_into(comp_off.data_ptr(), comp_len.data_ptr(), 1, nseg, device)
    _native.gpu_gzip_assemble(
        staging.data_ptr(), slot, comp_len.data_ptr(), comp_off.data_ptr(),
        seg_crc.data_ptr(), n, seg, nseg, out.data_ptr(), out_cap,
        err.data_ptr(), result.data_ptr(), _stream())
    size, err_word = (int(v) for v in result.tolist())
    if err_word != -1:
        raise RuntimeError(
            f"device deflate failed: segment {(err_word >> 8) - 1}, "
            f"cause {err_word & 0xFF}")
    return out[:size]


def _snap_max_waves(device) -> int:
    blocks_per_cu = max(1, (160 << 10) // int(_native.SNAP_LDS_BYTES_PER_BLOCK))
    return (int(_native.SNAP_WAVES_PER_BLOCK) * blocks_per_cu *
            torch.cuda.get_device_properties(device).multi_processor_count)


def snappy_image_device(img: torch.Tensor,
                        block: Optional[int] = None) -> torch.Tensor:
    from ..io import paths as P

    check_native()
    if img.dtype != torch.uint8 or img.dim() != 1 or not img.is_contiguous():
        raise ValueError(
            "snappy_image_device expects a contiguous 1-D uint8 tensor")
    if block is None:
        block = P.snappy_block_size()
    block = int(block)
    if block <= 0:
        raise ValueError(f"block size must be positive, got {block}")
    if block > SNAPPY_MAX_CHUNK_RAW:
        raise ValueError(
            f"block size {block} is above the device's {SNAPPY_MAX_CHUNK_RAW}"
            " bytes per chunk")
    n = img.numel()
    device = img.device
    if n == 0:
        return torch.empty(0, dtype=torch.uint8, device=device)
    nblk = -(-n // block)
    slot = (_native.snappy_out_bound(min(block, n)) + 7) & ~7
    nwaves = min(-(-nblk // 4) * 4, _snap_max_waves(device))
    staging = torch.empty(nblk * slot, dtype=torch.uint8, device=device)
    comp_len = torch.empty(nblk, dtype=torch.int64, device=device)
    comp_off = torch.empty(nblk + 1, dtype=torch.int64, device=device)
    err = torch.full((1,), -1, dtype=torch.int64, device=device)
    result = torch.empty(2, dtype=torch.int64, device=device)
    out_cap = nblk * (8 + 10) + n
    out = torch.empty(out_cap, dtype=torch.uint8, device=device)
    _native.gpu_snap_blocks(
        img.data_ptr(), n, block, nblk, staging.data_ptr(), slot,
        comp_len.data_ptr(), nwaves, err.data_ptr(), _stream())
    _excl_sum_into(comp_off.data_ptr(), comp_len.data_ptr(), 1, nblk, device)
    _native.gpu_snappy_assemble(
        staging.data_ptr(), slot, comp_len.data_ptr(), comp_off.data_ptr(),
        n, block, nblk, out.data_ptr(), out_cap, err.data_ptr(),
        result.data_ptr(), _stream())
    size, err_word = (int(v) for v in result.tolist())
    if err_word != -1:
        raise RuntimeError(
            f"device snappy compress failed: block {(err_word >> 8) - 1}, "
            f"cause {err_word & 0xFF}")
    if size > out_cap:
        raise RuntimeError(
            f"device snappy compress: image of {size} bytes, room for {out_cap}")
    return out[:size]


def read_files_to_batch(paths, schema: StructType, record_type: str,
                        verify_crc: bool = True, device="cuda",
                        foreign_gzip: bool = False, sources=None):
    from ..io import paths as P

    check_native()
    if sources is None:
        sources = [device_source(p, foreign_gzip) for p in paths]
    for p, src in zip(paths, sources):
        if src is None:
            what = {"gzip": "gzip file without segment table",
                    "snappy": "snappy file not for the device decoder"}
            raise ValueError(
                f"{what.get(P.codec_from_path(p), 'file not for the device')}"
                f": {p} (host path required)")
    sizes = [src.nbytes for src in sources]
    n = sum(sizes)
    if n == 0:
        if schema is None:
            raise ValueError(
                "Could not infer schema: no non-empty TFRecord files found")
        z = torch.zeros(0, dtype=torch.int64, device=device)
        return (decode_device(torch.zeros(0, dtype=torch.uint8, device=device),
                              z, z.clone(), schema, record_type, verify_crc),
                np.zeros(len(paths), np.int64))
    data = torch.empty(n, dtype=torch.uint8, device=device)
    bounds = np.zeros(len(paths) + 1, np.int64)
    np.cumsum(sizes, out=bounds[1:])
    raw_files = []
    items = {"gzip": [], "foreign": [], "snappy": []}
    for p, src, base in zip(paths, sources, bounds):
        if src.kind == "raw":
            raw_files.append((p, src.nbytes, int(base)))
        elif src.nbytes:
            items[src.kind].append((p, src.meta, int(base)))
    gz_items, foreign_items, snappy_items = (
        items["gzip"], items["foreign"], items["snappy"])
    _upload_files(data, raw_files)
    if foreign_items:
        ok = _device_inflate_foreign_group(data, foreign_items, device)
        refused = [it[0] for it, good in zip(foreign_items, ok) if not good]
        if refused:
            raise ForeignGzipRejected(refused)
    if snappy_items:
        ok = _device_unsnap_group(data, snappy_items, device)
        refused = [it[0] for it, good in zip(snappy_items, ok) if not good]
        if refused:
            raise SnappyRejected(refused)
    if gz_items and not _device_inflate_group(data, gz_items, device):
        import logging

        logging.getLogger(__name__).warning(
            "device inflate rejected a segment; host zlib fallback for "
            "%d gzip file(s)", len(gz_items))
        for p, meta, base in gz_items:
            blob = np.frombuffer(P.decompress_file(p), np.uint8)
            stage = pinned_buffer("gzfb", blob.size)
            stage.numpy()[:blob.size] = blob
            data[base:base + blob.size].copy_(stage[:blob.size],
                                              non_blocking=True)
            torch.cuda.current_stream().synchronize()
    off, lens = scan_frames_device(data)
    frame_start = off - 12
    counts = torch.searchsorted(
        frame_start, torch.as_tensor(bounds, device=device)).cpu().numpy()
    row_counts = np.diff(counts)
    if schema is None:
        from ..infer import byte_array_schema, schema_from_codes

        if record_type == "ByteArray":
            schema = byte_array_schema()
        else:
            i = next((k for k in range(len(paths)) if row_counts[k] > 0), None)
            if i is None:
                raise ValueError(
                    "Could not infer schema: no non-empty TFRecord files found")
            r0, r1 = int(counts[i]), int(counts[i + 1])
            codes = infer_codes_device(data, off[r0:r1].contiguous(),
                                       lens[r0:r1].contiguous(), record_type)
            schema = schema_from_codes(codes)
    batch = decode_device(data, off, lens, schema, record_type, verify_crc)
    return batch, row_counts


def encode_partitions_device(batch: RecordBatch, part_codes: np.ndarray,
                             num_parts: int, record_type: str):
    check_native()
    R = batch.num_rows
    device = batch.columns[0].presence.device if batch.columns else torch.device("cuda")
    cols_dev, blob, psize, frame_off = _size_records(batch, record_type, device)
    total = int(frame_off[-1].item())
    file = torch.empty(total, dtype=torch.uint8, device=device)
    err = torch.zeros(2, dtype=torch.int32, device=device)
    _native.gpu_emit_records(cols_dev.data_ptr(), blob.data_ptr(),
                             FMT[record_type], 0, R, frame_off.data_ptr(),
                             file.data_ptr(), err.data_ptr(), _stream(),
                             total // max(R, 1))
    codes = torch.as_tensor(np.ascontiguousarray(part_codes, np.int64),
                            device=device)
    order = torch.argsort(codes, stable=True)
    sizes = psize[order].contiguous()
    dst_off = excl_sum(sizes)
    src_off = frame_off[:-1][order].contiguous()
    out = torch.empty(total, dtype=torch.uint8, device=device)
    _native.gpu_gather_payloads(file.data_ptr(), src_off.data_ptr(),
                                sizes.data_ptr(), dst_off.data_ptr(), R,
                                out.data_ptr(), _stream(), total // max(R, 1))
    counts = torch.bincount(codes, minlength=num_parts)
    row_bound = torch.nn.functional.pad(torch.cumsum(counts, 0), (1, 0))
    byte_bound = dst_off[row_bound].cpu().numpy()
    _check_emit_err(err)
    ranges = [(p, int(byte_bound[p]), int(byte_bound[p + 1]))
              for p in range(num_parts) if byte_bound[p + 1] > byte_bound[p]]
    return out, ranges



_INFER_SLOTS = 2048
_INFER_SLOTS_MAX = 1 << 21
_ERR_OVERFLOW = -5
_ERR_NAME_TOO_LONG = -6


def infer_codes_device(data: torch.Tensor, off: torch.Tensor,
                       lens: torch.Tensor, record_type: str) -> dict:
    check_native()
    device = data.device
    fmt = FMT["SequenceExample" if record_type == "SequenceExample" else "Example"]
    R = off.numel()
    slots = _INFER_SLOTS
    while True:
        table = torch.zeros((slots, 3), dtype=torch.int64, device=device)
        err = torch.zeros(2, dtype=torch.int32, device=device)
        if R:
            _native.gpu_infer_codes(data.data_ptr(), off.data_ptr(),
                                    lens.data_ptr(), R, fmt, table.data_ptr(),
                                    slots, err.data_ptr(), _stream())
        tab = table.cpu().numpy()
        rc = int(err[0].item())
        if rc == _ERR_OVERFLOW:
            if slots < _INFER_SLOTS_MAX:
                slots *= 4
                continue
            raise RuntimeError(
                "schema inference failed: more than "
                f"{_INFER_SLOTS_MAX // 2} distinct feature names")
        if rc == _ERR_NAME_TOO_LONG:
            raise RuntimeError(
                "schema inference failed: a feature name exceeds 65535 bytes")
        if rc != 0:
            rec = int(err[1].item()) - 1
            where = f" (record {rec})" if rec >= 0 else ""
            raise RuntimeError(f"malformed record during schema inference"
                               f"{where} (native error {rc})")
        break
    used = np.nonzero(tab[:, 0])[0]
    if len(used) == 0:
        return {}
    refs = tab[used, 1]
    offs = (refs >> 16).astype(np.int64)
    nlens = (refs & 0xFFFF).astype(np.int64)
    lo = int(offs.min())
    hi = int((offs + nlens).max())
    codes: dict = {}
    if hi - lo <= (4 << 20):
        blob = data[lo:hi].cpu().numpy().tobytes()
        for o, ln, code in zip(offs, nlens, tab[used, 2]):
            name = blob[o - lo:o - lo + ln].decode("utf-8", errors="replace")
            codes[name] = max(codes.get(name, 0), int(code))
    else:
        for o, ln, code in zip(offs, nlens, tab[used, 2]):
            name = data[o:o + ln].cpu().numpy().tobytes().decode("utf-8", errors="replace")
            codes[name] = max(codes.get(name, 0), int(code))
    return codes


def infer_schema_file(path: str, record_type: str, device="cuda"):
    from ..infer import schema_from_codes

    data = read_file_to_device(path, device)
    off, lens = scan_frames_device(data)
    return schema_from_codes(infer_codes_device(data, off, lens, record_type))


def batch_to_device(batch: RecordBatch, device="cuda") -> RecordBatch:
    cols = []
    for c in batch.columns:
        cols.append(WireColumn(
            c.kind, c.is_seq,
            _dev(c.presence, torch.uint8, device),
            _dev(c.row_off, torch.int64, device),
            _dev(c.values, {KIND_INT64: torch.int64, KIND_FLOAT: torch.float32,
                            KIND_BYTES: torch.uint8}[c.kind], device),
            _dev(c.elem_off, torch.int64, device) if c.elem_off is not None else None,
            _dev(c.list_off, torch.int64, device) if c.list_off is not None else None,
            _dev(c.sub_off, torch.int64, device) if c.sub_off is not None else None,
        ))
    return RecordBatch(batch.schema, cols, batch.num_rows)


def batch_to_host(batch: RecordBatch) -> RecordBatch:
    streams = _dma_streams()
    main = torch.cuda.current_stream()
    state = {"used": False, "k": 0}

    def h(t):
        if not isinstance(t, torch.Tensor):
            return t
        if not t.is_cuda:
            return t.numpy()
        host = torch.empty_like(t, device="cpu", pin_memory=True)
        if not state["used"]:
            for s in streams:
                s.wait_stream(main)
            state["used"] = True
        nbytes = t.numel() * t.element_size()
        if nbytes >= (8 << 20) and t.is_contiguous() and len(streams) > 1:
            flat_d = t.view(-1)
            flat_h = host.view(-1)
            n = flat_d.numel()
            step = (n + len(streams) - 1) // len(streams)
            for i, st in enumerate(streams):
                lo = i * step
                hi = min(n, lo + step)
                if lo >= hi:
                    break
                with torch.cuda.stream(st):
                    flat_h[lo:hi].copy_(flat_d[lo:hi], non_blocking=True)
                t.record_stream(st)
            return host.numpy()
        st = streams[state["k"] % len(streams)]
        state["k"] += 1
        with torch.cuda.stream(st):
            host.copy_(t, non_blocking=True)
        t.record_stream(st)
        return host.numpy()

    cols = [WireColumn(c.kind, c.is_seq, h(c.presence), h(c.row_off), h(c.values),
                       h(c.elem_off) if c.elem_off is not None else None,
                       h(c.list_off) if c.list_off is not None else None,
                       h(c.sub_off) if c.sub_off is not None else None)
            for c in batch.columns]
    if state["used"]:
        for s in streams:
            s.synchronize()
    return RecordBatch(batch.schema, cols, batch.num_rows)



def decode_buffer_to_cpu(data_np: np.ndarray, schema: StructType, record_type: str,
                         verify_crc: bool = True) -> RecordBatch:
    return batch_to_host(decode_buffer_device(data_np, schema, record_type,
                                              verify_crc))


def encode_batch_from_cpu(batch: RecordBatch, record_type: str) -> bytes:
    dev_batch = batch_to_device(batch)
    file = encode_device(dev_batch, record_type)
    return device_to_bytes(file)
```

Before: 116.9 million rows/s.

## Stage record spans in LDS, cache frame masks, fuse gate and block scan

The scan kernel now runs wave-cooperatively. Each wave copies the contiguous byte span covering its records into shared memory with 16-byte vector loads, then parses and checksums from that copy instead of from scattered global reads. Frame scanning saves a per-chunk candidate bitmask during the count pass, so the emit pass reads the mask rather than re-running the CRC frame evaluation. The extract gate kernel is folded into the extract kernels, and the block-count exclusive scan is folded into the snapshot kernel, which removes separate launches. The cost is more shared memory per block, which can lower occupancy, plus added code complexity.

```diff
diff --git a/csrc/codec_core.h b/csrc/codec_core.h
--- a/csrc/codec_core.h
+++ b/csrc/codec_core.h
@@ -747,13 +747,13 @@
   return ERR_OK;
 }
 
-TFR_HOSTDEV inline int32_t scan_record_fused(const u8* data, i64 abs_off,
-                                             i64 rec_len, int32_t fmt,
-                                             const SchemaView& schema,
-                                             FieldStat* stats, u32* crc_out,
-                                             const uint32_t (*tab)[256]) {
+TFR_HOSTDEV inline int32_t scan_record_fused_at(const u8* payload, i64 abs_off,
+                                                i64 rec_len, int32_t fmt,
+                                                const SchemaView& schema,
+                                                FieldStat* stats, u32* crc_out,
+                                                const uint32_t (*tab)[256]) {
   ScanCur c;
-  cur_init(c, data + abs_off, rec_len, tab);
+  cur_init(c, payload, rec_len, tab);
   while (c.pos < rec_len) {
     u64 tag;
     if (!cur_varint(c, rec_len, &tag)) return ERR_BAD_VARINT;
@@ -774,6 +774,15 @@
   }
   *crc_out = cur_finish_crc(c);
   return ERR_OK;
+}
+
+TFR_HOSTDEV inline int32_t scan_record_fused(const u8* data, i64 abs_off,
+                                             i64 rec_len, int32_t fmt,
+                                             const SchemaView& schema,
+                                             FieldStat* stats, u32* crc_out,
+                                             const uint32_t (*tab)[256]) {
+  return scan_record_fused_at(data + abs_off, abs_off, rec_len, fmt, schema,
+                              stats, crc_out, tab);
 }
 
 
diff --git a/csrc/hip/kernels.hip b/csrc/hip/kernels.hip
--- a/csrc/hip/kernels.hip
+++ b/csrc/hip/kernels.hip
@@ -10,6 +10,7 @@
 #include <unistd.h>
 
 #include <cstdint>
+#include <cstdlib>
 #include <map>
 #include <mutex>
 #include <stdexcept>
@@ -69,47 +70,119 @@
 
 static_assert(sizeof(FieldStat) == 48, "FieldStat layout shared with Python");
 
-__global__ void scan_records_kernel(const u8* __restrict__ data,
-                                    const i64* __restrict__ off,
-                                    const i64* __restrict__ len, i64 R, int32_t fmt,
-                                    const u8* __restrict__ schema_blob, int F,
-                                    FieldStat* __restrict__ stats,
-                                    int32_t* __restrict__ err,
-                                    unsigned long long* crc_err,
-                                    i64 rec_base, const i64* gate) {
+#ifndef TFREC_SCAN_WAVES
+#define TFREC_SCAN_WAVES 10
+#endif
+#ifndef TFREC_SCAN_STAGE_BYTES
+#define TFREC_SCAN_STAGE_BYTES 15360
+#endif
+constexpr int kScanWaves = TFREC_SCAN_WAVES;
+constexpr int kScanBlock = kScanWaves * 64;
+constexpr int kScanStageBytes = TFREC_SCAN_STAGE_BYTES;
+constexpr int kScanStageSlot = kScanStageBytes + 16;
+
+__device__ inline void wave_lds_fence() {
+  __builtin_amdgcn_fence(__ATOMIC_ACQ_REL, "wavefront");
+  __builtin_amdgcn_wave_barrier();
+}
+
+__device__ inline const u8* stage_span(const u8* __restrict__ src, i64 n,
+                                       u8* __restrict__ slot, int lane) {
+  int mis = (int)(reinterpret_cast<uintptr_t>(src) & 15);
+  u8* dst = slot + mis;
+  i64 head = (16 - mis) & 15;
+  if (head > n) head = n;
+  if (lane < head) dst[lane] = src[lane];
+  i64 nvec = (n - head) >> 4;
+  const uint4* s4 = reinterpret_cast<const uint4*>(src + head);
+  uint4* d4 = reinterpret_cast<uint4*>(dst + head);
+#pragma unroll 4
+  for (i64 i = lane; i < nvec; i += 64) d4[i] = s4[i];
+  i64 done = head + (nvec << 4);
+  if (done + lane < n) dst[done + lane] = src[done + lane];
+  return dst;
+}
+
+__global__ __launch_bounds__(kScanBlock) void scan_records_kernel(
+    const u8* __restrict__ data, const i64* __restrict__ off,
+    const i64* __restrict__ len, i64 R, int32_t fmt,
+    const u8* __restrict__ schema_blob, int F, FieldStat* __restrict__ stats,
+    int32_t* __restrict__ err, unsigned long long* crc_err, i64 rec_base,
+    const i64* gate, int stage) {
   __shared__ uint32_t tab[8][256];
+  extern __shared__ __attribute__((aligned(16))) u8 staged[];
   if (gate && *gate) return;
   if (crc_err) stage_crc_tables(tab);
   SchemaView schema = schema_view(schema_blob);
-  for (i64 r = blockIdx.x * (i64)blockDim.x + threadIdx.x; r < R;
-       r += (i64)gridDim.x * blockDim.x) {
-    FieldStat* st = stats + r * F;
-    for (int f = 0; f < F; ++f) field_stat_clear(&st[f]);
-    int32_t rc;
-    if (crc_err) {
-      u32 payload_crc = 0;
-      rc = scan_record_fused(data, off[r], len[r], fmt, schema, st,
-                             &payload_crc, tab);
-      if (rc == ERR_RETRY_UNFUSED) {
+  const int lane = threadIdx.x & 63;
+  u8* slot = staged + (size_t)(threadIdx.x >> 6) * kScanStageSlot;
+  const bool do_stage = stage && crc_err;
+  for (i64 rb = blockIdx.x * (i64)blockDim.x + (threadIdx.x & ~63u); rb < R;
+       rb += (i64)gridDim.x * blockDim.x) {
+    const i64 r = rb + lane;
+    bool pending = r < R;
+    const i64 o = pending ? off[r] : 0;
+    const i64 l = pending ? len[r] : 0;
+    while (__ballot(pending)) {
+      bool mine = pending;
+      const u8* payload = data + o;
+      if (do_stage) {
+        i64 plo = pending ? o - 12 : INT64_MAX;
+        i64 phi = pending ? o + l + 4 : INT64_MIN;
+        for (int d = 1; d < 64; d <<= 1) {
+          i64 a = __shfl_up(plo, d);
+          i64 b = __shfl_up(phi, d);
+          if (lane >= d) {
+            plo = a < plo ? a : plo;
+            phi = b > phi ? b : phi;
+          }
+        }
+        bool fits = pending && (u64)(phi - plo) <= (u64)kScanStageBytes;
+        unsigned long long take = __ballot(fits);
+        if (take == 0) {
+          mine = lane == __builtin_ctzll(__ballot(pending));
+        } else {
+          int last = 63 - __builtin_clzll(take);
+          i64 lo = __shfl(plo, last);
+          i64 hi = __shfl(phi, last);
+          wave_lds_fence();
+          const u8* copy = stage_span(data + lo, hi - lo, slot, lane);
+          wave_lds_fence();
+          mine = fits;
+          if (mine) payload = copy + (o - lo);
+        }
+      }
+      if (mine) {
+        FieldStat* st = stats + r * F;
         for (int f = 0; f < F; ++f) field_stat_clear(&st[f]);
-        rc = scan_record(data, off[r], len[r], fmt, schema, st);
-        payload_crc = crc32c_sw(data + off[r], (size_t)len[r], 0, tab);
+        int32_t rc;
+        if (crc_err) {
+          u32 payload_crc = 0;
+          rc = scan_record_fused_at(payload, o, l, fmt, schema, st,
+                                    &payload_crc, tab);
+          if (rc == ERR_RETRY_UNFUSED) {
+            for (int f = 0; f < F; ++f) field_stat_clear(&st[f]);
+            rc = scan_record(data, o, l, fmt, schema, st);
+            payload_crc = crc32c_sw(data + o, (size_t)l, 0, tab);
+          }
+          if (rc != ERR_OK)
+            payload_crc = crc32c_sw(data + o, (size_t)l, 0, tab);
+          const u8* h = payload - 12;
+          u32 len_crc, data_crc;
+          __builtin_memcpy(&len_crc, h + 8, 4);
+          __builtin_memcpy(&data_crc, h + 12 + l, 4);
+          bool ok = mask_crc(crc32c_sw(h, 8, 0, tab)) == len_crc &&
+                    mask_crc(payload_crc) == data_crc;
+          if (!ok) atomicMin(crc_err, (unsigned long long)(rec_base + r + 1));
+        } else {
+          rc = scan_record(data, o, l, fmt, schema, st);
+        }
+        if (rc != ERR_OK) set_err(err, rc, rec_base + r);
+        for (int f = 0; f < F; ++f)
+          if (st[f].err != ERR_OK) set_err(err, st[f].err, rec_base + r);
       }
-      if (rc != ERR_OK)
-        payload_crc = crc32c_sw(data + off[r], (size_t)len[r], 0, tab);
-      const u8* h = data + off[r] - 12;
-      u32 len_crc, data_crc;
-      __builtin_memcpy(&len_crc, h + 8, 4);
-      __builtin_memcpy(&data_crc, h + 12 + len[r], 4);
-      bool ok = mask_crc(crc32c_sw(h, 8, 0, tab)) == len_crc &&
-                mask_crc(payload_crc) == data_crc;
-      if (!ok) atomicMin(crc_err, (unsigned long long)(rec_base + r + 1));
-    } else {
-      rc = scan_record(data, off[r], len[r], fmt, schema, st);
-    }
-    if (rc != ERR_OK) set_err(err, rc, rec_base + r);
-    for (int f = 0; f < F; ++f)
-      if (st[f].err != ERR_OK) set_err(err, st[f].err, rec_base + r);
+      pending = pending && !mine;
+    }
   }
 }
 
@@ -144,17 +217,23 @@
   }
 }
 
-__global__ void extract_gate_kernel(const DevFieldDst* __restrict__ metas, int F,
-                                    i64 r_end, const i64* broken,
-                                    const unsigned long long* crc,
-                                    const int32_t* scan_err, i64* refused) {
+struct ExtractGate {
+  const i64* broken;
+  const unsigned long long* crc;
+  const int32_t* scan_err;
+  i64* out;
+};
+
+__device__ inline bool extract_refused(const DevFieldDst* __restrict__ metas,
+                                       int F, i64 r_end, const ExtractGate& g) {
+  const int lane = threadIdx.x & 63;
   int bad = 0;
-  if (threadIdx.x == 0) {
-    if (broken && *broken) bad = 1;
-    if (crc && *crc != ~0ULL) bad = 1;
-    if (scan_err && scan_err[0] != 0) bad = 1;
-  }
-  for (int f = threadIdx.x; f < F; f += blockDim.x) {
+  if (lane == 0) {
+    if (g.broken && *g.broken) bad = 1;
+    if (g.crc && *g.crc != ~0ULL) bad = 1;
+    if (g.scan_err && g.scan_err[0] != 0) bad = 1;
+  }
+  for (int f = lane; f < F; f += 64) {
     const DevFieldDst& m = metas[f];
     i64 nv = m.val_base ? m.val_base[r_end] : 0;
     i64 nb = m.byte_base ? m.byte_base[r_end] : 0;
@@ -166,16 +245,17 @@
     }
     if (m.is_seq && nl + 1 > m.cap_sub_off) bad = 1;
   }
-  int any = __syncthreads_or(bad);
-  if (threadIdx.x == 0) *refused = any ? 1 : 0;
+  bool any = __any(bad) != 0;
+  if (blockIdx.x == 0 && threadIdx.x == 0) *g.out = any ? 1 : 0;
+  return any;
 }
 
 __global__ void extract_fields_kernel(const u8* __restrict__ data, i64 R, int F,
                                       const FieldStat* __restrict__ stats,
                                       const DevFieldDst* __restrict__ metas,
                                       int32_t* __restrict__ err, i64 r0,
-                                      const i64* refused) {
-  if (refused && *refused) return;
+                                      ExtractGate gate) {
+  if (gate.out && extract_refused(metas, F, r0 + R, gate)) return;
   store_end_sentinels(metas, F, r0 + R);
   i64 total = R * F;
   for (i64 idx = blockIdx.x * (i64)blockDim.x + threadIdx.x; idx < total;
@@ -548,8 +628,8 @@
                                            const FieldStat* __restrict__ stats,
                                            const DevFieldDst* __restrict__ metas,
                                            int32_t* __restrict__ err, i64 r0,
-                                           const i64* refused) {
-  if (refused && *refused) return;
+                                           ExtractGate gate) {
+  if (gate.out && extract_refused(metas, F, r0 + R, gate)) return;
   store_end_sentinels(metas, F, r0 + R);
   i64 total = R * F;
   i64 wave = (blockIdx.x * (i64)blockDim.x + threadIdx.x) / 64;
@@ -828,42 +908,61 @@
                                        i64 block_base,
                                        i64* __restrict__ block_data,
                                        i64* __restrict__ cand_pos,
-                                       i64* __restrict__ cand_len) {
-  __shared__ uint32_t tab[8][256];
+                                       i64* __restrict__ cand_len,
+                                       uint16_t* __restrict__ mask) {
   __shared__ unsigned int cnt[256];
-  stage_crc_tables(tab);
-  const u64* wdata = reinterpret_cast<const u64*>(data);
   i64 c_lo = pos_start / kPosPerLane;
   i64 c_hi = (pos_end + kPosPerLane - 1) / kPosPerLane;
   i64 c = c_lo + (i64)blockIdx.x * blockDim.x + threadIdx.x;
-  unsigned int my = 0;
-  if (c < c_hi)
-    eval_frame_chunk(data, wdata, N, c, pos_start, pos_end, tab,
-                     [&](i64, i64) { ++my; });
+  i64 p0 = c * kPosPerLane;
+  unsigned int m = 0;
+  if constexpr (!EMIT) {
+    __shared__ uint32_t tab[8][256];
+    stage_crc_tables(tab);
+    const u64* wdata = reinterpret_cast<const u64*>(data);
+    if (c < c_hi) {
+      eval_frame_chunk(data, wdata, N, c, pos_start, pos_end, tab,
+                       [&](i64 i, i64) { m |= 1u << (int)(i - p0); });
+      unsigned int keep = 0;
+      if (pos_start > p0)
+        keep = mask[c] & ((1u << (int)(pos_start - p0)) - 1u);
+      mask[c] = (uint16_t)(m | keep);
+    }
+  } else {
+    if (c < c_hi) {
+      m = mask[c];
+      if (pos_start > p0) m &= ~((1u << (int)(pos_start - p0)) - 1u);
+      if (pos_end < p0 + kPosPerLane) m &= (1u << (int)(pos_end - p0)) - 1u;
+    }
+  }
+  unsigned int my = __popc(m);
   cnt[threadIdx.x] = my;
   __syncthreads();
-  if (!EMIT) {
+  if constexpr (!EMIT) {
     for (int off = blockDim.x / 2; off; off >>= 1) {
       if ((int)threadIdx.x < off) cnt[threadIdx.x] += cnt[threadIdx.x + off];
       __syncthreads();
     }
     if (threadIdx.x == 0) block_data[block_base + blockIdx.x] = (i64)cnt[0];
-    return;
-  }
-  for (int off = 1; off < (int)blockDim.x; off <<= 1) {
-    unsigned int v = (int)threadIdx.x >= off ? cnt[threadIdx.x - off] : 0;
-    __syncthreads();
-    cnt[threadIdx.x] += v;
-    __syncthreads();
-  }
-  i64 slot = block_data[block_base + blockIdx.x] + (i64)(cnt[threadIdx.x] - my);
-  if (c < c_hi)
-    eval_frame_chunk(data, wdata, N, c, pos_start, pos_end, tab,
-                     [&](i64 i, i64 len) {
-                       cand_pos[slot] = i;
-                       cand_len[slot] = len;
-                       ++slot;
-                     });
+  } else {
+    for (int off = 1; off < (int)blockDim.x; off <<= 1) {
+      unsigned int v = (int)threadIdx.x >= off ? cnt[threadIdx.x - off] : 0;
+      __syncthreads();
+      cnt[threadIdx.x] += v;
+      __syncthreads();
+    }
+    i64 slot =
+        block_data[block_base + blockIdx.x] + (i64)(cnt[threadIdx.x] - my);
+    while (m) {
+      int k = __builtin_ctz(m);
+      m &= m - 1;
+      i64 len;
+      __builtin_memcpy(&len, data + p0 + k, 8);
+      cand_pos[slot] = p0 + k;
+      cand_len[slot] = len;
+      ++slot;
+    }
+  }
 }
 
 __global__ void frame_chain_kernel(const i64* __restrict__ pos,
@@ -882,15 +981,67 @@
   }
 }
 
-__global__ void stream_snapshot_kernel(const i64* count, const i64* status,
-                                       int nst, const i64* carry, const i64* v,
-                                       const i64* b, const i64* l, i64 stride,
-                                       int F, i64 r, i64* out) {
+constexpr int kSnapScanItems = 4;
+
+__device__ inline i64 finish_block_counts(const i64* __restrict__ counts,
+                                          i64 nb, i64* __restrict__ block_off) {
+  __shared__ i64 wave_sum[2][kBlock / 64];
+  const int lane = threadIdx.x & 63, wave = threadIdx.x >> 6;
+  const i64 tile = (i64)kBlock * kSnapScanItems;
+  auto load = [&](i64 t0, i64* v) {
+    i64 i0 = t0 + (i64)threadIdx.x * kSnapScanItems;
+#pragma unroll
+    for (int j = 0; j < kSnapScanItems; ++j)
+      v[j] = i0 + j < nb ? counts[i0 + j] : 0;
+  };
+  i64 carry = 0;
+  i64 v[kSnapScanItems], next[kSnapScanItems];
+  load(0, v);
+  int parity = 0;
+  for (i64 t0 = 0; t0 < nb; t0 += tile, parity ^= 1) {
+    load(t0 + tile, next);
+    i64 sum = 0;
+#pragma unroll
+    for (int j = 0; j < kSnapScanItems; ++j) sum += v[j];
+    i64 incl = sum;
+    for (int d = 1; d < 64; d <<= 1) {
+      i64 a = __shfl_up(incl, d);
+      if (lane >= d) incl += a;
+    }
+    if (lane == 63) wave_sum[parity][wave] = incl;
+    __syncthreads();
+    i64 before = 0, total = 0;
+#pragma unroll
+    for (int w = 0; w < kBlock / 64; ++w) {
+      i64 x = wave_sum[parity][w];
+      if (w < wave) before += x;
+      total += x;
+    }
+    i64 i0 = t0 + (i64)threadIdx.x * kSnapScanItems;
+    i64 run = carry + before + incl - sum;
+#pragma unroll
+    for (int j = 0; j < kSnapScanItems; ++j) {
+      if (i0 + j < nb) block_off[i0 + j] = run;
+      run += v[j];
+      v[j] = next[j];
+    }
+    carry += total;
+  }
+  if (threadIdx.x == 0) block_off[nb] = carry;
+  return carry;
+}
+
+__global__ __launch_bounds__(kBlock) void stream_snapshot_kernel(
+    const i64* count, const i64* status, int nst, const i64* carry,
+    const i64* v, const i64* b, const i64* l, i64 stride, int F, i64 r,
+    i64* out, const i64* block_counts, i64 nb, i64* block_off) {
+  i64 counted = 0;
+  if (block_counts) counted = finish_block_counts(block_counts, nb, block_off);
   int n = 2 + nst + (v ? 3 * F : 0);
   for (int i = threadIdx.x; i < n; i += blockDim.x) {
     i64 x;
     if (i == 0) {
-      x = count ? *count : 0;
+      x = block_counts ? counted : count ? *count : 0;
     } else if (i <= nst) {
       x = status[i - 1];
     } else if (i == nst + 1) {
@@ -1167,6 +1318,22 @@
   HIP_CHECK(hipGetLastError());
 }
 
+inline bool scan_stage_enabled() {
+  const char* v = std::getenv("TFREC_SCAN_STAGE");
+  return !(v && v[0] == '0' && v[1] == 0);
+}
+
+inline void allow_scan_stage_lds(size_t bytes) {
+  thread_local int allowed_device = -1;
+  int dev = 0;
+  HIP_CHECK(hipGetDevice(&dev));
+  if (allowed_device == dev) return;
+  HIP_CHECK(hipFuncSetAttribute(
+      reinterpret_cast<const void*>(&scan_records_kernel),
+      hipFuncAttributeMaxDynamicSharedMemorySize, (int)bytes));
+  allowed_device = dev;
+}
+
 void gpu_scan_records(uintptr_t data, uintptr_t off, uintptr_t len, i64 R,
                       int32_t fmt, uintptr_t schema_blob, int F, uintptr_t stats,
                       uintptr_t err, uintptr_t crc_err, uintptr_t stream,
@@ -1182,12 +1349,20 @@
                        (unsigned long long*)crc_err, rec_base,
                        (const i64*)gate);
   } else {
-    hipLaunchKernelGGL(scan_records_kernel, dim3(grid_for(R, max_blocks)),
-                       dim3(kBlock), 0, (hipStream_t)stream, (const u8*)data,
-                       (const i64*)off, (const i64*)len, R, fmt,
-                       (const u8*)schema_blob, F, (FieldStat*)stats,
+    bool stage = scan_stage_enabled() && crc_err &&
+                 (avg_bytes + 16) * 64 <= 2 * (i64)kScanStageBytes;
+    int threads = stage ? kScanBlock : kBlock;
+    size_t lds = stage ? (size_t)kScanWaves * kScanStageSlot : 0;
+    if (stage) allow_scan_stage_lds(lds);
+    i64 blocks = (R + threads - 1) / threads;
+    i64 cap = max_blocks > 0 && max_blocks < 8192 ? max_blocks : 8192;
+    if (blocks > cap) blocks = cap;
+    hipLaunchKernelGGL(scan_records_kernel, dim3((uint32_t)blocks),
+                       dim3(threads), lds, (hipStream_t)stream,
+                       (const u8*)data, (const i64*)off, (const i64*)len, R,
+                       fmt, (const u8*)schema_blob, F, (FieldStat*)stats,
                        (int32_t*)err, (unsigned long long*)crc_err, rec_base,
-                       (const i64*)gate);
+                       (const i64*)gate, stage ? 1 : 0);
   }
   HIP_CHECK(hipGetLastError());
 }
@@ -1230,25 +1405,21 @@
                              sizeof(DevFieldDst) * F, hipMemcpyHostToDevice,
                              (hipStream_t)stream));
   }
-  if (gate_out) {
-    hipLaunchKernelGGL(extract_gate_kernel, dim3(1), dim3(kBlock), 0,
-                       (hipStream_t)stream, (const DevFieldDst*)meta_dev, F,
-                       r0 + R, (const i64*)gate_broken,
-                       (const unsigned long long*)gate_crc,
-                       (const int32_t*)gate_err, (i64*)gate_out);
-  }
+  ExtractGate gate{(const i64*)gate_broken,
+                   (const unsigned long long*)gate_crc,
+                   (const int32_t*)gate_err, (i64*)gate_out};
   if (avg_bytes > kWaveRecordBytes) {
     hipLaunchKernelGGL(extract_fields_wave_kernel,
                        dim3(grid_for(R * F * 64, max_blocks)), dim3(kBlock), 0,
                        (hipStream_t)stream, (const u8*)data, R, F,
                        (const FieldStat*)stats, (const DevFieldDst*)meta_dev,
-                       (int32_t*)err, r0, (const i64*)gate_out);
+                       (int32_t*)err, r0, gate);
   } else {
     hipLaunchKernelGGL(extract_fields_kernel,
                        dim3(grid_for(R * F, max_blocks)), dim3(kBlock), 0,
                        (hipStream_t)stream, (const u8*)data, R, F,
                        (const FieldStat*)stats, (const DevFieldDst*)meta_dev,
-                       (int32_t*)err, r0, (const i64*)gate_out);
+                       (int32_t*)err, r0, gate);
   }
   HIP_CHECK(hipGetLastError());
 }
@@ -1262,7 +1433,8 @@
 void gpu_stream_snapshot(uintptr_t count, uintptr_t status, int nst,
                          uintptr_t carry, uintptr_t v, uintptr_t b, uintptr_t l,
                          i64 stride, int F, i64 r, uintptr_t out_host,
-                         uintptr_t stream) {
+                         uintptr_t stream, uintptr_t block_counts, i64 nb,
+                         uintptr_t block_off) {
   int dev = 0;
   HIP_CHECK(hipGetDevice(&dev));
   SnapshotEvent& se = snapshot_event;
@@ -1274,11 +1446,14 @@
   }
   void* out_dev = nullptr;
   HIP_CHECK(hipHostGetDevicePointer(&out_dev, (void*)out_host, 0));
+  if (block_counts && (nb <= 0 || !block_off))
+    throw std::runtime_error("gpu_stream_snapshot: block_counts without nb/block_off");
   hipLaunchKernelGGL(stream_snapshot_kernel, dim3(1), dim3(kBlock), 0,
                      (hipStream_t)stream, (const i64*)count,
                      (const i64*)status, nst, (const i64*)carry, (const i64*)v,
                      (const i64*)b, (const i64*)l, stride, v ? F : 0, r,
-                     (i64*)out_dev);
+                     (i64*)out_dev, (const i64*)block_counts, nb,
+                     (i64*)block_off);
   HIP_CHECK(hipGetLastError());
   HIP_CHECK(hipEventRecord(se.ev, (hipStream_t)stream));
 }
@@ -1366,28 +1541,30 @@
   return (n + kBlock - 1) / kBlock;
 }
 
+i64 gpu_frame_mask_words(i64 N) { return (N + kPosPerLane - 1) / kPosPerLane; }
+
 void gpu_frame_scan_count(uintptr_t data, i64 N, i64 pos_start, i64 pos_end,
                           i64 block_base, uintptr_t block_counts,
-                          uintptr_t stream) {
+                          uintptr_t mask, uintptr_t stream) {
   i64 B = gpu_frame_scan_blocks(pos_start, pos_end);
   if (B <= 0) return;
   hipLaunchKernelGGL(frame_scan_pass_kernel<false>, dim3((uint32_t)B),
                      dim3(kBlock), 0, (hipStream_t)stream, (const u8*)data, N,
                      pos_start, pos_end, block_base, (i64*)block_counts,
-                     nullptr, nullptr);
+                     nullptr, nullptr, (uint16_t*)mask);
   HIP_CHECK(hipGetLastError());
 }
 
 void gpu_frame_scan_emit(uintptr_t data, i64 N, i64 pos_start, i64 pos_end,
                          i64 block_base, uintptr_t block_off,
                          uintptr_t cand_pos, uintptr_t cand_len,
-                         uintptr_t stream) {
+                         uintptr_t mask, uintptr_t stream) {
   i64 B = gpu_frame_scan_blocks(pos_start, pos_end);
   if (B <= 0) return;
   hipLaunchKernelGGL(frame_scan_pass_kernel<true>, dim3((uint32_t)B),
                      dim3(kBlock), 0, (hipStream_t)stream, (const u8*)data, N,
                      pos_start, pos_end, block_base, (i64*)block_off,
-                     (i64*)cand_pos, (i64*)cand_len);
+                     (i64*)cand_pos, (i64*)cand_len, (uint16_t*)mask);
   HIP_CHECK(hipGetLastError());
 }
 
@@ -1712,6 +1889,7 @@
         py::arg("F"), py::arg("stats"), py::arg("err"), py::arg("crc_err"),
         py::arg("stream"), py::arg("avg_bytes") = 0, py::arg("rec_base") = 0,
         py::arg("max_blocks") = 0, py::arg("gate") = 0);
+  m.attr("SCAN_STAGE_BYTES") = (int)kScanStageBytes;
   m.def("gpu_extract_fields", &gpu_extract_fields, py::arg("data"),
         py::arg("R"), py::arg("F"), py::arg("stats"), py::arg("metas"),
         py::arg("meta_dev"), py::arg("err"), py::arg("stream"),
@@ -1722,7 +1900,9 @@
   m.def("gpu_stream_snapshot", &gpu_stream_snapshot, py::arg("count"),
         py::arg("status"), py::arg("nst"), py::arg("carry"), py::arg("v"),
         py::arg("b"), py::arg("l"), py::arg("stride"), py::arg("F"),
-        py::arg("r"), py::arg("out_host"), py::arg("stream"));
+        py::arg("r"), py::arg("out_host"), py::arg("stream"),
+        py::arg("block_counts") = 0, py::arg("nb") = 0,
+        py::arg("block_off") = 0);
   m.def("gpu_stream_snapshot_wait", &gpu_stream_snapshot_wait);
   m.def("gpu_size_records", &gpu_size_records);
   m.def("gpu_emit_records", &gpu_emit_records, py::arg("cols_dev"),
@@ -1733,6 +1913,7 @@
         py::arg("elem_off"), py::arg("frame_off"), py::arg("R"),
         py::arg("file"), py::arg("stream"), py::arg("avg_bytes") = 0);
   m.def("gpu_frame_scan_blocks", &gpu_frame_scan_blocks);
+  m.def("gpu_frame_mask_words", &gpu_frame_mask_words);
   m.def("gpu_frame_scan_count", &gpu_frame_scan_count);
   m.def("gpu_frame_scan_emit", &gpu_frame_scan_emit);
   m.def("gpu_frame_chain", &gpu_frame_chain);
diff --git a/spark_tfrecord_amd/engine/gpu.py b/spark_tfrecord_amd/engine/gpu.py
--- a/spark_tfrecord_amd/engine/gpu.py
+++ b/spark_tfrecord_amd/engine/gpu.py
@@ -266,13 +266,20 @@
         return z, z.clone()
     B = _native.gpu_frame_scan_blocks(0, N)
     block_counts = torch.empty(B, dtype=torch.int64, device=device)
+    mask = _frame_mask(N, device)
     _native.gpu_frame_scan_count(data.data_ptr(), N, 0, N, 0,
-                                 block_counts.data_ptr(), _stream())
-    off, lens, _ = _emit_and_chain(data, [(0, N)], block_counts, N)
+                                 block_counts.data_ptr(), mask.data_ptr(),
+                                 _stream())
+    off, lens, _ = _emit_and_chain(data, [(0, N)], block_counts, mask, N)
     return off, lens
 
 
-def _emit_and_chain(data, ranges, block_counts, N):
+def _frame_mask(N: int, device) -> torch.Tensor:
+    return torch.empty(max(int(_native.gpu_frame_mask_words(N)), 1),
+                       dtype=torch.int16, device=device)
+
+
+def _emit_and_chain(data, ranges, block_counts, mask, N):
     device = data.device
     block_off = excl_sum(block_counts)
     C = int(block_off[-1].item())
@@ -284,7 +291,8 @@
     for s, e in ranges:
         _native.gpu_frame_scan_emit(data.data_ptr(), N, s, e, base,
                                     block_off.data_ptr(), pos.data_ptr(),
-                                    lens.data_ptr(), _stream())
+                                    lens.data_ptr(), mask.data_ptr(),
+                                    _stream())
         base += _native.gpu_frame_scan_blocks(s, e)
     expect_next = pos + 16 + lens
     ok = bool(((pos[0] == 0) & (expect_next[-1] == N)
@@ -759,10 +767,11 @@
 
 class _StreamedRead:
 
-    def __init__(self, data: torch.Tensor, nslices: int, schema: StructType,
-                 record_type: str, verify_crc: bool):
+    def __init__(self, data: torch.Tensor, mask: torch.Tensor, nslices: int,
+                 schema: StructType, record_type: str, verify_crc: bool):
         device = data.device
         self.data = data
+        self.mask = mask
         self.n = data.numel()
         self.schema = schema
         self.record_type = record_type
@@ -786,16 +795,21 @@
         self.clean = True
         self.avg_bytes = None
 
-    def _snapshot(self, count_ptr: int, r: int) -> _Snapshot:
+    def _snapshot(self, r: int, counts: Optional[torch.Tensor] = None,
+                  block_off: Optional[torch.Tensor] = None) -> _Snapshot:
         F = self.F if self.rows.planes is not None else 0
         n = 2 + _ST_CARRY + 3 * F
         buf = pinned_buffer("snapshot", n * 8)
         v, b, l = ([t.data_ptr() for t in self.rows.planes] if F
                    else (0, 0, 0))
+        scan = {}
+        if counts is not None:
+            scan = dict(block_counts=counts.data_ptr(), nb=counts.numel(),
+                        block_off=block_off.data_ptr())
         _native.gpu_stream_snapshot(
-            count_ptr, self.status.addr(0), _ST_CARRY,
+            0, self.status.addr(0), _ST_CARRY,
             self.status.carry_addr(self.nchain), v, b, l, self.rows.cap + 1,
-            F, r, buf.data_ptr(), _stream())
+            F, r, buf.data_ptr(), _stream(), **scan)
         _native.gpu_stream_snapshot_wait()
         last_read["host_waits"] = last_read.get("host_waits", 0) + 1
         return _Snapshot(buf.numpy()[:n * 8].view(np.int64).copy(), F)
@@ -824,11 +838,11 @@
 
     def step(self, p: stream_plan.SlicePlan, counts: Optional[torch.Tensor],
              last: bool) -> bool:
-        count_ptr = 0
+        block_off = None
         if counts is not None:
-            block_off = excl_sum(counts)
-            count_ptr = block_off.data_ptr() + counts.numel() * 8
-        snap = self._snapshot(count_ptr, self.r_done)
+            block_off = torch.empty(counts.numel() + 1, dtype=torch.int64,
+                                    device=counts.device)
+        snap = self._snapshot(self.r_done, counts, block_off)
         if snap.broken:
             return False
         if self.do_scan:
@@ -840,7 +854,7 @@
             _native.gpu_frame_scan_emit(self.data.data_ptr(), self.n,
                                         p.scan_lo, p.scan_hi, 0,
                                         block_off.data_ptr(), pos, lens,
-                                        _stream())
+                                        self.mask.data_ptr(), _stream())
             _native.gpu_frame_chain(pos, lens, c_s,
                                     self.status.carry_addr(self.nchain),
                                     self.status.carry_addr(self.nchain + 1),
@@ -871,7 +885,7 @@
         if not self.sized:
             if last:
                 return True
-            snap = self._snapshot(0, avail)
+            snap = self._snapshot(avail)
             if snap.broken:
                 return False
             self._settle(snap)
@@ -887,7 +901,7 @@
         R, n = self.C, self.n
         if R == 0:
             return None
-        snap = self._snapshot(0, R)
+        snap = self._snapshot(R)
         if snap.broken or snap.chain_end != n:
             return None
         if not self.do_scan:
@@ -905,7 +919,7 @@
             self._extract(R, gated=False)
             self.x_done = R
             self.vals.confirm(snap.totals)
-            xerr = self._snapshot(0, R).xerr
+            xerr = self._snapshot(R).xerr
         val_base, _, list_base = self.rows.planes
         cols = self.vals.columns(self.rows.presence, val_base, list_base, R)
         if xerr[0] != 0:
@@ -943,7 +957,7 @@
     return int(_native.gpu_frame_scan_blocks(p.scan_lo, p.scan_hi))
 
 
-def _count_slice(data, p, evs, block_counts, base: int) -> int:
+def _count_slice(data, p, evs, block_counts, mask, base: int) -> int:
     main = torch.cuda.current_stream()
     for ev in evs:
         main.wait_event(ev)
@@ -951,19 +965,20 @@
     if nb:
         _native.gpu_frame_scan_count(data.data_ptr(), data.numel(), p.scan_lo,
                                      p.scan_hi, base, block_counts.data_ptr(),
-                                     _stream())
+                                     mask.data_ptr(), _stream())
     return nb
 
 
-def _read_unstreamed(data, plan, block_counts, events, first: int,
+def _read_unstreamed(data, plan, block_counts, mask, events, first: int,
                      schema: StructType, record_type: str,
                      verify_crc: bool) -> RecordBatch:
     last_read["path"] = "fallback" if _STREAM_DECODE else "unstreamed"
     base = sum(_scan_blocks(p) for p in plan[:first])
     for p, evs in zip(plan[first:], events[first:]):
-        base += _count_slice(data, p, evs, block_counts, base)
+        base += _count_slice(data, p, evs, block_counts, mask, base)
     ranges = [(p.scan_lo, p.scan_hi) for p in plan if p.scan_hi > p.scan_lo]
-    off, lens, _ = _emit_and_chain(data, ranges, block_counts, data.numel())
+    off, lens, _ = _emit_and_chain(data, ranges, block_counts, mask,
+                                   data.numel())
     return decode_device(data, off, lens, schema, record_type, verify_crc)
 
 
@@ -987,17 +1002,18 @@
     S = len(plan)
     block_counts = torch.empty(max(sum(_scan_blocks(p) for p in plan), 1),
                                dtype=torch.int64, device=data.device)
+    mask = _frame_mask(n, data.device)
     events = _issue_h2d_slices(data, ptr, plan)
     last_read.update(path="streamed", slices=S, regrows=0, host_waits=0)
-    unstreamed = (data, plan, block_counts, events)
+    unstreamed = (data, plan, block_counts, mask, events)
     decode = (schema, record_type, verify_crc)
     if not _STREAM_DECODE:
         return _read_unstreamed(*unstreamed, 0, *decode)
 
-    rd = _StreamedRead(data, S, *decode)
+    rd = _StreamedRead(data, mask, S, *decode)
     base = 0
     for s, p in enumerate(plan):
-        nb = _count_slice(data, p, events[s], block_counts, base)
+        nb = _count_slice(data, p, events[s], block_counts, mask, base)
         counts = block_counts[base:base + nb] if nb else None
         base += nb
         if not rd.step(p, counts, last=s == S - 1):
```

New measurement: 115.3 million rows/s. 1.3% lower.
